# Blackgaurd/pathtracer-cpp

Hardware: AMD Instinct MI355X
Metric: Mray/s (all bounces) + achieved HBM GB/s, Cornell 1024² 10k spp depth-5 (higher is better)
Workload: dtype f32

## Files before the change

include/pt_hip_debug.h:

```cpp
#ifndef PT_HIP_DEBUG_H
#define PT_HIP_DEBUG_H

#include "pt_hip.h"

#ifdef __cplusplus
extern "C" {
#endif

int pt_debug_math(int device, int which, const float* in, int n, float* out);
int pt_debug_sweep(int device, int which, uint32_t lo_bits, uint32_t hi_bits, uint64_t* mismatches,
                   uint32_t* first_bad);
int pt_debug_rgb8(int device, const float* linear_rgb, int32_t res_x, int32_t res_y, float gamma, uint8_t* rgb8);
int pt_debug_rccl_failover(int32_t n_devices, int32_t fail_step, int64_t* out);
int pt_debug_wide_verify(const pt_scene* scene, int32_t width);
int pt_debug_pack_hash(const pt_scene* scene, uint64_t* hash);
int pt_rtc_check(const pt_scene* scene, char* src_out, size_t cap);
int pt_debug_rtc_start(const pt_scene* scene);
int64_t pt_debug_rtc_cache(int32_t op);

int pt_debug_ctx_flags(const pt_ctx* ctx, int32_t out[5]);
int pt_debug_ctx_plan(const pt_ctx* ctx, int64_t out[24]);
int pt_debug_walk_placement(int32_t num_nodes, int32_t num_tris, int32_t tree_depth, int32_t tri_f4,
                            int32_t rec_rows, uint64_t lds_usable, int32_t out[4]);
int pt_debug_scene_dark(const pt_scene* scene);
int pt_debug_emit_reject(const float* box6, const float* org, const float* dir, int64_t n, uint8_t* out);
int pt_debug_emit_slab_reject(const float* box6, const float* org, const float* inv, int64_t n, uint8_t* out);
int pt_debug_emit_box(const pt_scene* scene, float out[6]);
int pt_debug_ctx_emit_reject(const pt_ctx* ctx, int32_t* on, float box[6], uint64_t* early);
int pt_debug_ray_stack(int32_t which, int32_t count, int32_t n, int32_t reserve, int32_t flag);
int64_t pt_debug_counter(int32_t which);

#ifdef __cplusplus
}
#endif
#endif
```

pathtracer-cpp_amd/csrc/pt_kernel.hip:

```cpp
#include <hip/hip_runtime.h>

#include <stdint.h>
#include <stdio.h>
#include <stdlib.h>
#include <string.h>

#include <algorithm>
#include <chrono>
#include <future>
#include <map>
#include <memory>
#include <mutex>
#include <string>
#include <thread>
#include <vector>

#include <atomic>

#include "pt_grad.h"
#include "pt_hip_debug.h"
#include "pt_launch.h"
#include "pt_moments.h"
#include "pt_nee_grad.h"
#include "pt_rtc.h"
// ... 226 lines not shown
            const v3 r = __builtin_fabsf(x) <= 2.0f ? rcp3_exact<true>(v3{x, x, x}) : rcp3_exact<false>(v3{x, x, x});
            const uint32_t q = __float_as_uint(1.0f / x);
            same = __float_as_uint(r.x) == q && __float_as_uint(r.y) == q && __float_as_uint(r.z) == q;
        } else if (which >= 6 && which <= 9) {
            const uint32_t h1 = pt_mix32(bits * 0x9e3779b9u + 0x7f4a7c15u), h2 = pt_mix32(h1 ^ 0x85ebca6bu);
            auto pick = [&](uint32_t h, uint32_t k) {
                const uint32_t sign = h & 0x80000000u, mant = h & 0x7fffffu;
                if (which <= 7 && (bits & 15u) == 11u) {
                    switch (k & 7u) {
                        case 0: return __uint_as_float(sign);
                        case 1: return __uint_as_float(sign | mant | 1u);
                        case 2: return 0x1p127f;
                        case 3: return __uint_as_float(sign | 0x7f800000u);
                        case 4: return __uint_as_float(sign | 0x7e800000u | mant | 1u);
                        case 5: return __uint_as_float(sign | 0x7f000000u | mant);
                        case 6: return __uint_as_float(sign | 1u);
                        default: return __uint_as_float(0x80000000u);
                    }
                }
                const uint32_t e = (which == 6 || which == 9) ? 1u + (h >> 23) % 252u : 87u + (h >> 23) % 81u;
                return __uint_as_float(sign | (e << 23) | mant);
            };
            v3 a{x, pick(h1, h1 >> 8), pick(h2, (h1 >> 8) + 3u)};
            if (which == 9 && (bits & 15u) == 11u) a.y = __uint_as_float((h1 & 0x80000000u) | 0x7fc00000u | (h1 & 0x3fffffu));
            v3 r, q;
            if (which == 6 || which == 9) {
                r = rcp3_exact<false>(a);
                q = v3{1.0f / a.x, 1.0f / a.y, 1.0f / a.z};
            } else {
                r = normalize_fast(a);
                const float len = __builtin_sqrtf(dot(a, a));
                q = v3{a.x / len, a.y / len, a.z / len};
            }
            same = __float_as_uint(r.x) == __float_as_uint(q.x) &&
                   (__float_as_uint(r.y) == __float_as_uint(q.y) || (which == 9 && r.y != r.y && q.y != q.y)) &&
                   __float_as_uint(r.z) == __float_as_uint(q.z);
        } else {
            float s1, c1, s0, c0;
            sincosf_fast(x, s1, c1);
            sincosf_ref(x, s0, c0);
            same = __float_as_uint(s1) == __float_as_uint(s0) && __float_as_uint(c1) == __float_as_uint(c0);
        }
        if (!same) {
            nb++;
            fb = min(fb, bits);
        }
    }
    if (nb) {
        atomicAdd(bad, nb);
        atomicMin(first, fb);
    }
}

}

using namespace pt;

struct pt_ctx {
    int device = 0;
    hipStream_t stream = nullptr;
    std::thread init;
    std::once_flag init_once;
    std::string init_error;
    bool counted = false;
    int num_cus = 0;
    size_t lds_usable = 0;
    float4* d_nodes = nullptr;
    float4* d_tris = nullptr;
    float4* d_mats = nullptr;
    float4* d_leaves = nullptr;
    float4* d_wide = nullptr;
    float4* d_wtris = nullptr;
    float4* d_nrm = nullptr;
    float4* d_umats = nullptr;
    int32_t* d_rank_tri = nullptr;
    std::vector<f4> flat_host;
    FlatLeaves flat_tab;
    int flat_boxes_padded = 0;
    PackedScene meta;
    bool have_scene = false;
    bool has_specular = false;
    bool albedo_x2 = false;
    bool dark = false;
    EmitBox emit;
    uint64_t last_early = 0;
    void* flat_fast = nullptr;
    int flat_boxes = 0;
    bool rtc_requested = false;
    float* d_radiance = nullptr;
    size_t radiance_floats = 0;
    uint32_t* d_flags = nullptr;
    size_t flags_words = 0;
    float* d_accum = nullptr;
    size_t accum_floats = 0;
    float* d_out = nullptr;
    size_t out_floats = 0;
    unsigned long long* d_ctr = nullptr;
    unsigned long long* d_stamps = nullptr;
    int* d_xstack = nullptr;
    size_t xstack_ints = 0;
    uint8_t* d_rgb8 = nullptr;
    size_t rgb8_bytes = 0;
    float* d_thr = nullptr;
    int* d_qstack = nullptr;
    size_t qstack_ints = 0;
    float* d_qbuf = nullptr;
    size_t qbuf_floats = 0;
    unsigned long long* d_qhits = nullptr;
    float* d_tslab = nullptr;
    size_t tslab_floats = 0;
    float* d_trec = nullptr;
    size_t trec_words = 0;
    float* d_tbuf = nullptr;
    size_t tbuf_floats = 0;
    float* d_tstates = nullptr;
    size_t tstates_words = 0;
    unsigned long long* d_tctr = nullptr;
    LightTable lights;
    bool lights_uploaded = false;
    uint8_t* d_lights = nullptr;
    size_t lights_bytes = 0;
    double* d_gtab = nullptr;
    size_t gtab_doubles = 0;
    float4* d_gmats = nullptr;
    size_t gmats_f4 = 0;
    float* d_gbuf = nullptr;
    size_t gbuf_floats = 0;
    double* d_mom = nullptr;
    size_t mom_doubles = 0;
    unsigned long long* d_mcount = nullptr;
    float* d_sem = nullptr;
    size_t sem_floats = 0;
    int32_t* d_alist[2] = {nullptr, nullptr};
    size_t alist_ints[2] = {0, 0};
    int32_t* d_aspp = nullptr;
    size_t aspp_ints = 0;
    float* d_aslab = nullptr;
    size_t aslab_floats = 0;
    float* d_arec = nullptr;
    size_t arec_words = 0;
    unsigned long long* d_actr = nullptr;
    void* d_dn[kDnScratchSlots] = {};
    size_t dn_bytes[kDnScratchSlots] = {};
    TemporalState temporal;
    bool prog_valid = false;
    bool prog_moments = false;
    int prog_spp = 0;
    int prog_npix = 0;
    pt_camera prog_cam{};
    pt_params prog_prm{};
    hipFunction_t rtc_flat = nullptr;
    std::string rtc_status;
    std::string rtc_src;
    RtcFuture rtc_job;
    int64_t last_plan[24] = {};
};

namespace {

#define HIP_TRY(expr)                                                                              \
    do {                                                                                           \
        hipError_t e_ = (expr);                                                                    \
        if (e_ != hipSuccess) return set_error(PT_E_HIP, "%s failed: %s", #expr, hipGetErrorString(e_)); \
    } while (0)

int ctx_ready(pt_ctx* c) {
    std::call_once(c->init_once, [c] {
        if (c->init.joinable()) c->init.join();
    });
    if (!c->init_error.empty()) return set_error(PT_E_HIP, "%s", c->init_error.c_str());
    return PT_OK;
}

std::mutex g_dev_mu;
std::map<int, int> g_dev_contexts;

size_t batch_bytes_budget(int device, bool compile_pending) {
    const char* e = hook_env("PT_BATCH_BYTES");
    if (e && *e) return (size_t)strtoull(e, nullptr, 0);
    int sharers = 1;
    {
        std::lock_guard<std::mutex> lock(g_dev_mu);
        sharers = std::max(1, g_dev_contexts[device]);
    }
    size_t budget = ((size_t)(compile_pending ? 16 : 48) << 30) / sharers, free_b = 0, total_b = 0;
    if (hipMemGetInfo(&free_b, &total_b) == hipSuccess && free_b / 2 / sharers < budget) budget = free_b / 2 / sharers;
    return std::max<size_t>(budget, (size_t)64 << 20);
}

std::atomic<int64_t> g_ctx_created{0}, g_scene_uploads{0};

constexpr double kRtcWaitPaths = 256.0 * 1024 * 1024;

constexpr int kTailDiv = 0;

}

int64_t pt::kernel_counter(int which) { return which == 0 ? g_ctx_created.load() : g_scene_uploads.load(); }

int pt::ctx_release_slabs(pt_ctx* c) {
    if (!c) return PT_OK;
    if (int rc = ctx_ready(c)) return rc;
    HIP_TRY(hipSetDevice(c->device));
    if (c->stream) HIP_TRY(hipStreamSynchronize(c->stream));
    if (c->d_radiance) (void)hipFree(c->d_radiance);
    if (c->d_flags) (void)hipFree(c->d_flags);
    c->d_radiance = nullptr;
    c->radiance_floats = 0;
    c->d_flags = nullptr;
    c->flags_words = 0;
    if (c->d_mom) (void)hipFree(c->d_mom);
    c->d_mom = nullptr;
    c->mom_doubles = 0;
    if (c->prog_moments) c->prog_valid = false;
    return PT_OK;
}


namespace {

void rtc_resolve(pt_ctx* c, bool wait) {
    if (!c->rtc_job.valid()) return;
    if (!wait && c->rtc_job.wait_for(std::chrono::seconds(0)) != std::future_status::ready) return;
    c->rtc_flat = rtc_load(c->device, c->rtc_src, *c->rtc_job.get(), c->rtc_status);
    if (!c->rtc_flat && c->rtc_status == "evicted") {
        c->rtc_job = rtc_job(c->rtc_src);
        c->rtc_status = "compiling";
        if (wait) rtc_resolve(c, true);
        return;
    }
    c->rtc_job = RtcFuture();
    c->rtc_src.clear();
}

}

static std::mutex g_theta_mu;
static std::map<int, float2*> g_theta_tabs;

static void theta_table_release(int device) {
    std::lock_guard<std::mutex> dev_lock(g_dev_mu);
    std::lock_guard<std::mutex> lock(g_theta_mu);
    if (g_dev_contexts[device] != 0) return;
    auto it = g_theta_tabs.find(device);
    if (it == g_theta_tabs.end()) return;
    (void)hipFree(it->second);
    g_theta_tabs.erase(it);
}

[[maybe_unused]] static int theta_table(pt_ctx* c, const float2** out) {
    std::lock_guard<std::mutex> lock(g_theta_mu);
    auto it = g_theta_tabs.find(c->device);
    if (it != g_theta_tabs.end()) {
        *out = it->second;
        return PT_OK;
    }
    float2* t = nullptr;
    HIP_TRY(hipMalloc((void**)&t, sizeof(float2) * (size_t)kThetaEntries));
    hipLaunchKernelGGL(pt_theta_table_kernel, dim3((kThetaEntries + kBlock - 1) / kBlock), dim3(kBlock), 0, c->stream, t);
    const hipError_t e = hipStreamSynchronize(c->stream);
    if (e != hipSuccess) {
        (void)hipFree(t);
        return set_error(PT_E_HIP, "theta table: %s", hipGetErrorString(e));
    }
    g_theta_tabs[c->device] = t;
    *out = t;
    return PT_OK;
}

namespace {

struct RenderPlan {
    PartShape shape;
    int s_lo = 0, spp = 0;
    int batch = 0, per_item = 1, tail = 0;
    bool fused = false, flagged = false;
    bool moments = false;
    int flags_pm = 0;
    size_t slab_floats = 0, slab_words = 0;
    bool flat = false, wide = false, pairs = false, wide_single = false, lds_scene = false;
    int rec = 1, stack = 1, exact_rows = 1;
    int pair_queue = 0, wide_rows = 0, wide_queue = 0, wide_top = 0;
    size_t box_tab_bytes = 0, lds_bytes = 0;
    TraceKernel kern = nullptr;
    bool use_rtc = false;
    bool may_switch = false;
    int rtc_switch_at = -1;
    int blocks_per_cu = 1;
};

int force_exact_slab() {
    const char* fe = hook_env("PT_FORCE_EXACT_SLAB");
    return (fe && (*fe == '1' || *fe == '2')) ? *fe - '0' : 0;
}

void plan_batch(const pt_ctx* c, const pt_params* prm, RenderPlan& P) {
    const int npix = P.shape.npix, spp = P.spp, s_lo = P.s_lo;
    int batch = prm->batch_spp > 0 ? prm->batch_spp : 0;
    const bool compile_pending = c->rtc_job.valid();
    bool halved = false;
    if (batch <= 0) {
        const size_t per_sample = 3 * sizeof(float) * (size_t)std::max(npix, 1);
        const size_t whole = std::max<size_t>(1, batch_bytes_budget(c->device, compile_pending) / per_sample);
        halved = (size_t)std::max(spp - s_lo, 1) > whole;
        batch = (int)std::min<size_t>(halved ? (whole + 1) / 2 : whole, (size_t)INT32_MAX);
    }
    batch = std::max(1, std::min(batch, std::max(spp - s_lo, 1)));
    int per_item = prm->samples_per_item > 0 ? std::min(prm->samples_per_item, batch) : 1;
    batch = (int)std::min<long long>(batch, std::max<long long>(per_item, ((1ll << 31) - 1) / std::max(npix, 1) * per_item));
    if (P.flat && per_item != 1) {
        per_item = 1;
        batch = (int)std::min<long long>(batch, std::max<long long>(1, ((1ll << 31) - 1) / std::max(npix, 1)));
    }
    bool fused = (spp - s_lo) > batch && !hook_off("PT_FUSED_ACC") && !P.moments;
    if (fused && prm->batch_spp <= 0 && !halved) batch = std::max(1, (batch + 1) / 2);
    if (fused && prm->batch_spp > 0 && 2 * 3 * sizeof(float) * (size_t)batch * npix > batch_bytes_budget(c->device, compile_pending))
        fused = false;
    P.batch = batch;
    P.per_item = per_item;
    P.fused = fused;
    P.slab_floats = 3 * (size_t)batch * npix;
    const int tail_div = std::max(0, hook_int("PT_TAIL_DIV", kTailDiv));
    P.tail = fused && tail_div > 0 ? std::max(1, batch / tail_div) : 0;
    P.flagged = c->dark && !hook_off("PT_FLAGS");
    const char* pm_env = hook_env("PT_FLAGS_PM");
    const bool several = fused || (P.moments && (spp - s_lo) > batch);
    P.flags_pm = (pm_env && *pm_env) ? (*pm_env == '1' ? 1 : 0) : (several ? 1 : 0);
    P.slab_words = P.flags_pm ? ((size_t)batch + 31) / 32 * npix : ((size_t)batch * npix + 31) / 32;
}

int batch_at(const RenderPlan& P, int s0) {
    const int left = P.spp - s0;
    if (P.tail <= 0 || left <= P.tail) return std::min(P.batch, left);
    return left <= P.batch + P.tail ? left - P.tail : P.batch;
}

size_t flat_lds_bytes(const pt_ctx* c, const RenderPlan& P, int queue) {
    return sizeof(float4) * (size_t)(3 + 2) * c->meta.num_tris + sizeof(uint16_t) * (size_t)queue * (kBlock / kWave) +
           (sizeof(uint16_t) + sizeof(float)) * (size_t)kBlock * P.rec + sizeof(unsigned long long) * kBlock +
           (sizeof(float4) + sizeof(uint32_t)) * kBlock + P.box_tab_bytes;
}

void plan_flat(const pt_ctx* c, RenderPlan& P) {
    P.pairs = !hook_off("PT_PAIRS");
    P.box_tab_bytes = (sizeof(uint16_t) * (size_t)c->flat_boxes + 3) & ~(size_t)3;
    int queue = P.pairs ? 512 : 0;
    const char* pq = hook_env("PT_PAIR_QUEUE");
    if (P.pairs && pq && *pq) {
        queue = std::max(1, std::min(queue, atoi(pq)));
    } else if (P.pairs && c->lds_usable > 0) {
        auto blocks = [&](int q) { return std::min(8, lds_blocks(c->lds_usable, flat_lds_bytes(c, P, q))); };
        const int want = blocks(kPairQueueMin);
        while (queue > kPairQueueMin && blocks(queue) < want) queue -= 32;
    }
    P.pair_queue = (queue + 3) & ~3;
    P.lds_scene = true;
    P.lds_bytes = flat_lds_bytes(c, P, P.pair_queue);
}

size_t wide_lds_bytes(const pt_ctx* c, const RenderPlan& P, int top) {
    return (size_t)top * 16 * kWideNodeU4(c->meta.wide_width, c->meta.wide_fmt) + sizeof(int) * (size_t)kBlock * P.wide_rows +
           (P.wide_single ? 4 : 8) * (size_t)P.wide_queue * (kBlock / kWave) +
           (sizeof(float) + (P.lds_scene ? sizeof(uint8_t) : sizeof(int))) * (size_t)kBlock * P.rec +
           sizeof(unsigned long long) * kBlock + (P.lds_scene ? sizeof(float4) * 2 * (size_t)c->meta.num_umats : 0);
}

int plan_wide(const pt_ctx* c, RenderPlan& P) {
    if (c->meta.num_tris >= (1 << 26))
        return set_error(PT_E_ARG, "wide path: %d triangles exceed 2^26", c->meta.num_tris);
    P.wide_rows = std::max(1, c->meta.wide_depth - 1);
    P.wide_queue = 160;
    if (const char* wl = hook_env("PT_WIDE_QUEUE_LEN")) P.wide_queue = std::max(64, std::min(1024, atoi(wl)));
    P.wide_top = c->meta.wide_top;
    P.wide_single = c->meta.wide_single && !hook_off("PT_WIDE_SINGLE");
    P.lds_scene = c->meta.num_umats <= std::min(hook_int("PT_UMAT_LDS_MAX", kMaxLdsMaterials), kMaxLdsRowsByte);
    P.lds_bytes = wide_lds_bytes(c, P, P.wide_top);
    return PT_OK;
}

int shrink_wide_top(const pt_ctx* c, RenderPlan& P) {
    int full = 0, with = 0, rc;
    if ((rc = occupancy((const void*)P.kern, wide_lds_bytes(c, P, 0), c->lds_usable, &full, "render"))) return rc;
    while (P.wide_top > 0) {
        if ((rc = occupancy((const void*)P.kern, wide_lds_bytes(c, P, P.wide_top), c->lds_usable, &with, "render"))) return rc;
        if (with >= full) break;
        P.wide_top--;
    }
    P.lds_bytes = wide_lds_bytes(c, P, P.wide_top);
    return PT_OK;
}

void plan_tree(const pt_ctx* c, RenderPlan& P) {
    const size_t work = sizeof(int) * (size_t)kBlock * (P.stack + 2 * P.rec);
    const size_t scene = sizeof(float4) * ((size_t)2 * c->meta.num_nodes + (size_t)(3 + 2) * c->meta.num_tris);
    P.lds_scene = scene <= lds_scene_budget() && scene + work <= 64 * 1024;
    P.lds_bytes = work + (P.lds_scene ? scene : 0);
}

int plan_render(pt_ctx* c, const PartShape& shape, const pt_params* prm, int s_lo, int spp, bool moments, RenderPlan& P) {
    P.shape = shape;
    P.moments = moments;
    P.s_lo = s_lo;
    P.spp = spp;
    P.rec = std::max(1, prm->depth - 1);
    P.stack = std::max(1, c->meta.tree_depth);
    P.exact_rows = std::max(1, c->meta.tree_depth);
    const char* wenv = hook_env("PT_WIDE");
    const bool flat_ok = flat_eligible(c->meta) && !hook_off("PT_FLAT");
    P.wide = c->meta.num_wide > 0 && !(wenv && *wenv == '0') && (!flat_ok || (wenv && *wenv == '1'));
    P.flat = flat_ok && !P.wide;
    plan_batch(c, prm, P);
    int rc;
    if (P.flat) plan_flat(c, P);
    else if (P.wide) {
        if ((rc = plan_wide(c, P))) return rc;
    } else plan_tree(c, P);
    if (P.lds_bytes > 160 * 1024)
        return set_error(PT_E_ARG, "BVH depth (%d) x path depth needs %zu B of LDS", P.wide ? P.wide_rows : P.stack, P.lds_bytes);
    const bool rtc_switch = !hook_off("PT_RTC_SWITCH");
    P.rtc_switch_at = hook_int("PT_RTC_SWITCH_AT", -1);
    if (P.flat && c->rtc_job.valid()) rtc_resolve(c, !rtc_switch && (double)shape.npix * (spp - s_lo) >= kRtcWaitPaths);
    P.kern = P.flat        ? (c->flat_fast                    ? (TraceKernel)c->flat_fast
                              : ray_stack_on(c->has_specular) ? pt_trace_kernel<true, true>
                                                              : pt_trace_kernel<true, true, 0, kWideByte, false>)
             : P.wide      ? wide_kernel(c->meta.wide_width, c->meta.wide_fmt, P.lds_scene)
             : P.lds_scene ? pt_trace_kernel<true, false>
                           : pt_trace_kernel<false, false>;
    P.use_rtc = P.flat && c->rtc_flat != nullptr;
    if (P.wide && P.wide_top > 0 && (rc = shrink_wide_top(c, P))) return rc;
    if ((rc = P.use_rtc ? plan_grid_module(c->rtc_flat, P.lds_bytes, c->lds_usable, c->num_cus, 0, &P.blocks_per_cu, nullptr, "render")
                        : plan_grid((const void*)P.kern, P.lds_bytes, c->lds_usable, c->num_cus, 0, &P.blocks_per_cu, nullptr, "render")))
        return rc;
    P.may_switch = P.flat && !P.use_rtc && c->rtc_job.valid();
    return PT_OK;
}

int render_buffers(pt_ctx* c, const RenderPlan& P, bool out_is_device) {
    const size_t npix = (size_t)P.shape.npix;
    int rc;
    if ((rc = ensure(&c->d_accum, &c->accum_floats, 3 * npix))) return rc;
    if (P.moments && (rc = ensure(&c->d_mom, &c->mom_doubles, 6 * npix))) return rc;
    if (!out_is_device && (rc = ensure(&c->d_out, &c->out_floats, 3 * npix))) return rc;
    if (P.wide || P.flat) {
        const size_t need = (size_t)(P.may_switch ? std::max(P.blocks_per_cu, 8) : P.blocks_per_cu) * c->num_cus * kBlock * P.exact_rows;
        if ((rc = ensure(&c->d_xstack, &c->xstack_ints, need))) return rc;
    }
    if ((rc = ensure(&c->d_radiance, &c->radiance_floats, (P.fused ? 2 : 1) * P.slab_floats))) return rc;
    if (P.flagged && (rc = ensure(&c->d_flags, &c->flags_words, (P.fused ? 2 : 1) * P.slab_words))) return rc;
    return PT_OK;
}

int theta_choice(pt_ctx* c, int* lanes, const float2** tab) {
    *lanes = 0;
    *tab = nullptr;
#if PT_THETA_TAB
    *lanes = hook_int("PT_THETA_LANES", c->has_specular ? 32 : 0);
    if (PT_THETA_TAB == 1 || *lanes > 0) {
        if (int rc = theta_table(c, tab)) {
            if (PT_THETA_TAB == 1) return rc;
            *lanes = 0;
            *tab = nullptr;
        }
    }
#else
    (void)c;
#endif
    return PT_OK;
}

void build_flat_table(pt_ctx* c) {
    memset(&c->flat_tab, 0, sizeof(c->flat_tab));
    c->flat_boxes_padded = 0;
    if (!flat_eligible(c->meta)) return;
    int nb = 0;
    for (int k = 0; k < c->meta.num_leaves; k++) {
        const f4* L = &c->flat_host[2 * k];
        const float b6[6] = {L[0].x, L[0].y, L[0].z, L[0].w, L[1].x, L[1].y};
        int u = 0;
        while (u < nb && memcmp(c->flat_tab.box[u], b6, sizeof(b6)) != 0) u++;
        if (u == nb) {
            memcpy(c->flat_tab.box[nb], b6, sizeof(b6));
            c->flat_tab.bits[nb++] = 0;
        }
        c->flat_tab.bits[u] |= 1ull << k;
    }
    c->flat_boxes_padded = (nb + 3) & ~3;
    for (int u = nb; u < c->flat_boxes_padded; u++) memcpy(c->flat_tab.box[u], c->flat_tab.box[0], sizeof(c->flat_tab.box[0]));
}

int fill_trace_args(pt_ctx* c, const RenderPlan& P, const pt_camera* cam, const pt_params* prm, TraceArgs& A) {
    memset(&A, 0, sizeof(A));
    A.nodes = c->d_nodes;
    A.tris = c->d_tris;
    A.mats = c->d_mats;
    A.leaves = c->d_leaves;
    A.wide = reinterpret_cast<const uint4*>(c->d_wide);
    A.wtris = c->d_wtris;
    A.nrm = c->d_nrm;
    A.umats = c->d_umats;
    A.num_umat4 = P.wide ? 2 * c->meta.num_umats : 0;
    if (P.flat) {
        A.num_leaves = c->meta.num_leaves;
        A.num_boxes_padded = c->flat_boxes_padded;
        A.flat = c->flat_tab;
    }
    A.radiance = c->d_radiance;
    const float2* theta_tab = nullptr;
    if (int rc = theta_choice(c, &A.theta_lanes, &theta_tab)) return rc;
    A.theta_tab = theta_tab;
    A.work = c->d_ctr;
    A.ctr = c->d_ctr;
    A.dark = c->dark ? 1 : 0;
    A.emit_on = emit_mode(c->emit);
    A.emit_lo_x = c->emit.lo[0], A.emit_lo_y = c->emit.lo[1], A.emit_lo_z = c->emit.lo[2];
    A.emit_hi_x = c->emit.hi[0], A.emit_hi_y = c->emit.hi[1], A.emit_hi_z = c->emit.hi[2];
    fill_camera(A, cam, P.shape, prm);
    A.depth = prm->depth;
    A.per_item = P.per_item;
    A.stack_size = P.stack;
    A.rec_size = P.rec;
    A.num_node4 = 2 * c->meta.num_nodes;
    A.num_tri4 = 3 * c->meta.num_tris;
    A.num_mat4 = 2 * c->meta.num_tris;
    A.force_exact_slab = force_exact_slab();
    A.wide_thresh = std::max(1, std::min(64, hook_int("PT_WIDE_THRESH", 28)));
    A.pair_queue = P.pair_queue;
    A.wide_rows = P.wide_rows;
    A.exact_stack = c->d_xstack;
    A.exact_rows = P.exact_rows;
    A.wide_queue = P.wide_queue;
    A.wide_top = P.wide_top;
    A.wide_nodes = P.wide ? (uint32_t)c->meta.num_wide : 0u;
    A.wide_span_x = c->meta.wide_span[0];
    A.wide_span_y = c->meta.wide_span[1];
    A.wide_span_z = c->meta.wide_span[2];
    A.wide_single = P.wide_single ? 1 : 0;
    A.wide_compact = P.wide && c->meta.wide_compact ? 1 : 0;
    A.tri_fast = P.wide && c->meta.coords_small && !hook_off("PT_WIDE_NB") ? 1 : 0;
    const char* wq = hook_env("PT_WIDE_QUEUE_CAP");
    if (P.wide && wq && *wq) A.wide_queue = std::max(1, std::min(A.wide_queue, atoi(wq)));
    A.regen_thresh = std::max(1, std::min(64, hook_int("PT_REGEN_THRESH", c->has_specular ? 40 : 32)));
    A.ray_reserve = ray_reserve();
    A.flags_pm = P.flags_pm;
    A.acc_chunks = 0;
    return PT_OK;
}

struct RenderEvents {
    std::vector<hipEvent_t> ev;
    ~RenderEvents() {
        for (hipEvent_t e : ev) (void)hipEventDestroy(e);
    }
};

struct LaunchLog {
    std::vector<int> samples;
    int grid = 0, chunk = 0, acc_every = 0;
    uint32_t static_items = 0;
};

int launch_batch(pt_ctx* c, RenderPlan& P, TraceArgs& A, int b, int s0, int sc, int prev_s0, int prev_sc, float* dst, int keep,
                 RenderEvents& E, LaunchLog& log) {
    const int npix = P.shape.npix;
    auto flags_at = [&](int k) -> uint32_t* {
        return P.flagged ? c->d_flags + (P.fused ? (size_t)(k & 1) * P.slab_words : 0) : nullptr;
    };
    A.s_begin = s0;
    A.s_count = sc;
    float* slab = c->d_radiance + (P.fused ? (size_t)(b & 1) * P.slab_floats : 0);
    A.radiance = slab;
    A.flags = flags_at(b);
    const size_t words_b = P.flags_pm ? ((size_t)sc + 31) / 32 * npix : ((size_t)sc * npix + 31) / 32;
    if (A.flags && hipMemsetAsync(A.flags, 0, words_b * sizeof(uint32_t), c->stream) != hipSuccess)
        return set_error(PT_E_HIP, "hipMemsetAsync of the slab flags failed");
    A.total_items = (unsigned long long)((sc + P.per_item - 1) / P.per_item) * (unsigned long long)npix;
    if (A.total_items >= (1ull << 31))
        return set_error(PT_E_ARG, "batch of %d samples x %d pixels exceeds 2^31 work items", sc, npix);
    if (P.flat && !P.use_rtc && c->rtc_job.valid() && b >= 1) {
        (void)hipEventSynchronize(E.ev[3 * (size_t)(b - 1) + 1]);
        rtc_resolve(c, b == P.rtc_switch_at);
        if (c->rtc_flat) {
            int rb = 0;
            if (int rc = plan_grid_module(c->rtc_flat, P.lds_bytes, c->lds_usable, c->num_cus, 0, &rb, nullptr, "render")) return rc;
            P.blocks_per_cu = std::min(rb, 8);
            P.use_rtc = true;
        }
    }
    const unsigned long long want_blocks = (A.total_items + kBlock - 1) / kBlock;
    const int grid = (int)std::min<unsigned long long>(want_blocks, (unsigned long long)P.blocks_per_cu * c->num_cus);
    const PoolSizing pool = pool_sizing(A.total_items, grid, P.flat ? 512 : 128);
    A.chunk = pool.chunk;
    A.static_items = pool.static_items;
    A.static_base = pool.static_base;
    hipEvent_t e[3] = {nullptr, nullptr, nullptr};
    for (hipEvent_t& ek : e) {
        if (hipEventCreate(&ek) != hipSuccess) {
            for (hipEvent_t made : e)
                if (made) (void)hipEventDestroy(made);
            return set_error(PT_E_HIP, "hipEventCreate failed");
        }
    }
    E.ev.insert(E.ev.end(), e, e + 3);
    (void)hipMemsetAsync(c->d_ctr, 0, sizeof(unsigned long long), c->stream);
    if (P.fused && prev_s0 >= 0) {
        A.acc_src = c->d_radiance + (size_t)((b - 1) & 1) * P.slab_floats;
        A.acc_flags = flags_at(b - 1);
        A.acc_sum = c->d_accum;
        A.acc_count = prev_sc;
        A.acc_first = prev_s0 == 0 ? 1 : 0;
        A.acc_chunks = (npix + kWave - 1) / kWave;
        const unsigned long long refills =
            std::max<unsigned long long>(1, (A.total_items - A.static_base) / (unsigned long long)A.chunk);
        const unsigned long long div = (unsigned long long)std::max(1, hook_int("PT_ACC_DIV", 2));
        A.acc_every = (int)std::max<unsigned long long>(1, refills / (div * (unsigned long long)A.acc_chunks));
        (void)hipMemsetAsync(c->d_ctr + 2, 0, sizeof(unsigned long long), c->stream);
    } else {
        A.acc_chunks = 0;
        A.acc_flags = nullptr;
    }
    (void)hipEventRecord(e[0], c->stream);
    if (P.use_rtc) {
        size_t arg_bytes = sizeof(A);
        void* cfg[] = {HIP_LAUNCH_PARAM_BUFFER_POINTER, &A, HIP_LAUNCH_PARAM_BUFFER_SIZE, &arg_bytes,
                       HIP_LAUNCH_PARAM_END};
        const hipError_t le = hipModuleLaunchKernel(c->rtc_flat, grid, 1, 1, kBlock, 1, 1, (unsigned)P.lds_bytes,
                                                    c->stream, nullptr, cfg);
        if (le != hipSuccess) return set_error(PT_E_HIP, "hipModuleLaunchKernel failed: %s", hipGetErrorString(le));
    } else {
        hipLaunchKernelGGL(P.kern, dim3(grid), dim3(kBlock), P.lds_bytes, c->stream, A);
    }
    (void)hipEventRecord(e[1], c->stream);
    if (P.moments)
        hipLaunchKernelGGL(pt_accumulate_moments_kernel, dim3((npix + kBlock - 1) / kBlock), dim3(kBlock), 0, c->stream,
                           slab, c->d_accum, dst, c->d_mom, npix, sc, s0 == 0 ? 1 : 0, s0 + sc >= P.spp ? 1 : 0,
                           (float)P.spp, A.flags, P.flags_pm);
    else if (!P.fused || s0 + sc >= P.spp)
        hipLaunchKernelGGL(pt_accumulate_kernel, dim3((npix + kBlock - 1) / kBlock), dim3(kBlock), 0, c->stream, slab,
                           c->d_accum, dst, npix, sc, s0 == 0 ? 1 : 0, s0 + sc >= P.spp ? 1 : 0, keep, (float)P.spp, A.flags,
                           P.flags_pm);
    (void)hipEventRecord(e[2], c->stream);
    log.samples.push_back(sc);
    log.grid = grid;
    log.chunk = A.chunk;
    log.static_items = A.static_items;
    log.acc_every = A.acc_chunks ? A.acc_every : 0;
    return PT_OK;
}

#ifdef PT_STAMPS
void report_stamps(const pt_ctx* c, bool wide, const unsigned long long* h_ctr) {
    unsigned long long hs[kStampSections];
    if (hipMemcpy(hs, c->d_stamps, sizeof(hs), hipMemcpyDeviceToHost) == hipSuccess) {
        if (wide) {
            const double tot = (double)(hs[0] + hs[1] + hs[2] + hs[3] + hs[4]);
            fprintf(stderr,
                    "[stamps] wide: waves %llu  cycles/wave %.3g  start %.1f%%  steps %.1f%%  drains %.1f%%  "
                    "shade %.1f%%  fold %.1f%%  | steps/wave %.0f, traversing lanes/step %.1f, in-loop drains/wave %.0f\n",
                    hs[6], tot / (double)(hs[6] ? hs[6] : 1), 100 * hs[0] / tot, 100 * hs[1] / tot, 100 * hs[2] / tot,
                    100 * hs[3] / tot, 100 * hs[4] / tot, (double)hs[7] / (hs[6] ? hs[6] : 1),
                    (double)hs[8] / (hs[7] ? hs[7] : 1), (double)hs[9] / (hs[6] ? hs[6] : 1));
            const double oi = (double)(hs[10] ? hs[10] : 1), ray = (double)(h_ctr[1] ? h_ctr[1] : 1);
            fprintf(stderr,
// ... 201 lines not shown
            HIP_TRY(hipGetLastError());
        }
        if (!is_device) HIP_TRY(hipMemcpyAsync(mom->sem, dst, nval * sizeof(float), hipMemcpyDeviceToHost, c->stream));
    }
    HIP_TRY(hipStreamSynchronize(c->stream));
    return PT_OK;
}

int unconverged_count(pt_ctx* c, float rel, float abs_tol, int64_t* count, uint8_t* mask, int mask_is_device, double* ms) {
    const int npix = c->prog_npix;
    *count = 0;
    if (npix <= 0) return PT_OK;
    HIP_TRY(hipSetDevice(c->device));
    if (!c->d_mcount) HIP_TRY(hipMalloc((void**)&c->d_mcount, sizeof(unsigned long long)));
    uint8_t* d_mask = mask;
    if (mask && !mask_is_device) {
        if (int rc = ensure(&c->d_rgb8, &c->rgb8_bytes, (size_t)npix)) return rc;
        d_mask = c->d_rgb8;
    }
    hipEvent_t e0 = nullptr, e1 = nullptr;
    if (ms && (hipEventCreate(&e0) != hipSuccess || hipEventCreate(&e1) != hipSuccess)) {
        if (e0) (void)hipEventDestroy(e0);
        return set_error(PT_E_HIP, "hipEventCreate failed");
    }
    unsigned long long h = 0;
    hipError_t e = hipMemsetAsync(c->d_mcount, 0, sizeof(unsigned long long), c->stream);
    if (ms) (void)hipEventRecord(e0, c->stream);
    hipLaunchKernelGGL(pt_unconverged_kernel, dim3((npix + kBlock - 1) / kBlock), dim3(kBlock), 0, c->stream, c->d_mom, npix,
                       c->prog_spp, (double)rel, (double)abs_tol, c->d_mcount, d_mask);
    if (ms) (void)hipEventRecord(e1, c->stream);
    if (e == hipSuccess) e = hipGetLastError();
    if (e == hipSuccess) e = hipMemcpyAsync(&h, c->d_mcount, sizeof(h), hipMemcpyDeviceToHost, c->stream);
    if (e == hipSuccess && mask && !mask_is_device)
        e = hipMemcpyAsync(mask, d_mask, (size_t)npix, hipMemcpyDeviceToHost, c->stream);
    if (e == hipSuccess) e = hipStreamSynchronize(c->stream);
    if (ms) {
        float t = 0;
        if (e == hipSuccess && hipEventElapsedTime(&t, e0, e1) == hipSuccess) *ms += t;
        (void)hipEventDestroy(e0);
        (void)hipEventDestroy(e1);
    }
    if (e != hipSuccess) return set_error(PT_E_HIP, "convergence count failed: %s", hipGetErrorString(e));
    *count = (int64_t)h;
    return PT_OK;
}

}

extern "C" {

int pt_device_count(void) {
    int n = 0;
    if (hipGetDeviceCount(&n) != hipSuccess) return 0;
    return n;
}

int pt_ctx_create(int device, pt_ctx** out) {
    if (!out) return set_error(PT_E_ARG, "pt_ctx_create: out is NULL");
    *out = nullptr;
    const bool timed = hook_env("PT_TIME_CTX") != nullptr;
    auto t_last = std::chrono::steady_clock::now();
    auto phase = [&](const char* what) {
        if (!timed) return;
        const auto t = std::chrono::steady_clock::now();
        fprintf(stderr, "[pt_ctx_create] %s %.3f ms\n", what, std::chrono::duration<double, std::milli>(t - t_last).count());
        t_last = t;
    };
    int n = 0;
    if (hipGetDeviceCount(&n) != hipSuccess || n <= 0) return set_error(PT_E_HIP, "no HIP device available");
    if (device < 0 || device >= n) return set_error(PT_E_ARG, "device %d out of range (have %d)", device, n);
    HIP_TRY(hipSetDevice(device));
    phase("device count + set");
    pt_ctx* c = new pt_ctx();
    c->device = device;
    hipDeviceProp_t prop;
    if (hipGetDeviceProperties(&prop, device) != hipSuccess) {
        delete c;
        return set_error(PT_E_HIP, "hipGetDeviceProperties failed");
    }
    phase("device properties");
    c->num_cus = prop.multiProcessorCount;
    c->lds_usable = strncmp(prop.gcnArchName, "gfx950", 6) == 0 ? kLdsUsable
                    : prop.sharedMemPerMultiprocessor > 0   ? (size_t)prop.sharedMemPerMultiprocessor
                                                            : (size_t)65536;
    auto make = [c] {
        if (hipSetDevice(c->device) != hipSuccess) c->init_error = "hipSetDevice failed";
        else if (hipStreamCreateWithFlags(&c->stream, hipStreamNonBlocking) != hipSuccess)
            c->init_error = "stream creation failed";
        else if (hipMalloc((void**)&c->d_ctr, 5 * sizeof(unsigned long long)) != hipSuccess)
            c->init_error = "counter allocation failed";
    };
    const char* cs = hook_env("PT_CTX_SYNC");
    if (!(cs && *cs == '1')) {
        try {
            c->init = std::thread(make);
        } catch (const std::system_error&) {
        }
    }
    if (!c->init.joinable()) make();
    if (!c->init_error.empty()) {
        const std::string err = c->init_error;
        pt_ctx_destroy(c);
        return set_error(PT_E_HIP, "%s", err.c_str());
    }
    phase("stream + counter (started)");
    {
        std::lock_guard<std::mutex> lock(g_dev_mu);
        g_dev_contexts[device]++;
    }
    c->counted = true;
    g_ctx_created++;
    *out = c;
    return PT_OK;
}

void pt_ctx_destroy(pt_ctx* c) {
    if (!c) return;
    (void)ctx_ready(c);
    bool last = false;
    if (c->counted) {
        std::lock_guard<std::mutex> lock(g_dev_mu);
        last = --g_dev_contexts[c->device] == 0;
    }
    (void)hipSetDevice(c->device);
    if (c->stream) (void)hipStreamSynchronize(c->stream);
    if (last) theta_table_release(c->device);
    for (void* p : {(void*)c->d_nodes, (void*)c->d_tris, (void*)c->d_mats, (void*)c->d_leaves, (void*)c->d_wide, (void*)c->d_wtris, (void*)c->d_nrm, (void*)c->d_umats, (void*)c->d_radiance, (void*)c->d_flags,
                    (void*)c->d_accum, (void*)c->d_out, (void*)c->d_ctr, (void*)c->d_stamps, (void*)c->d_rgb8, (void*)c->d_thr, (void*)c->d_xstack,
                    (void*)c->d_rank_tri, (void*)c->d_qstack, (void*)c->d_qbuf, (void*)c->d_qhits,
                    (void*)c->d_tslab, (void*)c->d_trec, (void*)c->d_tbuf, (void*)c->d_tstates, (void*)c->d_tctr,
                    (void*)c->d_lights,
                    (void*)c->d_gtab, (void*)c->d_gmats, (void*)c->d_gbuf, (void*)c->d_mom, (void*)c->d_mcount, (void*)c->d_sem,
                    (void*)c->d_alist[0], (void*)c->d_alist[1], (void*)c->d_aspp, (void*)c->d_aslab, (void*)c->d_arec, (void*)c->d_actr})
        if (p) (void)hipFree(p);
    for (void* p : c->d_dn)
        if (p) (void)hipFree(p);
    if (c->stream) (void)hipStreamDestroy(c->stream);
    delete c;
}

int pt_ctx_set_scene(pt_ctx* c, const pt_scene* scene) {
    if (!c) return set_error(PT_E_ARG, "context is NULL");
    g_scene_uploads++;
    PackedScene ps;
    int rc = pack_scene(scene, ps);
    if (rc) return rc;
    const bool specular = scene_has_specular(ps);
    const bool albedo_x2 = albedo_x2_ok(ps);
    const bool dark = scene_dark(ps);
    const EmitBox emit = scene_emit_box(ps, dark);
    const bool want_rtc = flat_eligible(ps) && !hook_off("PT_RTC");
    std::string src;
    RtcFuture job;
    if (want_rtc) {
        src = rtc_flat_source(ps.leaves, ps.num_leaves, specular, ps.coords_small, albedo_x2, dark, emit);
        job = rtc_job(src);
    }
    if ((rc = ctx_ready(c))) return rc;
    HIP_TRY(hipSetDevice(c->device));
    for (float4** p : {&c->d_nodes, &c->d_tris, &c->d_mats, &c->d_leaves, &c->d_wide, &c->d_wtris, &c->d_nrm, &c->d_umats}) {
        if (*p) (void)hipFree(*p);
        *p = nullptr;
    }
    if (c->d_rank_tri) (void)hipFree(c->d_rank_tri);
    c->d_rank_tri = nullptr;
    c->have_scene = false;
    c->prog_valid = false;
    c->temporal.valid = false;
    c->lights_uploaded = false, scene_light_table(scene, c->lights);
    HIP_TRY(hipMalloc((void**)&c->d_nodes, ps.nodes.size() * sizeof(float4)));
    HIP_TRY(hipMalloc((void**)&c->d_tris, ps.tris.size() * sizeof(float4)));
    HIP_TRY(hipMalloc((void**)&c->d_mats, ps.mats.size() * sizeof(float4)));
    HIP_TRY(hipMemcpyAsync(c->d_nodes, ps.nodes.data(), ps.nodes.size() * sizeof(float4), hipMemcpyHostToDevice,
                           c->stream));
    HIP_TRY(hipMemcpyAsync(c->d_tris, ps.tris.data(), ps.tris.size() * sizeof(float4), hipMemcpyHostToDevice,
                           c->stream));
    HIP_TRY(hipMemcpyAsync(c->d_mats, ps.mats.data(), ps.mats.size() * sizeof(float4), hipMemcpyHostToDevice,
                           c->stream));
    HIP_TRY(hipMalloc((void**)&c->d_rank_tri, ps.rank_tri.size() * sizeof(int32_t)));
    HIP_TRY(hipMemcpyAsync(c->d_rank_tri, ps.rank_tri.data(), ps.rank_tri.size() * sizeof(int32_t),
                           hipMemcpyHostToDevice, c->stream));
    if (!ps.leaves.empty()) {
        HIP_TRY(hipMalloc((void**)&c->d_leaves, ps.leaves.size() * sizeof(float4)));
        HIP_TRY(hipMemcpyAsync(c->d_leaves, ps.leaves.data(), ps.leaves.size() * sizeof(float4),
                               hipMemcpyHostToDevice, c->stream));
    }
    if (!ps.wide.empty()) {
        HIP_TRY(hipMalloc((void**)&c->d_wide, ps.wide.size() * sizeof(float4)));
        HIP_TRY(hipMemcpyAsync(c->d_wide, ps.wide.data(), ps.wide.size() * sizeof(float4), hipMemcpyHostToDevice,
                               c->stream));
        HIP_TRY(hipMalloc((void**)&c->d_wtris, ps.wtris.size() * sizeof(float4)));
        HIP_TRY(hipMemcpyAsync(c->d_wtris, ps.wtris.data(), ps.wtris.size() * sizeof(float4), hipMemcpyHostToDevice,
                               c->stream));
        HIP_TRY(hipMalloc((void**)&c->d_nrm, ps.nrm.size() * sizeof(float4)));
        HIP_TRY(hipMemcpyAsync(c->d_nrm, ps.nrm.data(), ps.nrm.size() * sizeof(float4), hipMemcpyHostToDevice,
                               c->stream));
        HIP_TRY(hipMalloc((void**)&c->d_umats, ps.umats.size() * sizeof(float4)));
        HIP_TRY(hipMemcpyAsync(c->d_umats, ps.umats.data(), ps.umats.size() * sizeof(float4), hipMemcpyHostToDevice,
                               c->stream));
    }
    HIP_TRY(hipStreamSynchronize(c->stream));
    ps.wide.clear();
    ps.wtris.clear();
    ps.nrm.clear();
    ps.umats.clear();
    ps.nodes.clear();
    ps.tris.clear();
    ps.mats.clear();
    ps.rank_tri.clear();
    c->has_specular = specular;
    c->dark = dark;
    c->emit = emit;
    c->albedo_x2 = false;
    c->flat_fast = nullptr;
    if (flat_eligible(ps) && !hook_off("PT_FLAT_FAST") && leaves_single(ps.leaves, ps.num_leaves) && ps.coords_small &&
        c->dark && albedo_x2)
        c->flat_fast = flat_fast_kernel(specular, ps.num_leaves <= 32);
    c->flat_boxes = 0;
    c->rtc_requested = false;
    c->flat_host = ps.leaves;
    ps.leaves.clear();
    c->meta = ps;
    build_flat_table(c);
    c->rtc_flat = nullptr;
    c->rtc_job = RtcFuture();
    c->rtc_src.clear();
    c->rtc_status = "not a flat scene";
    if (want_rtc) {
        c->rtc_src = std::move(src);
        c->albedo_x2 = albedo_x2;
        c->rtc_requested = true;
        c->flat_boxes = flat_box_pairs(c->flat_host, ps.num_leaves);
        c->rtc_job = job;
        c->rtc_status = "compiling";
        const char* w = hook_env("PT_RTC_WAIT");
        if ((w && *w == '1') || !rtc_async_ready()) rtc_resolve(c, true);
    }
    c->have_scene = true;
    return PT_OK;
}

int pt_rtc_wait(void) { return rtc_wait_all(); }

int pt_ctx_prepare(pt_ctx* c) {
    if (!c) return set_error(PT_E_ARG, "context is NULL");
    if (int rc = ctx_ready(c)) return rc;
    if (c->rtc_job.valid()) {
        HIP_TRY(hipSetDevice(c->device));
        rtc_resolve(c, true);
    }
    return PT_OK;
}

int pt_ctx_render(pt_ctx* c, const pt_camera* cam, const pt_params* prm, float* out, int out_is_device,
                  pt_stats* stats) {
    if (c) c->prog_valid = false;
    return render_range(c, cam, prm, 0, prm && prm->spp > 0 ? prm->spp : 0, 0, out, out_is_device, stats);
}

int pt_ctx_render_progressive(pt_ctx* c, const pt_camera* cam, const pt_params* prm, int32_t s_first,
                              int32_t s_count, float* out, int out_is_device, pt_stats* stats) {
    if (!c || !cam || !prm) return set_error(PT_E_ARG, "pt_ctx_render_progressive: NULL argument");
    if (s_first < 0 || s_count < 0 || (long long)s_first + s_count > 0x7fffffffll)
        return set_error(PT_E_ARG, "pt_ctx_render_progressive: bad sample range");
    if (s_first > 0 && !continues_sum(c, false, cam, prm, s_first))
        return set_error(PT_E_ARG,
                         "progressive render: samples from %d do not continue this context's running sum "
                         "(%d samples, a moments sum, or another camera / parameters)",
                         s_first, c->prog_valid && !c->prog_moments ? c->prog_spp : 0);
    c->prog_valid = false;
    const int rc = render_range(c, cam, prm, s_first, s_first + s_count, 1, out, out_is_device, stats);
    if (rc) return rc;
    keep_sum(c, false, cam, prm, s_first + s_count, 0);
    return PT_OK;
}

int pt_ctx_render_moments(pt_ctx* c, const pt_camera* cam, const pt_params* prm, int32_t s_first, int32_t s_count,
                          float* out, const pt_moments* mom, int out_is_device, pt_stats* stats) {
    const int rc = moments_range(c, cam, prm, s_first, s_count, out, out_is_device, stats);
    if (rc && rc != PT_E_RUNAWAY) return rc;
    if (int xrc = moments_export(c, mom, out_is_device, c->prog_npix, c->prog_spp)) return xrc;
    return rc;
}

int pt_ctx_unconverged(pt_ctx* c, float rel, float abs_tol, int64_t* count, uint8_t* mask, int mask_is_device) {
    if (!c || !count) return set_error(PT_E_ARG, "pt_ctx_unconverged: NULL argument");
    if (!tolerances_ok(rel, abs_tol))
        return set_error(PT_E_ARG, "pt_ctx_unconverged: rel and abs must be >= 0 and not both 0");
    if (!c->prog_valid || !c->prog_moments)
        return set_error(PT_E_ARG, "pt_ctx_unconverged: the context has no running moments sum");
    return unconverged_count(c, rel, abs_tol, count, mask, mask_is_device, nullptr);
}

int pt_ctx_render_converge(pt_ctx* c, const pt_camera* cam, const pt_params* prm, const pt_converge* cv, float* out,
                           const pt_moments* mom, int out_is_device, pt_converge_stats* cs) {
    const auto t_start = std::chrono::steady_clock::now();
    if (!c || !cam || !prm || !cv) return set_error(PT_E_ARG, "pt_ctx_render_converge: NULL argument");
    if (!tolerances_ok(cv->rel, cv->abs))
        return set_error(PT_E_ARG, "pt_ctx_render_converge: rel and abs must be >= 0 and not both 0");
    if (cv->min_spp < 2 || cv->max_spp < cv->min_spp || cv->step < 0 || cv->max_unconverged < 0)
        return set_error(PT_E_ARG, "pt_ctx_render_converge: needs 2 <= min_spp <= max_spp, step >= 0, max_unconverged >= 0");
    pt_converge_stats S{};
    int runaway = PT_OK;
    for (int32_t done = 0, n = cv->min_spp;;) {
        pt_stats st{};
        const int rc = moments_range(c, cam, prm, done, n - done, out_is_device ? out : nullptr, out_is_device, &st);
        if (rc && rc != PT_E_RUNAWAY) return rc;
        if (rc) runaway = rc;
        S.rays += st.rays;
        S.kernel_ms += st.kernel_ms;
        S.reduce_ms += st.reduce_ms;
        if (int urc = unconverged_count(c, cv->rel, cv->abs, &S.unconverged, nullptr, 0, &S.reduce_ms)) return urc;
        S.rounds++;
        S.spp = done = n;
        if (S.unconverged <= cv->max_unconverged || n >= cv->max_spp) break;
        const int64_t next = cv->step > 0 ? (int64_t)n + cv->step : 2 * (int64_t)n;
        n = (int32_t)std::min<int64_t>(next, cv->max_spp);
    }
    if (out && !out_is_device && c->prog_npix > 0) {
        HIP_TRY(hipMemcpyAsync(out, c->d_out, 3 * (size_t)c->prog_npix * sizeof(float), hipMemcpyDeviceToHost, c->stream));
        HIP_TRY(hipStreamSynchronize(c->stream));
    }
    if (int xrc = moments_export(c, mom, out_is_device, c->prog_npix, c->prog_spp)) return xrc;
    S.total_ms = std::chrono::duration<double, std::milli>(std::chrono::steady_clock::now() - t_start).count();
    if (cs) *cs = S;
    if (runaway)
        return set_error(PT_E_RUNAWAY, "specular rejection loops hit the %d-iteration bound during the rounds", kMaxSpecularIters);
    return PT_OK;
}

}

namespace {

constexpr int64_t kQueryChunk = 1ll << 28;
constexpr int64_t kQueryHostChunk = 1ll << 22;

QueryScene query_scene(const pt_ctx* c) {
    return QueryScene{reinterpret_cast<const f4*>(c->d_nodes), reinterpret_cast<const f4*>(c->d_tris),
                      reinterpret_cast<const f4*>(c->d_mats), c->d_rank_tri, c->meta.num_nodes, c->meta.num_tris,
                      c->meta.tree_depth};
}

int query_force_exact() {
    return force_exact_slab() ? 1 : 0;
}

int query_buffers(pt_ctx* c, const WalkPlan& plan) {
    if (plan.stack_ints > 0)
        if (int rc = ensure(&c->d_qstack, &c->qstack_ints, plan.stack_ints)) return rc;
    if (!c->d_qhits) HIP_TRY(hipMalloc((void**)&c->d_qhits, sizeof(unsigned long long)));
    HIP_TRY(hipMemsetAsync(c->d_qhits, 0, sizeof(unsigned long long), c->stream));
    return PT_OK;
}

struct EventPair {
    hipEvent_t a = nullptr, b = nullptr;
    int create() {
        HIP_TRY(hipEventCreate(&a));
        HIP_TRY(hipEventCreate(&b));
        return PT_OK;
    }
    ~EventPair() {
        if (a) (void)hipEventDestroy(a);
        if (b) (void)hipEventDestroy(b);
    }
};

int query_finish(pt_ctx* c, const WalkPlan& plan, uint64_t rays, double kernel_ms, int launches,
                 std::chrono::steady_clock::time_point t_start, pt_query_stats* stats) {
    unsigned long long hits = 0;
    HIP_TRY(hipMemcpyAsync(&hits, c->d_qhits, sizeof(hits), hipMemcpyDeviceToHost, c->stream));
    HIP_TRY(hipStreamSynchronize(c->stream));
    if (stats) {
        stats->rays = rays;
        stats->hits = hits;
        stats->kernel_ms = kernel_ms;
        stats->total_ms = std::chrono::duration<double, std::milli>(std::chrono::steady_clock::now() - t_start).count();
        stats->launches = launches;
        stats->lds_scene = plan.lds_scene;
        stats->lds_stack = plan.lds_stack;
    }
// ... 903 lines not shown
    if (!c || slot < 0 || slot >= kDnScratchSlots) return set_error(PT_E_ARG, "ctx_scratch: bad argument");
    if (int rc = ctx_ready(c)) return rc;
    HIP_TRY(hipSetDevice(c->device));
    if (int rc = ensure_bytes(&c->d_dn[slot], &c->dn_bytes[slot], bytes, 1)) return rc;
    *out = c->d_dn[slot];
    return PT_OK;
}

void* pt::ctx_stream(pt_ctx* c) { return c && ctx_ready(c) == PT_OK ? (void*)c->stream : nullptr; }

pt::TemporalState* pt::ctx_temporal_state(pt_ctx* c) { return &c->temporal; }

int pt::rgb8_device(pt_ctx* c, const float* d_lin, int rows, int W, float gamma, int flip, uint8_t* d_dst) {
    if (int rc0 = ctx_ready(c)) return rc0;
    float thr[256];
    int32_t neg_mode = 0;
    const int rc = pt_rgb8_thresholds(gamma, thr, &neg_mode);
    if (rc) return rc;
    thr[255] = __builtin_inff();
    if (rows > 65535) return set_error(PT_E_ARG, "pt_rgb8: %d rows exceed the quantiser grid", rows);
    if (!c->d_thr) HIP_TRY(hipMalloc((void**)&c->d_thr, 256 * sizeof(float)));
    HIP_TRY(hipMemcpyAsync(c->d_thr, thr, sizeof(thr), hipMemcpyHostToDevice, c->stream));
    if (rows > 0 && W > 0)
        hipLaunchKernelGGL(pt_rgb8_kernel, dim3((3 * W + kBlock - 1) / kBlock, rows), dim3(kBlock), 0, c->stream,
                           d_lin, d_dst, c->d_thr, rows, W, flip, neg_mode);
    HIP_TRY(hipGetLastError());
    HIP_TRY(hipStreamSynchronize(c->stream));
    return PT_OK;
}

extern "C" {

int pt_ctx_render_rgb8(pt_ctx* c, const pt_camera* cam, const pt_params* prm, float gamma, int flip, uint8_t* out,
                       int out_is_device, pt_stats* stats) {
    if (!c || !cam || !prm || !out) return set_error(PT_E_ARG, "pt_ctx_render_rgb8: NULL argument");
    PartShape shape;
    int rc;
    if ((rc = part_shape(cam, prm, -1, &shape))) return rc;
    const int rows = shape.rows, W = shape.W;
    const size_t n = (size_t)shape.npix * 3;
    HIP_TRY(hipSetDevice(c->device));
    if ((rc = ensure(&c->d_out, &c->out_floats, n))) return rc;
    c->prog_valid = false;
    if ((rc = render_range(c, cam, prm, 0, prm->spp > 0 ? prm->spp : 0, 0, c->d_out, 1, stats))) return rc;
    uint8_t* dst = out;
    if (!out_is_device) {
        if ((rc = ensure(&c->d_rgb8, &c->rgb8_bytes, n))) return rc;
        dst = c->d_rgb8;
    }
    if ((rc = rgb8_device(c, c->d_out, rows, W, gamma, flip, dst))) return rc;
    if (!out_is_device && n) HIP_TRY(hipMemcpy(out, dst, n, hipMemcpyDeviceToHost));
    return PT_OK;
}

int pt_debug_rgb8(int device, const float* lin, int32_t W, int32_t H, float gamma, uint8_t* rgb8) {
    if (!lin || !rgb8 || W <= 0 || H <= 0) return set_error(PT_E_ARG, "pt_debug_rgb8: bad argument");
    pt_ctx* c = nullptr;
    int rc = pt_ctx_create(device, &c);
    if (rc) return rc;
    const size_t n = (size_t)W * H * 3;
    float* d_lin = nullptr;
    uint8_t* d_o = nullptr;
    hipError_t e = hipMalloc((void**)&d_lin, n * sizeof(float));
    if (e == hipSuccess) e = hipMalloc((void**)&d_o, n);
    if (e == hipSuccess) e = hipMemcpy(d_lin, lin, n * sizeof(float), hipMemcpyHostToDevice);
    if (e != hipSuccess) rc = set_error(PT_E_HIP, "pt_debug_rgb8: %s", hipGetErrorString(e));
    if (!rc) rc = rgb8_device(c, d_lin, H, W, gamma, 1, d_o);
    if (!rc && hipMemcpy(rgb8, d_o, n, hipMemcpyDeviceToHost) != hipSuccess)
        rc = set_error(PT_E_HIP, "pt_debug_rgb8: copy failed");
    if (d_lin) (void)hipFree(d_lin);
    if (d_o) (void)hipFree(d_o);
    pt_ctx_destroy(c);
    return rc;
}

int pt_render_f32(const pt_scene* scene, const pt_camera* cam, const pt_params* params, float* out_rgb,
                  pt_stats* stats) {
    if (!params) return set_error(PT_E_ARG, "params is NULL");
    if (scene && scene->num_tris <= 0) return set_error(PT_E_EMPTY, "No triangles in scene.");
    pt_ctx* c = nullptr;
    int rc = pt_ctx_create(0, &c);
    if (rc) return rc;
    rc = pt_ctx_set_scene(c, scene);
    if (!rc) {
        pt_params p = *params;
        p.part_index = 0;
        p.part_count = 1;
        if (p.band_rows <= 0) p.band_rows = 1;
        rc = pt_ctx_render(c, cam, &p, out_rgb, 0, stats);
    }
    pt_ctx_destroy(c);
    return rc;
}

int pt_debug_ctx_flags(const pt_ctx* c, int32_t out[5]) {
    if (!c || !out) return set_error(PT_E_ARG, "pt_debug_ctx_flags: NULL argument");
    out[0] = c->albedo_x2 ? 1 : 0;
    out[1] = c->has_specular ? 1 : 0;
    out[2] = c->rtc_requested ? 1 : 0;
    out[3] = c->meta.num_wide;
    out[4] = c->dark ? 1 : 0;
    return PT_OK;
}

int pt_debug_ctx_emit_reject(const pt_ctx* c, int32_t* on, float box[6], uint64_t* early) {
    if (!c) return set_error(PT_E_ARG, "pt_debug_ctx_emit_reject: NULL argument");
    if (on) *on = c->emit.on ? 1 : 0;
    if (box)
        for (int a = 0; a < 3; a++) box[a] = c->emit.lo[a], box[3 + a] = c->emit.hi[a];
    if (early) *early = c->last_early;
    return PT_OK;
}

int pt_debug_emit_box(const pt_scene* scene, float out[6]) {
    if (!out) return set_error(PT_E_ARG, "pt_debug_emit_box: NULL argument");
    PackedScene ps;
    const int rc = pack_scene(scene, ps);
    if (rc) return rc;
    const EmitBox e = scene_emit_box(ps, scene_dark(ps));
    for (int a = 0; a < 3; a++) out[a] = e.lo[a], out[3 + a] = e.hi[a];
    return e.on ? 1 : 0;
}

int pt_debug_emit_reject(const float* box6, const float* org, const float* dir, int64_t n, uint8_t* out) {
    if (!box6 || !org || !dir || !out || n < 0) return set_error(PT_E_ARG, "pt_debug_emit_reject: bad argument");
    for (int64_t i = 0; i < n; i++) {
        const float *b = box6 + 6 * i, *o = org + 3 * i, *d = dir + 3 * i;
        out[i] = emit_reject(v3{b[0], b[1], b[2]}, v3{b[3], b[4], b[5]}, v3{o[0], o[1], o[2]}, v3{d[0], d[1], d[2]}) ? 1 : 0;
    }
    return PT_OK;
}

int pt_debug_emit_slab_reject(const float* box6, const float* org, const float* inv, int64_t n, uint8_t* out) {
    if (!box6 || !org || !inv || !out || n < 0) return set_error(PT_E_ARG, "pt_debug_emit_slab_reject: bad argument");
    for (int64_t i = 0; i < n; i++) {
        const float *b = box6 + 6 * i, *o = org + 3 * i, *v = inv + 3 * i;
        out[i] = emit_slab_reject(v3{b[0], b[1], b[2]}, v3{b[3], b[4], b[5]}, v3{o[0], o[1], o[2]}, v3{v[0], v[1], v[2]}) ? 1 : 0;
    }
    return PT_OK;
}

int pt_debug_ray_stack(int32_t which, int32_t count, int32_t n, int32_t reserve, int32_t flag) {
    switch (which) {
        case 0: return ray_stack_generate(count, n, reserve, flag != 0) ? 1 : 0;
        case 1: return ray_stack_filled(count, n);
        case 2: return ray_stack_dry(count, n) ? 1 : 0;
        case 3: return ray_stack_slot(count, n);
        case 4: return ray_stack_taken(count, n);
        case 5: return ray_stack_done(flag != 0, count, n != 0) ? 1 : 0;
    }
    return set_error(PT_E_ARG, "pt_debug_ray_stack: which = %d", which);
}

int pt_debug_ctx_plan(const pt_ctx* c, int64_t out[24]) {
    if (!c || !out) return set_error(PT_E_ARG, "pt_debug_ctx_plan: NULL argument");
    memcpy(out, c->last_plan, sizeof(c->last_plan));
    return PT_OK;
}

int pt_debug_scene_dark(const pt_scene* scene) {
    PackedScene ps;
    const int rc = pack_scene(scene, ps);
    if (rc) return rc;
    return scene_dark(ps) ? 1 : 0;
}

int pt_debug_math(int device, int which, const float* in, int n, float* out) {
    if (!in || !out || n <= 0 || which < 0 || which > 2) return set_error(PT_E_ARG, "pt_debug_math: bad argument");
    HIP_TRY(hipSetDevice(device));
    const size_t in_n = (size_t)n * (which == 2 ? 9 : 1), out_n = (size_t)n * (which == 0 ? 1 : which == 1 ? 2 : 4);
    float *di = nullptr, *dout = nullptr;
    HIP_TRY(hipMalloc((void**)&di, in_n * sizeof(float)));
    if (hipMalloc((void**)&dout, out_n * sizeof(float)) != hipSuccess) {
        (void)hipFree(di);
        return set_error(PT_E_HIP, "hipMalloc failed");
    }
    hipError_t e = hipMemcpy(di, in, in_n * sizeof(float), hipMemcpyHostToDevice);
    if (e == hipSuccess) {
        hipLaunchKernelGGL(pt_math_kernel, dim3((n + 255) / 256), dim3(256), 0, 0, which, di, dout, n);
        e = hipGetLastError();
    }
    if (e == hipSuccess) e = hipMemcpy(out, dout, out_n * sizeof(float), hipMemcpyDeviceToHost);
    (void)hipFree(di);
    (void)hipFree(dout);
    if (e != hipSuccess) return set_error(PT_E_HIP, "pt_debug_math: %s", hipGetErrorString(e));
    return PT_OK;
}

int pt_debug_sweep(int device, int which, uint32_t lo_bits, uint32_t hi_bits, uint64_t* mismatches,
                   uint32_t* first_bad) {
    if (!mismatches || !first_bad || which < 0 || which > 9 || hi_bits < lo_bits)
        return set_error(PT_E_ARG, "pt_debug_sweep: bad argument");
    HIP_TRY(hipSetDevice(device));
    unsigned long long* d_bad = nullptr;
    uint32_t* d_first = nullptr;
    HIP_TRY(hipMalloc((void**)&d_bad, sizeof(unsigned long long)));
    if (hipMalloc((void**)&d_first, sizeof(uint32_t)) != hipSuccess) {
        (void)hipFree(d_bad);
        return set_error(PT_E_HIP, "hipMalloc failed");
    }
    hipError_t e = hipMemset(d_bad, 0, sizeof(unsigned long long));
    if (e == hipSuccess) e = hipMemset(d_first, 0xff, sizeof(uint32_t));
    if (e == hipSuccess) {
        const unsigned long long n = (unsigned long long)(hi_bits - lo_bits) + 1ull;
        hipLaunchKernelGGL(pt_sweep_kernel, dim3(8192), dim3(256), 0, 0, which, lo_bits, n, d_bad, d_first);
        e = hipGetLastError();
    }
    unsigned long long hb = 0;
    uint32_t hf = 0;
    if (e == hipSuccess) e = hipMemcpy(&hb, d_bad, sizeof(hb), hipMemcpyDeviceToHost);
    if (e == hipSuccess) e = hipMemcpy(&hf, d_first, sizeof(hf), hipMemcpyDeviceToHost);
    (void)hipFree(d_bad);
    (void)hipFree(d_first);
    if (e != hipSuccess) return set_error(PT_E_HIP, "pt_debug_sweep: %s", hipGetErrorString(e));
    *mismatches = hb;
    *first_bad = hf;
    return PT_OK;
}

}
```

pathtracer-cpp_amd/csrc/pt_rtc.h:

```cpp
#pragma once

#include <hip/hip_runtime_api.h>

#include <future>
#include <memory>
#include <string>
#include <vector>

#include "pt_internal.h"

namespace pt {

struct RtcCode {
    std::vector<char> code;
    std::string status;
    std::string disk_key;
};
typedef std::shared_future<std::shared_ptr<const RtcCode>> RtcFuture;

int flat_box_pairs(const std::vector<f4>& leaves, int n, std::vector<uint16_t>* tab = nullptr);
bool leaves_single(const std::vector<f4>& leaves, int n);
std::string rtc_flat_source(const std::vector<f4>& leaves, int n, bool specular, bool tri_fast, bool albedo_x2,
                            bool dark, const EmitBox& emit);
RtcFuture rtc_job(const std::string& src);
bool rtc_async_ready();
int rtc_wait_all();
hipFunction_t rtc_load(int device, const std::string& src, const RtcCode& code, std::string& status);

}
```

pathtracer-cpp_amd/csrc/pt_rtc.hip:

```cpp
#include <hip/hip_runtime.h>
#include <hip/hiprtc.h>

#include <dlfcn.h>
#include <errno.h>
#include <fcntl.h>
#include <link.h>
#include <signal.h>
#include <spawn.h>
#include <stdint.h>
#include <stdio.h>
#include <stdlib.h>
#include <string.h>
#include <sys/socket.h>
#include <sys/stat.h>
#include <sys/wait.h>
#include <unistd.h>

#include <algorithm>
#include <atomic>
#include <chrono>
#include <fstream>
#include <future>
#include <limits>
#include <map>
#include <memory>
#include <mutex>
#include <set>
#include <sstream>
#include <string>
#include <thread>
#include <vector>

extern char** environ;

#include "pt_hip_debug.h"
#include "pt_launch.h"
#include "pt_rtc.h"
#include "pt_sha256.h"
#include "pt_trace.h"

extern "C" const char* pt_rtc_src_trace;
extern "C" const char* pt_rtc_src_math;
extern "C" const char* pt_rtc_src_stack;
extern "C" const char* pt_rtc_src_hip;

namespace pt {

namespace {

std::string hexf(float v) {
    char b[64];
    snprintf(b, sizeof(b), "%af", (double)v);
    return b;
}

std::string litf(float v) {
    if (v == std::numeric_limits<float>::infinity()) return "__builtin_inff()";
    if (v == -std::numeric_limits<float>::infinity()) return "-__builtin_inff()";
    return hexf(v);
}

}

int flat_box_pairs(const std::vector<f4>& leaves, int n, std::vector<uint16_t>* tab) {
    const char* e = hook_env("PT_BOX_PAIRS");
    if (!e || *e != '1') return 0;
    std::map<std::vector<uint32_t>, int> box_id;
    std::vector<std::vector<int>> box_leaves;
    for (int k = 0; k < n; k++) {
        const f4 a = leaves[2 * k], b = leaves[2 * k + 1];
        if (__builtin_bit_cast(int, b.z) != k || __builtin_bit_cast(int, b.w) != k) return 0;
        const std::vector<uint32_t> key = {f2u(a.x), f2u(a.y), f2u(a.z), f2u(a.w), f2u(b.x), f2u(b.y)};
        auto it = box_id.find(key);
        if (it == box_id.end()) {
            it = box_id.emplace(key, (int)box_leaves.size()).first;
            box_leaves.emplace_back();
        }
        box_leaves[it->second].push_back(k);
    }
    for (const auto& l : box_leaves)
        if (l.size() > 2 || l.back() > 254) return 0;
    if (tab) {
        tab->clear();
        for (const auto& l : box_leaves) tab->push_back((uint16_t)(l[0] | ((l.size() > 1 ? l[1] : 0xff) << 8)));
    }
    return (int)box_leaves.size();
}

bool leaves_single(const std::vector<f4>& leaves, int n) {
    for (int k = 0; k < n; k++)
        if (__builtin_bit_cast(int, leaves[2 * k + 1].z) != k || __builtin_bit_cast(int, leaves[2 * k + 1].w) != k)
            return false;
    return true;
}

namespace {

std::string flat_mask_source(const std::vector<f4>& leaves, int n, bool specular, bool tri_fast, bool albedo_x2,
                             bool dark, const EmitBox& emit) {
    std::vector<std::map<uint32_t, int>> planes(3);
    auto plane = [&](int ax, float c) {
        auto it = planes[ax].find(f2u(c));
        if (it != planes[ax].end()) return it->second;
        const int id = (int)planes[ax].size();
        planes[ax][f2u(c)] = id;
        return id;
    };
    std::string body;
    std::map<std::vector<uint32_t>, int> box_id;
    std::vector<unsigned long long> box_bits;
    struct BoxExpr {
        std::string lo[3], hi[3];
    };
    std::vector<BoxExpr> boxes;
    for (int k = 0; k < n; k++) {
        const f4 a = leaves[2 * k], b = leaves[2 * k + 1];
        const float lb[3] = {a.x, a.y, a.z}, rt[3] = {a.w, b.x, b.y};
        std::vector<uint32_t> key = {f2u(lb[0]), f2u(lb[1]), f2u(lb[2]), f2u(rt[0]), f2u(rt[1]), f2u(rt[2])};
        auto it = box_id.find(key);
        if (it != box_id.end()) {
            box_bits[it->second] |= 1ull << k;
            continue;
        }
        const int id = (int)box_bits.size();
        box_id[key] = id;
        box_bits.push_back(1ull << k);
        BoxExpr e;
        const char ax_name[3] = {'x', 'y', 'z'};
        for (int ax = 0; ax < 3; ax++) {
            const std::string p1 = std::string("t") + ax_name[ax] + std::to_string(plane(ax, lb[ax]));
            const std::string p2 = std::string("t") + ax_name[ax] + std::to_string(plane(ax, rt[ax]));
            if (p1 == p2) {
                e.lo[ax] = e.hi[ax] = p1;
            } else {
                e.lo[ax] = "__builtin_fminf(" + p1 + ", " + p2 + ")";
                e.hi[ax] = "__builtin_fmaxf(" + p1 + ", " + p2 + ")";
            }
        }
        boxes.push_back(e);
    }
    std::map<std::string, int> lo_uses;
    for (const BoxExpr& e : boxes)
        for (int ax = 0; ax < 3; ax++) lo_uses[e.lo[ax]]++;
    std::map<std::string, std::string> clamp_name;
    std::string clamps, tests, tests_plain, tests_sign;
    for (size_t id = 0; id < boxes.size(); id++) {
        const BoxExpr& e = boxes[id];
        int cax = 0;
        for (int ax = 1; ax < 3; ax++)
            if (lo_uses[e.lo[ax]] > lo_uses[e.lo[cax]]) cax = ax;
        auto cn = clamp_name.find(e.lo[cax]);
        if (cn == clamp_name.end()) {
            const std::string nm = "c" + std::to_string(clamp_name.size());
            clamps += "        const float " + nm + " = __builtin_fmaxf(" + e.lo[cax] + ", 0.0f);\n";
            cn = clamp_name.emplace(e.lo[cax], nm).first;
        }
        const int a1 = cax == 0 ? 1 : 0, a2 = cax == 2 ? 1 : 2;
        const std::string tmax = "__builtin_fminf(__builtin_fminf(" + e.hi[0] + ", " + e.hi[1] + "), " + e.hi[2] + ")";
        tests += "        const bool b" + std::to_string(id) + " = __builtin_fmaxf(__builtin_fmaxf(" + e.lo[a1] + ", " +
                 e.lo[a2] + "), " + cn->second + ") <= " + tmax + ";\n";
        tests_plain += "        const bool b" + std::to_string(id) + " = __builtin_fmaxf(__builtin_fmaxf(__builtin_fmaxf(" +
                       e.lo[0] + ", " + e.lo[1] + "), " + e.lo[2] + "), 0.0f) <= " + tmax + ";\n";
        tests_sign += "        const uint32_t f" + std::to_string(id) + " = box_fail_bits(__builtin_fmaxf(__builtin_fmaxf(" +
                      e.lo[0] + ", " + e.lo[1] + "), " + e.lo[2] + "), " + tmax + " + 0.0f);\n";
    }
    tests = "#if KSIGN\n" + tests_sign + "#elif PT_SHARED_CLAMP\n" + clamps + tests + "#else\n" + tests_plain + "#endif\n";
    const char ax_name[3] = {'x', 'y', 'z'};
    body += "#if PT_PK_PLANES\n";
    for (int ax = 0; ax < 3; ax++) {
        const std::string comp(1, ax_name[ax]);
        std::vector<std::pair<uint32_t, int>> ps(planes[ax].begin(), planes[ax].end());
        if (ps.empty()) continue;
        body += "        const f2v o" + comp + "2 = {o." + comp + ", o." + comp + "}, i" + comp + "2 = {inv." + comp +
                ", inv." + comp + "};\n";
        for (size_t i = 0; i < ps.size(); i += 2) {
            const auto& a = ps[i];
            const auto& b = ps[i + 1 < ps.size() ? i + 1 : i];
            const std::string pv = "p" + comp + std::to_string(i);
            body += "        const f2v " + pv + " = (f2v{" + hexf(u2f(a.first)) + ", " + hexf(u2f(b.first)) + "} - o" +
                    comp + "2) * i" + comp + "2;\n";
            body += "        const float t" + comp + std::to_string(a.second) + " = " + pv + ".x;\n";
            if (i + 1 < ps.size()) body += "        const float t" + comp + std::to_string(b.second) + " = " + pv + ".y;\n";
        }
    }
    body += "#else\n";
    for (int ax = 0; ax < 3; ax++)
        for (const auto& kv : planes[ax]) {
            const std::string comp(1, ax_name[ax]);
            body += "        const float t" + comp + std::to_string(kv.second) + " = (" + hexf(u2f(kv.first)) +
                    " - o." + comp + ") * inv." + comp + ";\n";
        }
    body += "#endif\n";
    std::vector<int> leaf_box(n, -1);
    for (size_t i = 0; i < box_bits.size(); i++)
        for (int k = 0; k < n; k++)
            if (box_bits[i] >> k & 1) leaf_box[k] = (int)i;
    auto multi = [&](int k) { return __builtin_popcountll(box_bits[leaf_box[k]]) > 1; };
    std::string acc = "        uint32_t lo = 0, hi = 0;\n#if KSIGN\n";
    for (int k = n - 1; k >= 0; k--) {
        const char* w = k >= 32 ? "hi" : "lo";
        acc += std::string("        ") + w + " = shl1_add_sign(" + w + ", f" + std::to_string(leaf_box[k]) + ");\n";
    }
    acc += "        lo = ~lo" + std::string(n < 32 ? " & " + std::to_string((1u << n) - 1u) + "u" : "") + ";\n";
    if (n > 32) acc += "        hi = ~hi" + std::string(n < 64 ? " & " + std::to_string((uint32_t)((1ull << (n - 32)) - 1u)) + "u" : "") + ";\n";
    acc += "#else\n";
    for (int k = n - 1; k >= 0; k--) {
        const char* w = k >= 32 ? "hi" : "lo";
        const std::string bit = std::string("#if PT_ADDC_MASK\n        ") + w + " = shl1_add_bit(" + w +
                                ", __builtin_amdgcn_ballot_w64(b" + std::to_string(leaf_box[k]) + "));\n#else\n        " + w +
                                " = " + w + " + " + w + " + (b" + std::to_string(leaf_box[k]) + " ? 1u : 0u);\n#endif\n";
        if (multi(k))
            acc += std::string("#if PT_MULTI_LEAF_OR\n        ") + w + " = dbl_u32(" + w + ");\n#else\n" + bit + "#endif\n";
        else
            acc += bit;
    }
    acc += "#if PT_MULTI_LEAF_OR\n";
    for (size_t i = 0; i < box_bits.size(); i++) {
        const unsigned long long m = box_bits[i];
        if (__builtin_popcountll(m) < 2) continue;
        const std::string bal = "__builtin_amdgcn_ballot_w64(b" + std::to_string(i) + ")";
        if ((uint32_t)m)
            acc += "        lo = or_if_bit(lo, " + std::to_string((uint32_t)m) + "u, " + bal + ");\n";
        if ((uint32_t)(m >> 32))
            acc += "        hi = or_if_bit(hi, " + std::to_string((uint32_t)(m >> 32)) + "u, " + bal + ");\n";
    }
    acc += "#endif\n";
    acc += "#endif\n";
    std::vector<uint16_t> box_tab;
    const int nbox = flat_box_pairs(leaves, n, &box_tab);
    if (nbox > 0) {
        std::string chain = "        lo = 0;\n        hi = 0;\n";
        for (int u = nbox - 1; u >= 0; u--) {
            const char* w = u >= 32 ? "hi" : "lo";
            chain += std::string("        ") + w + " = shl1_add_bit(" + w + ", __builtin_amdgcn_ballot_w64(b" +
                     std::to_string(u) + "));\n";
        }
        acc = "#if KBOX\n        uint32_t lo, hi;\n" + chain + "#else\n" + acc + "#endif\n";
    }
    acc += "        const unsigned long long m = ((unsigned long long)hi << 32) | lo;\n";
    const bool single = leaves_single(leaves, n);
    const bool sign = tri_fast;
    std::string tabs = "{";
    for (size_t u = 0; u < box_tab.size(); u++) tabs += (u ? ", " : "") + std::to_string(box_tab[u]) + "u";
    tabs += box_tab.empty() ? "0u}" : "}";
    std::string rej = "    using EmitRej = NoEmitReject;\n";
    if (emit.on)
        rej = "    struct EmitRej {\n        static constexpr bool kCompiled = true;\n"
              "        __device__ __forceinline__ static bool on() { return true; }\n"
              "        __device__ __forceinline__ static bool rejected(v3 o, v3 d) {\n"
              "            return emit_reject(v3{" + litf(emit.lo[0]) + ", " + litf(emit.lo[1]) + ", " + litf(emit.lo[2]) +
              "}, v3{" + litf(emit.hi[0]) + ", " + litf(emit.hi[1]) + ", " + litf(emit.hi[2]) + "}, o, d);\n"
              "        }\n"
              "        static constexpr bool kSlab = !PT_EMIT_SIGN_ONLY;\n"
              "        __device__ __forceinline__ static bool rejected_slab(v3 o, v3, v3 inv) {\n"
              "            return emit_slab_reject(v3{" + litf(emit.lo[0]) + ", " + litf(emit.lo[1]) + ", " + litf(emit.lo[2]) +
              "}, v3{" + litf(emit.hi[0]) + ", " + litf(emit.hi[1]) + ", " + litf(emit.hi[2]) + "}, o, inv);\n"
              "        }\n    };\n";
    return std::string("#ifndef PT_FLAT_SIGN_MASK\n#define PT_FLAT_SIGN_MASK 0\n#endif\n#define KSIGN (PT_FLAT_SIGN_MASK && ") +
           (sign ? "1" : "0") + ")\n" + "#define KBOX " + (nbox > 0 ? "(!KSIGN)" : "0") + "\n" +
           "namespace pt {\nstruct SceneBoxMask {\n    static constexpr bool kSignMask = KSIGN;\n"
           "    static constexpr bool kBoxPairs = KBOX;\n    static constexpr bool kCamInvGen = PT_CAM_INV == 2;\n"
           "    static constexpr bool kRayStack = PT_RAY_STACK != 0;\n"
           "    static constexpr int kBoxes = " + std::to_string(nbox) +
           ";\n    static constexpr uint16_t kBoxTab[" + std::to_string(std::max<size_t>(1, box_tab.size())) + "] = " + tabs +
           ";\n    static constexpr bool kMask32 = " +
           (n <= 32 ? "true" : "false") + ";\n    static constexpr bool kSingleTri = " + (single ? "true" : "false") +
           ";\n    static constexpr bool kSpecular = " + (specular ? "true" : "false") +
           ";\n    static constexpr bool kTriFast = " + (tri_fast ? "true" : "false") +
           ";\n    static constexpr bool kAlbedoX2 = " + (albedo_x2 ? "true" : "false") +
           ";\n    static constexpr bool kDarkKnown = true;\n    static constexpr bool kDark = " + (dark ? "true" : "false") +
           ";\n" + rej + "    __device__ __forceinline__ static unsigned long long "
           "mask(const TraceArgs&, v3 o, v3 inv) {\n" +
           body + tests + acc + "        return m;\n    }\n};\n}  // namespace pt\n";
}

struct RtcCache {
    std::mutex mu;
    std::map<std::string, RtcFuture> code;
    std::map<std::pair<int, std::string>, hipFunction_t> funcs;
    std::set<std::string> refused;
};
RtcCache& rtc_cache() {
    static RtcCache* c = new RtcCache();
    return *c;
}

int rtc_waves() {
    const int w = hook_int("PT_RTC_WAVES", 8);
    return (w >= 1 && w <= 8) ? w : 8;
}

std::string rtc_defines() {
    const char* e = hook_env("PT_RTC_DEFINES");
    std::string out;
    if (!e) return out;
    std::stringstream ss(e);
    std::string item;
    while (std::getline(ss, item, ',')) {
        const size_t eq = item.find('=');
        if (!item.empty()) out += "#define " + (eq == std::string::npos ? item : item.substr(0, eq) + " " + item.substr(eq + 1)) + "\n";
    }
    return out;
}

std::vector<std::string> rtc_extra_flags() {
    std::vector<std::string> out;
    const char* e = hook_env("PT_RTC_FLAGS");
    if (!e) return out;
    std::string flags(e);
    std::replace(flags.begin(), flags.end(), ',', ' ');
    std::stringstream ss(flags);
    std::string f;
    while (ss >> f) out.push_back(f);
    return out;
}

}

std::string rtc_flat_source(const std::vector<f4>& leaves, int n, bool specular, bool tri_fast, bool albedo_x2,
                            bool dark, const EmitBox& emit) {
    std::string fl = "// extra flags:";
    for (const std::string& f : rtc_extra_flags()) fl += " " + f;
    return fl + "\n" + rtc_defines() + (emit.on && emit.sign_only ? "#define PT_EMIT_SIGN_ONLY 1\n" : "") +
           (ray_stack_on(specular) ? "#define PT_RAY_RESERVE " + std::to_string(ray_reserve()) + "\n" : "#define PT_RAY_STACK 0\n") +
           "#define PT_WAVES " + std::to_string(rtc_waves()) +
           "\n#define PT_FLAT_ONLY 1\n#ifndef PT_CAM_KERNARG\n#define PT_CAM_KERNARG 0\n#endif\n"
           "#ifndef PT_FRESH_TID\n#define PT_FRESH_TID " + (specular ? "1" : "0") + "\n#endif\n"
           "typedef __hip_internal::int32_t int32_t; typedef __hip_internal::uint32_t uint32_t;\n"
           "typedef __hip_internal::int64_t int64_t; typedef __hip_internal::uint64_t uint64_t;\n"
           "typedef __hip_internal::uint8_t uint8_t; typedef __hip_internal::uint16_t uint16_t;\n"
           "#if !defined(__HIP_DEVICE_COMPILE__)\n#error expected a device compilation (pt_math.h fast paths)\n#endif\n"
           "#include \"pt_trace.h\"\n" +
           flat_mask_source(leaves, n, specular, tri_fast, albedo_x2, dark, emit) +
           "extern \"C\" __global__ __launch_bounds__(256, PT_WAVES) void pt_trace_flat_rtc(pt::TraceArgs A) {\n"
           "    pt::trace_body_flat<pt::SceneBoxMask>(A);\n}\n";
}

namespace {

std::vector<std::string> rtc_flags() {
    std::vector<std::string> flags = {"--offload-arch=gfx950", "-O3", "-std=c++17", "-ffp-contract=off",
                                      "-fno-fast-math", "-fhip-fp32-correctly-rounded-divide-sqrt",
                                      "-fno-gpu-flush-denormals-to-zero", "-fno-slp-vectorize",
                                      "-mllvm", "-disable-machine-licm", "-mllvm", "-amdgpu-use-amdgpu-trackers"};
#ifdef PT_STAMPS
    flags.push_back("-DPT_STAMPS");
#endif
    for (const std::string& f : rtc_extra_flags()) flags.push_back(f);
    return flags;
}

std::atomic<int64_t> g_rtc_disk_hits{0}, g_rtc_disk_rejects{0}, g_rtc_compiles{0};
std::atomic<int64_t> g_rtc_last_compile_us{0}, g_rtc_server_compiles{0};
constexpr char kRtcMagic[8] = {'P', 'T', 'R', 'T', 'C', '0', '0', '1'};

std::string rtc_cache_dir() {
    const char* off = getenv("PT_RTC_CACHE");
    if (off && *off == '0') return "";
    const char* d = getenv("PT_RTC_CACHE_DIR");
    if (d && *d) return d;
    const char* x = getenv("XDG_CACHE_HOME");
    if (x && *x) return std::string(x) + "/pathtracer-amd/rtc";
    const char* h = getenv("HOME");
    if (h && *h) return std::string(h) + "/.cache/pathtracer-amd/rtc";
    return "";
}

std::string lib_of(const void* addr) {
    Dl_info di;
    return dladdr(addr, &di) && di.dli_fname ? std::string(di.dli_fname) : std::string();
}

std::vector<std::string> rtc_compiler_libs(bool runtime) {
    std::vector<std::string> libs;
    if (void* h = dlopen("libamd_comgr.so.3", RTLD_NOW | RTLD_NOLOAD)) {
        struct link_map* lm = nullptr;
        if (dlinfo(h, RTLD_DI_LINKMAP, &lm) == 0 && lm && lm->l_name && *lm->l_name) libs.push_back(lm->l_name);
        dlclose(h);
    }
    const std::string rtc = lib_of(reinterpret_cast<const void*>(&hiprtcCompileProgram));
    if (!rtc.empty()) libs.push_back(rtc);
    if (runtime) {
        const std::string hip = lib_of(reinterpret_cast<const void*>(&hipModuleLoadData));
        if (!hip.empty()) libs.push_back(hip);
    }
    return libs;
}

std::string rtc_key(const std::string& src) {
    Sha256 k;
    k.update("pathtracer-amd hipRTC code object v1");
    k.update(src.c_str(), src.size() + 1);
    for (const char* h : {pt_rtc_src_trace, pt_rtc_src_math, pt_rtc_src_stack, pt_rtc_src_hip}) k.update(h, strlen(h) + 1);
    for (const std::string& f : rtc_flags()) k.update(f.c_str(), f.size() + 1);
    int maj = 0, mnr = 0;
    (void)hiprtcVersion(&maj, &mnr);
    k.update(std::to_string(maj) + "." + std::to_string(mnr));
    k.update(std::to_string(HIP_VERSION) + " " + HIP_VERSION_GITHASH);
    for (const std::string& lib : rtc_compiler_libs(true)) {
        struct stat st;
        const bool ok = stat(lib.c_str(), &st) == 0;
        k.update(lib + " " + (ok ? std::to_string((long long)st.st_size) + " " + std::to_string((long long)st.st_mtime) : "?"));
    }
    return k.hex();
}

bool rtc_dir_private(const std::string& dir) {
    struct stat st;
    return stat(dir.c_str(), &st) == 0 && S_ISDIR(st.st_mode) && st.st_uid == geteuid() &&
           !(st.st_mode & (S_IWGRP | S_IWOTH));
}

bool rtc_disk_load(const std::string& key, std::vector<char>& code) {
    const std::string dir = rtc_cache_dir();
    if (dir.empty()) return false;
    if (!rtc_dir_private(dir)) {
        g_rtc_disk_rejects++;
        return false;
    }
    const std::string path = dir + "/" + key + ".co";
    const int fd = open(path.c_str(), O_RDONLY | O_NOFOLLOW | O_CLOEXEC);
    if (fd < 0) {
        if (errno == ELOOP) g_rtc_disk_rejects++;
        return false;
    }
    struct stat st;
    if (fstat(fd, &st) != 0 || st.st_uid != geteuid() || (st.st_mode & (S_IWGRP | S_IWOTH)) || !S_ISREG(st.st_mode)) {
        close(fd);
        g_rtc_disk_rejects++;
        return false;
    }
    auto rd = [fd](void* p, size_t n) {
        char* c = static_cast<char*>(p);
        while (n > 0) {
            const ssize_t r = read(fd, c, n);
            if (r <= 0) return false;
            c += r;
            n -= (size_t)r;
        }
        return true;
    };
    char magic[8], kh[64];
    uint64_t size = 0;
    uint8_t sum[32], got[32];
    bool ok = rd(magic, 8) && memcmp(magic, kRtcMagic, 8) == 0 && rd(kh, 64) && memcmp(kh, key.data(), 64) == 0 &&
              rd(&size, 8) && size > 0 && size < ((uint64_t)1 << 30) && (uint64_t)st.st_size == 112 + size &&
              rd(sum, 32);
    if (ok) {
        code.resize(size);
        ok = rd(code.data(), size);
    }
    close(fd);
    if (ok) {
        Sha256 p;
        p.update(code.data(), code.size());
        p.digest(got);
        ok = memcmp(got, sum, 32) == 0;
    }
    if (!ok) {
        code.clear();
        g_rtc_disk_rejects++;
        return false;
    }
    g_rtc_disk_hits++;
    return true;
}

void rtc_disk_store(const std::string& key, const std::vector<char>& code) {
    const std::string dir = rtc_cache_dir();
    if (dir.empty() || code.empty()) return;
    for (size_t i = 1; i <= dir.size(); i++)
        if (i == dir.size() || dir[i] == '/') (void)mkdir(dir.substr(0, i).c_str(), 0700);
    if (!rtc_dir_private(dir)) return;
    std::ostringstream tn;
    tn << dir << "/" << key << ".co.tmp." << getpid() << "." << std::this_thread::get_id();
    const std::string tmp = tn.str();
    {
        const int fd = open(tmp.c_str(), O_WRONLY | O_CREAT | O_EXCL, 0600);
        if (fd < 0) return;
        close(fd);
        std::ofstream f(tmp, std::ios::binary | std::ios::trunc);
        if (!f) return;
        uint8_t sum[32];
        Sha256 p;
        p.update(code.data(), code.size());
        p.digest(sum);
        const uint64_t size = code.size();
        f.write(kRtcMagic, 8);
        f.write(key.data(), 64);
        f.write(reinterpret_cast<const char*>(&size), 8);
        f.write(reinterpret_cast<const char*>(sum), 32);
        f.write(code.data(), (std::streamsize)code.size());
        if (!f) {
            f.close();
            (void)unlink(tmp.c_str());
            return;
        }
    }
    if (rename(tmp.c_str(), (dir + "/" + key + ".co").c_str()) != 0) (void)unlink(tmp.c_str());
}

struct RtcServer {
    std::mutex mu;
    pid_t pid = -1;
    int fd = -1;
    bool broken = false;
};
RtcServer& rtc_server() {
    static RtcServer* s = new RtcServer();
    return *s;
}

std::string rtc_server_path() {
    if (hook_off("PT_RTC_SERVER")) return "";
    std::string p = lib_of(reinterpret_cast<const void*>(&rtc_server_path));
    const size_t k = p.rfind('/');
    if (k == std::string::npos) return "";
    p = p.substr(0, k) + "/../bin/pt_rtc_server";
    return access(p.c_str(), X_OK) == 0 ? p : "";
}

bool rtc_server_start(RtcServer& s) {
    const std::string path = rtc_server_path();
    if (path.empty()) return false;
    int sv[2];
    if (socketpair(AF_UNIX, SOCK_STREAM | SOCK_CLOEXEC, 0, sv) != 0) return false;
    std::vector<std::string> args{path};
    for (const std::string& lib : rtc_compiler_libs(false)) args.insert(args.end(), {"--lib", lib});
    std::vector<char*> argv;
    for (std::string& a : args) argv.push_back(&a[0]);
    argv.push_back(nullptr);
    posix_spawn_file_actions_t fa;
    posix_spawnattr_t at;
    posix_spawn_file_actions_init(&fa);
    posix_spawn_file_actions_adddup2(&fa, sv[1], 0);
    posix_spawn_file_actions_adddup2(&fa, sv[1], 1);
    posix_spawn_file_actions_addclosefrom_np(&fa, 3);
    posix_spawnattr_init(&at);
    sigset_t none, dflt;
    sigemptyset(&none);
    sigemptyset(&dflt);
    sigaddset(&dflt, SIGPIPE);
    posix_spawnattr_setsigmask(&at, &none);
    posix_spawnattr_setsigdefault(&at, &dflt);
    posix_spawnattr_setflags(&at, POSIX_SPAWN_SETSIGMASK | POSIX_SPAWN_SETSIGDEF);
    pid_t pid = -1;
    const int rc = posix_spawn(&pid, path.c_str(), &fa, &at, argv.data(), environ);
    posix_spawn_file_actions_destroy(&fa);
    posix_spawnattr_destroy(&at);
    close(sv[1]);
    if (rc != 0) {
        close(sv[0]);
        return false;
    }
    s.pid = pid;
    s.fd = sv[0];
    return true;
}

void rtc_server_stop(RtcServer& s) {
    if (s.fd >= 0) close(s.fd);
    if (s.pid > 0) {
        kill(s.pid, SIGKILL);
        (void)waitpid(s.pid, nullptr, 0);
    }
    s.fd = -1;
    s.pid = -1;
    s.broken = true;
}

bool rtc_server_compile(const std::string& src, RtcCode& out) {
    RtcServer& s = rtc_server();
    std::lock_guard<std::mutex> lock(s.mu);
    if (s.broken) return false;
    if (s.fd < 0 && !rtc_server_start(s)) {
        s.broken = true;
        return false;
    }
    const int fd = s.fd;
    auto put = [fd](const void* p, size_t n) {
        const char* c = static_cast<const char*>(p);
        while (n > 0) {
            const ssize_t r = send(fd, c, n, MSG_NOSIGNAL);
            if (r <= 0) return false;
            c += r;
            n -= (size_t)r;
        }
        return true;
    };
    auto get = [fd](void* p, size_t n) {
        char* c = static_cast<char*>(p);
        while (n > 0) {
            const ssize_t r = recv(fd, c, n, 0);
            if (r <= 0) return false;
            c += r;
            n -= (size_t)r;
        }
        return true;
    };
    auto put_str = [&put](const char* str, size_t n) {
        const uint64_t len = n;
        return put(&len, 8) && put(str, n);
    };
    const char* hdrs[] = {pt_rtc_src_trace, pt_rtc_src_math, pt_rtc_src_stack, pt_rtc_src_hip};
    const char* names[] = {"pt_trace.h", "pt_math.h", "pt_raystack.h", "pt_hip.h"};
    const std::vector<std::string> flags = rtc_flags();
    const uint32_t head[3] = {0x51525450u , 4u, (uint32_t)flags.size()};
    bool ok = put(head, 12) && put_str(src.data(), src.size());
    for (int i = 0; ok && i < 4; i++) ok = put_str(names[i], strlen(names[i])) && put_str(hdrs[i], strlen(hdrs[i]));
    for (size_t i = 0; ok && i < flags.size(); i++) ok = put_str(flags[i].data(), flags[i].size());
    uint32_t resp[2] = {0, 0};
    uint64_t n = 0;
    ok = ok && get(resp, 8) && resp[0] == 0x53525450u  && get(&n, 8) && n < ((uint64_t)1 << 30);
    std::vector<char> bytes;
    if (ok) {
        bytes.resize(n);
        ok = n == 0 || get(bytes.data(), n);
    }
    if (!ok) {
        rtc_server_stop(s);
        return false;
    }
    if (resp[1] == 1) {
        out.code = std::move(bytes);
    } else {
        out.status = "hipRTC compile failed: " + std::string(bytes.begin(), bytes.begin() + std::min<size_t>(bytes.size(), 400));
    }
    return true;
}

std::shared_ptr<const RtcCode> rtc_compile(const std::string& src, const std::string& key) {
    auto out = std::make_shared<RtcCode>();
    g_rtc_compiles++;
    const auto t0 = std::chrono::steady_clock::now();
    auto done = [&t0]() {
        g_rtc_last_compile_us =
            std::chrono::duration_cast<std::chrono::microseconds>(std::chrono::steady_clock::now() - t0).count();
    };
    if (rtc_server_compile(src, *out)) {
        done();
        g_rtc_server_compiles++;
        if (!out->code.empty()) rtc_disk_store(key, out->code);
        return out;
    }
    const char* hdrs[] = {pt_rtc_src_trace, pt_rtc_src_math, pt_rtc_src_stack, pt_rtc_src_hip};
    const char* names[] = {"pt_trace.h", "pt_math.h", "pt_raystack.h", "pt_hip.h"};
    hiprtcProgram prog;
    if (hiprtcCreateProgram(&prog, src.c_str(), "pt_trace_flat_rtc.hip", 4, hdrs, names) != HIPRTC_SUCCESS) {
        out->status = "hiprtcCreateProgram failed";
        return out;
    }
    const std::vector<std::string> flags = rtc_flags();
    std::vector<const char*> opts;
    for (const std::string& f : flags) opts.push_back(f.c_str());
    if (hiprtcCompileProgram(prog, (int)opts.size(), opts.data()) != HIPRTC_SUCCESS) {
        size_t ls = 0;
        hiprtcGetProgramLogSize(prog, &ls);
        std::string log(ls, '\0');
        if (ls) hiprtcGetProgramLog(prog, &log[0]);
        out->status = "hipRTC compile failed: " + log.substr(0, 400);
    } else {
        size_t cs = 0;
        hiprtcGetCodeSize(prog, &cs);
        out->code.resize(cs);
        hiprtcGetCode(prog, out->code.data());
        done();
        rtc_disk_store(key, out->code);
    }
    hiprtcDestroyProgram(&prog);
    return out;
}

}

int rtc_wait_all() {
    std::vector<RtcFuture> jobs;
    {
        RtcCache& c = rtc_cache();
        std::lock_guard<std::mutex> lock(c.mu);
        for (auto& kv : c.code) jobs.push_back(kv.second);
    }
    int running = 0;
    for (RtcFuture& f : jobs) {
        if (!f.valid()) continue;
        const std::future_status st = f.wait_for(std::chrono::seconds(0));
        if (st == std::future_status::deferred) continue;
        if (st != std::future_status::ready) running++;
        f.wait();
    }
    return running;
}

bool rtc_async_ready() {
    static const bool ok = [] {
        if (rtc_server_path().empty()) {
            void* h = dlopen("libamd_comgr.so.3", RTLD_NOW | RTLD_GLOBAL);
            if (!h) h = dlopen("libamd_comgr.so", RTLD_NOW | RTLD_GLOBAL);
            if (!h) return false;
        }
        std::atexit([] { (void)rtc_wait_all(); });
        return true;
    }();
    return ok;
}

RtcFuture rtc_job(const std::string& src) {
    RtcCache& cache = rtc_cache();
    const bool async = rtc_async_ready();
    std::lock_guard<std::mutex> lock(cache.mu);
    auto it = cache.code.find(src);
    if (it != cache.code.end()) return it->second;
    const std::string key = rtc_key(src);
    RtcFuture f;
    auto disk = std::make_shared<RtcCode>();
    if (!cache.refused.count(key) && rtc_disk_load(key, disk->code)) {
        disk->disk_key = key;
        std::promise<std::shared_ptr<const RtcCode>> p;
        p.set_value(disk);
        f = p.get_future().share();
    } else {
        f = async ? std::async(std::launch::async, rtc_compile, src, key).share()
                  : std::async(std::launch::deferred, rtc_compile, src, key).share();
    }
    cache.code.emplace(src, f);
    return f;
}

hipFunction_t rtc_load(int device, const std::string& src, const RtcCode& code, std::string& status) {
    if (code.code.empty()) {
        status = code.status;
        return nullptr;
    }
    RtcCache& cache = rtc_cache();
    std::lock_guard<std::mutex> lock(cache.mu);
    auto fit = cache.funcs.find({device, src});
    if (fit != cache.funcs.end()) return fit->second;
    hipModule_t mod;
    hipFunction_t fn;
    if (hipModuleLoadData(&mod, code.code.data()) != hipSuccess ||
        hipModuleGetFunction(&fn, mod, "pt_trace_flat_rtc") != hipSuccess) {
        status = "hipModuleLoadData/GetFunction failed";
        if (!code.disk_key.empty()) {
            const std::string dir = rtc_cache_dir();
            if (!dir.empty()) (void)unlink((dir + "/" + code.disk_key + ".co").c_str());
            g_rtc_disk_rejects++;
            cache.code.erase(src);
            cache.refused.insert(code.disk_key);
            status = "evicted";
        }
        return nullptr;
    }
    cache.funcs[{device, src}] = fn;
    status.clear();
    return fn;
}

}

using namespace pt;

extern "C" {

int pt_rtc_check(const pt_scene* scene, char* src_out, size_t cap) {
    PackedScene ps;
    const int rc = pack_scene(scene, ps);
    if (rc) return rc;
    if (!flat_eligible(ps))
        return set_error(PT_E_ARG, "scene has no flat leaf list (%d leaves, %d triangles)", ps.num_leaves, ps.num_tris);
    const std::string src =
        rtc_flat_source(ps.leaves, ps.num_leaves, scene_has_specular(ps), ps.coords_small, albedo_x2_ok(ps), scene_dark(ps),
                        scene_emit_box(ps, scene_dark(ps)));
    if (src_out && cap) {
        const size_t n = std::min(cap - 1, src.size());
        memcpy(src_out, src.data(), n);
        src_out[n] = 0;
    }
    const std::shared_ptr<const RtcCode> code = rtc_job(src).get();
    if (code->code.empty()) return set_error(PT_E_HIP, "%s", code->status.c_str());
    return (int)code->code.size();
}

int pt_debug_rtc_start(const pt_scene* scene) {
    PackedScene ps;
    const int rc = pack_scene(scene, ps);
    if (rc) return rc;
    if (!flat_eligible(ps))
        return set_error(PT_E_ARG, "scene has no flat leaf list (%d leaves, %d triangles)", ps.num_leaves, ps.num_tris);
    const RtcFuture f = rtc_job(
        rtc_flat_source(ps.leaves, ps.num_leaves, scene_has_specular(ps), ps.coords_small, albedo_x2_ok(ps), scene_dark(ps),
                        scene_emit_box(ps, scene_dark(ps))));
    return f.wait_for(std::chrono::seconds(0)) == std::future_status::ready ? 0 : 1;
}

int64_t pt_debug_rtc_cache(int32_t op) {
    if (op == 0) {
        RtcCache& c = rtc_cache();
        std::lock_guard<std::mutex> lock(c.mu);
        for (auto& kv : c.code) kv.second.wait();
        c.code.clear();
        c.funcs.clear();
        return 0;
    }
    if (op == 1) return g_rtc_disk_hits.load();
    if (op == 2) return g_rtc_disk_rejects.load();
    if (op == 3) return g_rtc_compiles.load();
    if (op == 4) return g_rtc_last_compile_us.load();
    if (op == 5) return g_rtc_server_compiles.load();
    return set_error(PT_E_ARG, "pt_debug_rtc_cache: bad op %d", op);
}

}
```

pathtracer-cpp_amd/csrc/pt_trace.h:

```cpp
#pragma once

#include "pt_hip.h"
#include "pt_math.h"
#include "pt_raystack.h"

namespace pt {

constexpr int kBlock = 256;
constexpr int kWave = 64;
static_assert(kRaySlots == kWave, "one prefetched camera ray per lane (pt_raystack.h)");
constexpr int kMaxSpecularIters = 1 << 16;
#ifndef PT_CHUNK
#define PT_CHUNK 1024
#endif
constexpr int kChunk = PT_CHUNK;
static_assert(kChunk >= kWave, "a work-pool refill must cover one claim of every lane of a wave");
constexpr int kMaxFlatLeaves = 64;

#ifndef PT_WAVES
#define PT_WAVES 7
#endif

#ifdef PT_STAMPS
#define PT_STAMP(v)                                  \
    __builtin_amdgcn_sched_barrier(0);               \
    const uint64_t v = __builtin_amdgcn_s_memtime(); \
    __builtin_amdgcn_sched_barrier(0);
#define PT_STAMP_ADD(i, a, b) stamp_acc[i] += (b) - (a);
#elif defined(PT_MARKS)
#define PT_STAMP(v)                       \
    __builtin_amdgcn_sched_barrier(0);    \
    asm volatile("; @mark " #v);          \
    __builtin_amdgcn_sched_barrier(0);
#define PT_STAMP_ADD(i, a, b)
#else
#define PT_STAMP(v)
#define PT_STAMP_ADD(i, a, b)
#endif
constexpr int kStampSections = 23;

#ifndef PT_PK_PLANES
#define PT_PK_PLANES 0
#endif
#ifndef PT_PRIO_PAIRS
#define PT_PRIO_PAIRS 1
#endif
#ifndef PT_PRIO_MASK
#define PT_PRIO_MASK 0
#endif
#ifndef PT_PRIO_FOLD
#define PT_PRIO_FOLD 0
#endif
#ifndef PT_PRIO_SHADE
#define PT_PRIO_SHADE 0
#endif
#ifndef PT_PRIO_DRAIN
#define PT_PRIO_DRAIN 2
#endif
#ifndef PT_PRIO_STEP
#define PT_PRIO_STEP 0
#endif
#ifndef PT_WIDE_THR_SCALE
#define PT_WIDE_THR_SCALE 1
#endif
#ifndef PT_WIDE_ADDC
#define PT_WIDE_ADDC 1
#endif
#ifndef PT_WIDE_FAST_M
#define PT_WIDE_FAST_M 1
#endif
#ifndef PT_ADDC_MASK
#define PT_ADDC_MASK 1
#endif
#ifndef PT_SIGN_MASK
#define PT_SIGN_MASK 1
#endif
__device__ __forceinline__ bool bounded_ray(v3 o, v3 inv) {
    const float ri = __builtin_fmaxf(__builtin_fmaxf(__builtin_fabsf(inv.x), __builtin_fabsf(inv.y)), __builtin_fabsf(inv.z));
    const float ro = __builtin_fmaxf(__builtin_fmaxf(__builtin_fabsf(o.x), __builtin_fabsf(o.y)), __builtin_fabsf(o.z));
    return ri <= 0x1p60f && ro < 0x1p60f;
}
__device__ __forceinline__ uint32_t shl1_add_sign(uint32_t fail, uint32_t f) {
    return __builtin_amdgcn_alignbit(fail, f, 31u);
}
__device__ __forceinline__ uint32_t box_fail_bits(float tmin3, float tmax) {
    return __float_as_uint(tmax - tmin3) | __float_as_uint(tmax);
}
#ifndef PT_SHARED_CLAMP
#define PT_SHARED_CLAMP 1
#endif
#ifndef PT_MULTI_LEAF_OR
#define PT_MULTI_LEAF_OR 0
#endif

typedef float f2v __attribute__((ext_vector_type(2)));

__device__ __forceinline__ uint32_t shl1_add_bit(uint32_t x, unsigned long long m) {
    uint32_t r;
    unsigned long long c;
    asm("v_addc_co_u32_e64 %0, %1, %2, %2, %3" : "=v"(r), "=s"(c) : "v"(x), "s"(m));
    return r;
}

__device__ __forceinline__ uint32_t dbl_u32(uint32_t x) {
    uint32_t r;
    asm("v_add_u32_e32 %0, %1, %1" : "=v"(r) : "v"(x));
    return r;
}

__device__ __forceinline__ uint32_t or_if_bit(uint32_t x, uint32_t pattern, unsigned long long m) {
    uint32_t t, r;
    asm("v_cndmask_b32_e64 %0, 0, %1, %2" : "=v"(t) : "v"(pattern), "s"(m));
    asm("v_or_b32_e32 %0, %1, %2" : "=v"(r) : "v"(t), "v"(x));
    return r;
}

struct FlatLeaves {
    float box[kMaxFlatLeaves][6];
    unsigned long long bits[kMaxFlatLeaves];
};

struct FastDiv {
    uint32_t d, m, sh1, sh2;
};

__device__ __forceinline__ uint32_t fdiv(uint32_t n, FastDiv f) {
    const uint32_t t = __umulhi(f.m, n);
    return (t + ((n - t) >> f.sh1)) >> f.sh2;
}

struct TraceArgs {
    const float4* __restrict__ nodes;
    const float4* __restrict__ tris;
    const float4* __restrict__ mats;
    const float4* __restrict__ leaves;
    const uint4* __restrict__ wide;
    const float4* __restrict__ wtris;
    const float4* __restrict__ nrm;
    const float4* __restrict__ umats;
    float* __restrict__ radiance;
    unsigned long long* __restrict__ ctr;
    unsigned long long* __restrict__ work;
    unsigned long long* stamps;
    unsigned long long total_items;
    float pos_x, pos_y, pos_z;
    float col0_x, col0_y, col0_z;
    float col1_x, col1_y, col1_z;
    float col2_x, col2_y, col2_z;
    float half_vres_x, half_vres_y, cell;
    float cz_col0, cz_col1, cz_col2;
    int W, npix;
    int part_index, part_count, band_rows;
    int depth;
    uint32_t seed;
    int s_begin, s_count, per_item;
    int stack_size;
    int rec_size;
    int num_node4, num_tri4, num_mat4;
    int num_umat4;
    int num_leaves;
    int num_boxes_padded;
    int force_exact_slab;
    int wide_thresh;
    int chunk;
    uint32_t static_items;
    unsigned long long static_base;
    int pair_queue;
    int regen_thresh;
    int wide_queue;
    int wide_rows;
    int wide_top;
    uint32_t wide_nodes;
    float wide_span_x, wide_span_y, wide_span_z;
    int wide_single;
    int wide_compact;
    int tri_fast;
    int* __restrict__ exact_stack;
    int exact_rows;
    const float* __restrict__ acc_src;
    float* __restrict__ acc_sum;
    int acc_count, acc_first, acc_chunks, acc_every;
    FastDiv div_npix, div_w, div_band;
    const float2* __restrict__ theta_tab;
    int theta_lanes;
    int dark;
    int emit_on;
    float emit_lo_x, emit_lo_y, emit_lo_z, emit_hi_x, emit_hi_y, emit_hi_z;
    uint32_t* __restrict__ flags;
    int flags_pm;
    const uint32_t* __restrict__ acc_flags;
    int ray_reserve;
    FlatLeaves flat;
};

__device__ __forceinline__ int part_row(const TraceArgs& A, int r) {
    const int k = (int)fdiv((uint32_t)r, A.div_band), i = r - k * A.band_rows;
    return (k * A.part_count + A.part_index) * A.band_rows + i;
}

__device__ __forceinline__ const __attribute__((address_space(4))) TraceArgs* kernarg_args() {
    const __attribute__((address_space(4))) TraceArgs* K =
        (const __attribute__((address_space(4))) TraceArgs*)__builtin_amdgcn_kernarg_segment_ptr();
    asm volatile("" : "+s"(K));
    return K;
}

struct NoEmitReject {
    static constexpr bool kCompiled = false;
    __device__ __forceinline__ static bool on() { return false; }
    __device__ __forceinline__ static bool rejected(v3, v3) { return false; }
};
struct KernargEmitReject {
    static constexpr bool kCompiled = true;
    __device__ __forceinline__ static bool on() { return kernarg_args()->emit_on != 0; }
    __device__ __forceinline__ static bool rejected(v3 o, v3 d) {
        const auto* K = kernarg_args();
        return emit_reject(v3{K->emit_lo_x, K->emit_lo_y, K->emit_lo_z}, v3{K->emit_hi_x, K->emit_hi_y, K->emit_hi_z}, o,
                           d);
    }
};

constexpr int kEmitSlab = 1, kEmitSignOnly = 2, kEmitSlabEmpty = 3;
#ifndef PT_EMIT_SIGN_ONLY
#define PT_EMIT_SIGN_ONLY 0
#endif
struct KernargEmitSlabReject : KernargEmitReject {
    static constexpr bool kSlab = true;
    __device__ __forceinline__ static bool rejected_slab(v3 o, v3, v3 inv) {
        const auto* K = kernarg_args();
        const int mode = K->emit_on;
        if (mode == kEmitSlabEmpty) return true;
        return emit_slab_reject_nonempty(v3{K->emit_lo_x, K->emit_lo_y, K->emit_lo_z},
                                         v3{K->emit_hi_x, K->emit_hi_y, K->emit_hi_z}, o, inv, mode == kEmitSignOnly);
    }
};
template <typename Rej, typename = void>
struct RejSlab {
    static constexpr bool value = false;
};
template <typename Rej>
struct RejSlab<Rej, decltype((void)Rej::kSlab)> {
    static constexpr bool value = Rej::kCompiled && Rej::kSlab;
};

struct NodeBox {
    v3 lb, rt;
    int a, b;
};

__device__ __forceinline__ NodeBox load_node(const float4* __restrict__ nodes, int n) {
    const float4 p = nodes[2 * n], q = nodes[2 * n + 1];
    return NodeBox{v3{p.x, p.y, p.z}, v3{p.w, q.x, q.y}, __float_as_int(q.z), __float_as_int(q.w)};
}

template <bool kFiniteInv>
__device__ __forceinline__ bool box_hit(v3 lb, v3 rt, v3 o, v3 inv) {
    return kFiniteInv ? slab_hit_finite(lb, rt, o, inv) : slab_hit(lb, rt, o, inv);
}

template <bool kFiniteInv, typename NodePtr, typename TriPtr>
__device__ __forceinline__ int intersect_tree(NodePtr nodes, TriPtr tris, int* __restrict__ stk, int tid, v3 o,
                                              v3 d, v3 inv, float& t_out) {
    int hit = -1;
    float t = 1e30f;
    int sp = 0;
    const NodeBox root = load_node(nodes, 0);
    int ca = root.a, cb = root.b;
    bool go = box_hit<kFiniteInv>(root.lb, root.rt, o, inv);
    while (go) {
        if (ca >= 0) {
            const NodeBox L = load_node(nodes, ca);
            const NodeBox R = load_node(nodes, ca + 1);
            const bool hl = box_hit<kFiniteInv>(L.lb, L.rt, o, inv);
            const bool hr = box_hit<kFiniteInv>(R.lb, R.rt, o, inv);
            if (hr) {
                if (hl) {
                    stk[sp * kBlock + tid] = ca;
                    sp++;
                }
                ca = R.a;
                cb = R.b;
                continue;
            }
            if (hl) {
                ca = L.a;
                cb = L.b;
                continue;
            }
        } else {
            for (int i = -ca - 1; i <= cb; i++) {
                const float4 t0 = tris[3 * i], t1 = tris[3 * i + 1], t2 = tris[3 * i + 2];
                float tt;
                if (tri_hit(v3{t0.x, t0.y, t0.z}, v3{t0.w, t1.x, t1.y}, v3{t1.z, t1.w, t2.x}, o, d, tt) && tt < t) {
                    t = tt;
                    hit = i;
                }
            }
        }
        if (sp == 0) break;
        sp--;
        const float4 q = nodes[2 * stk[sp * kBlock + tid] + 1];
        ca = __float_as_int(q.z);
        cb = __float_as_int(q.w);
    }
    t_out = t;
    return hit;
}

struct TableBoxMask {
    static constexpr bool kMask32 = false;
    static constexpr bool kSingleTri = false;
    static constexpr bool kSpecular = true;
    static constexpr bool kTriFast = false;
    static constexpr bool kSignMask = false;
    static constexpr bool kAlbedoX2 = false;
    static constexpr bool kDarkKnown = false;
    static constexpr bool kBoxPairs = false;
    static constexpr bool kCamInvGen = false;
    static constexpr bool kRayStack = true;
    static constexpr int kBoxes = 0;
    static constexpr uint16_t kBoxTab[1] = {0};
    static constexpr bool kDark = false;
    using EmitRej = KernargEmitSlabReject;
    __device__ __forceinline__ static unsigned long long mask(const TraceArgs& A, v3 o, v3 inv) {
        const float(*box)[6] = A.flat.box;
        unsigned long long m = 0;
        const int n = A.num_boxes_padded;
        for (int k = 0; k < n; k += 4) {
#pragma unroll
            for (int j = 0; j < 4; j++) {
                const float* b = box[k + j];
                if (slab_hit_finite(v3{b[0], b[1], b[2]}, v3{b[3], b[4], b[5]}, o, inv)) m |= A.flat.bits[k + j];
            }
        }
        return m;
    }
};

template <bool kSpec, bool kM32>
struct FastTableMask : TableBoxMask {
    static constexpr bool kMask32 = kM32;
    static constexpr bool kSingleTri = true;
    static constexpr bool kSpecular = kSpec;
    static constexpr bool kTriFast = true;
    static constexpr bool kAlbedoX2 = true;
    static constexpr bool kDarkKnown = true;
    static constexpr bool kDark = true;
    static constexpr bool kCamInvGen = kSpec;
    static constexpr bool kRayStack = false;
};

template <typename Mask>
struct PerLaneRays : Mask {
    static constexpr bool kRayStack = false;
};

template <typename TriPtr, typename LeafPtr>
__device__ __forceinline__ int flat_tri_loop(unsigned long long mask, LeafPtr lleaves, TriPtr tris, v3 o, v3 d,
                                             float& t_out) {
    int hit = -1;
    float t = 1e30f;
    while (mask) {
        const int k = __builtin_ctzll(mask);
        mask &= mask - 1;
        const float4 b = lleaves[2 * k + 1];
        const int last = __float_as_int(b.w);
        for (int i = __float_as_int(b.z); i <= last; i++) {
            const float4 t0 = tris[3 * i], t1 = tris[3 * i + 1], t2 = tris[3 * i + 2];
            float tt;
            if (tri_hit(v3{t0.x, t0.y, t0.z}, v3{t0.w, t1.x, t1.y}, v3{t1.z, t1.w, t2.x}, o, d, tt) && tt < t) {
                t = tt;
                hit = i;
            }
        }
    }
    t_out = t;
    return hit;
}

__device__ __forceinline__ int flat_box_loop(unsigned long long mask, const uint16_t* __restrict__ boxtab,
                                             const float4* __restrict__ tris, v3 o, v3 d, float& t_out) {
    int hit = -1;
    float t = 1e30f;
    while (mask) {
        const int u = __builtin_ctzll(mask);
        mask &= mask - 1;
        const uint32_t code = boxtab[u];
        for (int j = 0; j < 2; j++) {
            const uint32_t r = j ? code >> 8 : code & 0xffu;
            if (r == 0xffu) continue;
            const int i = (int)r;
            const float4 t0 = tris[3 * i], t1 = tris[3 * i + 1], t2 = tris[3 * i + 2];
            float tt;
            if (tri_hit(v3{t0.x, t0.y, t0.z}, v3{t0.w, t1.x, t1.y}, v3{t1.z, t1.w, t2.x}, o, d, tt) &&
                (tt < t || (tt == t && i < hit))) {
                t = tt;
                hit = i;
            }
        }
    }
    t_out = t;
    return hit;
}

template <typename BoxMask, typename TriPtr, typename LeafPtr>
__device__ __forceinline__ int intersect_flat(const TraceArgs& A, LeafPtr lleaves, TriPtr tris, v3 o, v3 d, v3 inv,
                                              float& t_out, const uint16_t* __restrict__ boxtab) {
    if constexpr (BoxMask::kBoxPairs) return flat_box_loop(BoxMask::mask(A, o, inv), boxtab, tris, o, d, t_out);
    return flat_tri_loop(BoxMask::mask(A, o, inv), lleaves, tris, o, d, t_out);
}

__device__ __forceinline__ uint32_t wave_incl_scan(uint32_t x) {
    x += (uint32_t)__builtin_amdgcn_update_dpp(0, (int)x, 0x111, 0xf, 0xf, false);
    x += (uint32_t)__builtin_amdgcn_update_dpp(0, (int)x, 0x112, 0xf, 0xf, false);
    x += (uint32_t)__builtin_amdgcn_update_dpp(0, (int)x, 0x114, 0xf, 0xf, false);
    x += (uint32_t)__builtin_amdgcn_update_dpp(0, (int)x, 0x118, 0xf, 0xf, false);
    x += (uint32_t)__builtin_amdgcn_update_dpp(0, (int)x, 0x142, 0xa, 0xf, false);
    x += (uint32_t)__builtin_amdgcn_update_dpp(0, (int)x, 0x143, 0xc, 0xf, false);
    return x;
}

__device__ __forceinline__ void wave_lds_sync() {
    __builtin_amdgcn_fence(__ATOMIC_RELEASE, "wavefront");
    __builtin_amdgcn_wave_barrier();
    __builtin_amdgcn_fence(__ATOMIC_ACQUIRE, "wavefront");
}

__device__ __forceinline__ float lane_float(int addr, float v) {
    return __int_as_float(__builtin_amdgcn_ds_bpermute(addr, __float_as_int(v)));
}

template <typename BoxMask, typename TriPtr, typename LeafPtr>
__device__ __forceinline__ int intersect_flat_pairs(const TraceArgs& A, unsigned long long mask, LeafPtr lleaves,
                                                    TriPtr tris, uint16_t* __restrict__ queue,
                                                    unsigned long long* __restrict__ best, int tid, int lane, v3 o,
                                                    v3 d, float& t_out, const uint16_t* __restrict__ boxtab) {
    const uint32_t c = (uint32_t)__popcll(mask);
    const uint32_t incl = wave_incl_scan(c);
    const uint32_t total = (uint32_t)__builtin_amdgcn_readlane((int)incl, 63);
    if (total > (uint32_t)A.pair_queue) {
        if constexpr (BoxMask::kBoxPairs) return flat_box_loop(mask, boxtab, tris, o, d, t_out);
        return flat_tri_loop(mask, lleaves, tris, o, d, t_out);
    }
    best[tid] = ~0ull;
    uint16_t* at = queue + (incl - c);
    uint32_t tag = (uint32_t)lane << 6;
    asm volatile("" : "+v"(tag));
    if constexpr (BoxMask::kMask32) {
        uint32_t m = (uint32_t)mask;
        while (m) {
            const uint32_t b0 = (uint32_t)__builtin_ctz(m);
            m &= m - 1;
            at[0] = (uint16_t)(tag | b0);
            if (m) {
                at[1] = (uint16_t)(tag | (uint32_t)__builtin_ctz(m));
                m &= m - 1;
            }
            at += 2;
        }
    } else {
        while (mask) {
            const uint32_t b0 = (uint32_t)__builtin_ctzll(mask);
            mask &= mask - 1;
            at[0] = (uint16_t)(tag | b0);
            if (mask) {
                at[1] = (uint16_t)(tag | (uint32_t)__builtin_ctzll(mask));
                mask &= mask - 1;
            }
            at += 2;
        }
    }
    wave_lds_sync();
    unsigned long long* wbest = best + (tid - lane);
    for (uint32_t base = 0; base < total; base += kWave) {
        const uint32_t p = base + (uint32_t)lane;
        const uint32_t e = p < total ? (uint32_t)queue[p] : 0u;
        const int owner = (int)(e >> 6), leaf = (int)(e & 63u);
        const int addr = owner << 2;
        const v3 ro{lane_float(addr, o.x), lane_float(addr, o.y), lane_float(addr, o.z)};
        const v3 rd{lane_float(addr, d.x), lane_float(addr, d.y), lane_float(addr, d.z)};
        if (BoxMask::kBoxPairs && p < total) {
            const uint32_t code = boxtab[leaf];
#pragma unroll
            for (int j = 0; j < 2; j++) {
                const uint32_t r = j ? code >> 8 : code & 0xffu;
                if (j == 0 || r != 0xffu) {
                    const int i = (int)r;
                    const float4 t0 = tris[3 * i], t1 = tris[3 * i + 1], t2 = tris[3 * i + 2];
                    const v3 v1{t0.x, t0.y, t0.z}, e1{t0.w, t1.x, t1.y}, e2{t1.z, t1.w, t2.x};
                    float tt;
                    const bool h = BoxMask::kTriFast ? tri_hit_nb(v1, e1, e2, ro, rd, tt) : tri_hit(v1, e1, e2, ro, rd, tt);
                    if (h && tt < 1e30f)
                        atomicMin(wbest + owner, ((unsigned long long)__float_as_uint(tt) << 32) | (uint32_t)i);
                }
            }
        } else if (p < total) {
            int first = leaf, last = leaf;
            if constexpr (!BoxMask::kSingleTri) {
                const float4 b = lleaves[2 * leaf + 1];
                first = __float_as_int(b.z);
                last = __float_as_int(b.w);
            }
            for (int i = first; i <= last; i++) {
                const float4 t0 = tris[3 * i], t1 = tris[3 * i + 1], t2 = tris[3 * i + 2];
                const v3 v1{t0.x, t0.y, t0.z}, e1{t0.w, t1.x, t1.y}, e2{t1.z, t1.w, t2.x};
                float tt;
                const bool h = BoxMask::kTriFast ? tri_hit_nb(v1, e1, e2, ro, rd, tt) : tri_hit(v1, e1, e2, ro, rd, tt);
#ifdef PT_EXP_DUP_PAIR
                {
                    v3 o2 = ro;
                    asm volatile("" : "+v"(o2.x));
                    float t2;
                    const bool h2 = BoxMask::kTriFast ? tri_hit_nb(v1, e1, e2, o2, rd, t2) : tri_hit(v1, e1, e2, o2, rd, t2);
                    asm volatile("" ::"v"(t2), "v"((int)h2));
                }
#endif
                if (h && tt < 1e30f)
                    atomicMin(wbest + owner, ((unsigned long long)__float_as_uint(tt) << 32) | (uint32_t)i);
            }
        }
    }
    wave_lds_sync();
    const unsigned long long kb = best[tid];
    if ((uint32_t)kb == 0xffffffffu) {
        t_out = 1e30f;
        return -1;
    }
    t_out = __uint_as_float((uint32_t)(kb >> 32));
    return (int)(uint32_t)kb;
}

#ifndef PT_THETA_TAB
#define PT_THETA_TAB 2
#endif

#ifndef PT_FLAT_ONLY
template <int W, int kPF = 1>
constexpr int kNodeU4 = kPF == 2 ? 1 + 3 * W / 2 : W == 8 ? 8 : 5;

__device__ __forceinline__ uint32_t lane_sel(uint32_t a, uint32_t b, unsigned long long m) {
    uint32_t r;
    asm volatile("v_cndmask_b32_e64 %0, %1, %2, %3" : "=v"(r) : "v"(a), "v"(b), "s"(m));
    return r;
}

template <int W, bool kF16>
struct WideNode {
    static constexpr int kWords = kF16 ? W / 2 : W / 4;
    uint4 h0, h1;
    uint32_t en[3][kWords], ex[3][kWords];
};

template <int W, bool kF16>
struct WideOff {
    uint32_t en[3], ex[3];
};

#ifndef PT_WIDE_EXIT_SUB
#define PT_WIDE_EXIT_SUB 1
#endif
template <int W>
__device__ __forceinline__ constexpr uint32_t wide_exit_c(int a) { return PT_WIDE_EXIT_SUB ? 32u + 4u * W * a : 0u; }
template <int W, bool kF16>
__device__ __forceinline__ WideOff<W, kF16> wide_offsets(uint32_t nb, const unsigned long long (&neg)[3]) {
    WideOff<W, kF16> f;
    const uint32_t nb2 = nb + 2u * W;
#if PT_WIDE_EXIT_SUB
    const uint32_t both = nb + nb2;
#endif
#pragma unroll
    for (int a = 0; a < 3; a++) {
        if constexpr (kF16) {
#if PT_WIDE_EXIT_SUB
            const uint32_t e = lane_sel(nb, nb2, neg[a]);
            f.en[a] = e + (32u + 4u * W * a);
            f.ex[a] = both - e;
#else
            f.en[a] = lane_sel(nb, nb2, neg[a]) + (32u + 4u * W * a);
            f.ex[a] = lane_sel(nb2, nb, neg[a]) + (32u + 4u * W * a);
#endif
        } else {
            f.en[a] = lane_sel(nb, nb2, neg[a]) + (32u + 4u * W * a);
            f.ex[a] = 0u;
        }
    }
    return f;
}

template <int W, bool kF16>
__device__ __forceinline__ WideNode<W, kF16> load_wide_node_lds(const char* __restrict__ base, uint32_t nb,
                                                                const WideOff<W, kF16>& off) {
    WideNode<W, kF16> n;
    n.h0 = *reinterpret_cast<const uint4*>(base + nb);
// ... 680 lines not shown
        float3 v[kDense];
#pragma unroll
        for (int j = 0; j < kDense; j++) v[j] = slab_at(src, (size_t)(s + j), q, npix);
#pragma unroll
        for (int j = 0; j < kDense; j++) {
            acc.add(v[j]);
        }
    }
    for (; s < n; s++) {
        const float3 v = slab_at(src, (size_t)s, q, npix);
        acc.add(v);
    }
}

struct SumF32 {
    float &x, &y, &z;
    __device__ __forceinline__ void add(const float3 v) {
        x += v.x;
        y += v.y;
        z += v.z;
    }
};
template <bool kParallel = false>
__device__ __forceinline__ void slab_sum(const float* __restrict__ src, const uint32_t* __restrict__ flags, int pm,
                                         int n, uint32_t q, uint32_t npix, float& x, float& y, float& z) {
    SumF32 acc{x, y, z};
    slab_walk<kParallel>(src, flags, pm, n, q, npix, acc);
}

__device__ __forceinline__ bool fused_accumulate_chunk(int lane) {
#ifdef PT_EXP_NO_ACC
    return false;
#endif
    const auto* K = kernarg_args();
    unsigned long long c = 0;
    if (lane == 0) c = atomicAdd(K->ctr + 2, 1ull);
    c = __builtin_amdgcn_readfirstlane((uint32_t)c);
    if (c >= (unsigned long long)K->acc_chunks) return false;
    const uint32_t npix = (uint32_t)K->npix, q = (uint32_t)c * kWave + (uint32_t)lane;
    if (q < npix) {
        float* __restrict__ sum = K->acc_sum;
        const float* __restrict__ src = K->acc_src;
        const int n = K->acc_count;
        float x = 0.0f, y = 0.0f, z = 0.0f;
        if (!K->acc_first) {
            x = sum[q];
            y = sum[npix + q];
            z = sum[2 * (size_t)npix + q];
        }
        slab_sum(src, K->acc_flags, K->flags_pm, n, q, npix, x, y, z);
        sum[q] = x;
        sum[npix + q] = y;
        sum[2 * (size_t)npix + q] = z;
    }
    return true;
}

__device__ __forceinline__ void after_refill(const TraceArgs& A, int lane, Pool& pool) {
    if (A.acc_chunks > 0 && --pool.acc_left == 0) {
        pool.acc_left = (uint32_t)A.acc_every;
        fused_accumulate_chunk(lane);
    }
}

__device__ __forceinline__ void drain_accumulate(const TraceArgs& A, int lane) {
    if (A.acc_chunks > 0)
        while (fused_accumulate_chunk(lane)) {
        }
}

__device__ __forceinline__ void claim_work(const TraceArgs& A, int lane, bool need, Pool& pool, bool& alive, int& q,
                                           int& s, int& s_end) {
    const unsigned long long want = __ballot(need);
    if (want == 0ull) return;
    const uint32_t cnt = (uint32_t)__popcll(want);
    const uint32_t avail = pool.end - pool.next;
    uint32_t fresh = 0;
    if (avail < cnt) {
        unsigned long long b = 0;
        if (lane == 0) b = atomicAdd(A.work, (unsigned long long)A.chunk);
        fresh = (uint32_t)A.static_base + __builtin_amdgcn_readfirstlane((uint32_t)b);
    }
    if (need) {
        const uint32_t rank =
            __builtin_amdgcn_mbcnt_hi((uint32_t)(want >> 32), __builtin_amdgcn_mbcnt_lo((uint32_t)want, 0u));
        const uint32_t item = rank < avail ? pool.next + rank : fresh + (rank - avail);
        if (item >= (uint32_t)A.total_items) {
            alive = false;
        } else {
            const uint32_t blk = fdiv(item, A.div_npix);
            q = (int)(item - blk * (uint32_t)A.npix);
            s = A.s_begin + (int)blk * A.per_item;
            s_end = min(s + A.per_item, A.s_begin + A.s_count);
        }
    }
    if (avail < cnt) {
        pool.next = fresh + (cnt - avail);
        pool.end = fresh + (uint32_t)A.chunk;
        after_refill(A, lane, pool);
    } else {
        pool.next += cnt;
    }
}

__device__ __forceinline__ void claim_item(const TraceArgs& A, int lane, bool need, Pool& pool, bool& alive,
                                           uint32_t& item_out) {
    const unsigned long long want = __ballot(need);
    if (want == 0ull) return;
    const uint32_t cnt = (uint32_t)__popcll(want);
    const uint32_t avail = pool.end - pool.next;
    uint32_t fresh = 0;
    if (avail < cnt) {
        unsigned long long b = 0;
        if (lane == 0) b = atomicAdd(A.work, (unsigned long long)A.chunk);
        fresh = (uint32_t)A.static_base + __builtin_amdgcn_readfirstlane((uint32_t)b);
    }
    if (need) {
        const uint32_t rank =
            __builtin_amdgcn_mbcnt_hi((uint32_t)(want >> 32), __builtin_amdgcn_mbcnt_lo((uint32_t)want, 0u));
        const uint32_t item = rank < avail ? pool.next + rank : fresh + (rank - avail);
        if (item >= (uint32_t)A.total_items) alive = false;
        else item_out = item;
    }
    if (avail < cnt) {
        pool.next = fresh + (cnt - avail);
        pool.end = fresh + (uint32_t)A.chunk;
        after_refill(A, lane, pool);
    } else {
        pool.next += cnt;
    }
}

#ifndef PT_CAM_KERNARG
#define PT_CAM_KERNARG 1
#endif
__device__ __forceinline__ void camera_ray(const TraceArgs& A, int q, int s, Lcg& g, v3& o, v3& d) {
    const auto* K = PT_CAM_KERNARG ? kernarg_args() : nullptr;
    const TraceArgs& C = PT_CAM_KERNARG ? *(const TraceArgs*)K : A;
    const int r = (int)fdiv((uint32_t)q, C.div_w);
    const int px = q - r * C.W;
    const int py = part_row(C, r);
    g.s = pt_sample_seed((uint32_t)(py * C.W + px), (uint32_t)s, C.seed);
    const float jy = g.next01();
    const float jx = g.next01();
    const float cx = ((float)px + jx) * C.cell - C.half_vres_x;
    const float cy = ((float)py + jy) * C.cell - C.half_vres_y;
    d = normalize_fast(v3{cx * C.col0_x + cy * C.col0_y + C.cz_col0, cx * C.col1_x + cy * C.col1_y + C.cz_col1,
                     cx * C.col2_x + cy * C.col2_y + C.cz_col2});
    o = v3{C.pos_x, C.pos_y, C.pos_z};
}

constexpr int kShadeGo = 0, kShadeEnd = 1, kShadeEndEarly = 2;

template <bool kSpecular = true, typename RecT = int, bool kIds = false, typename Rej = NoEmitReject>
__device__ __forceinline__ int shade_inv(const TraceArgs& A, const float4* __restrict__ mats,
                                          const float4* __restrict__ tris, RecT* __restrict__ rec_tri,
                                          float* __restrict__ rec_cos, int tid, int hit, float t, Lcg& g, v3& o,
                                          v3& d, v3& inv, int& k, v3& L) {
    L = v3{0.0f, 0.0f, 0.0f};
    if (hit < 0) return kShadeEnd;
#ifdef PT_EXP_DUP_SHADE
    {
        int h2 = hit;
        asm volatile("" : "+v"(h2));
        const float4 tn2 = kIds ? tris[h2] : tris[3 * h2 + 2];
        const int row2 = kIds ? __float_as_int(tn2.w) : h2;
        const float4 m02 = mats[2 * row2], m12 = mats[2 * row2 + 1];
        v3 n2 = kIds ? v3{tn2.x, tn2.y, tn2.z} : v3{tn2.y, tn2.z, tn2.w};
        if (!(dot(n2, d) < 0.0f)) n2 = neg(n2);
        const v3 hp2 = add(o, scale(d, t));
        asm volatile("" ::"v"(m02.x), "v"(m12.x), "v"(hp2.x), "v"(hp2.y), "v"(hp2.z), "v"(n2.x), "v"(n2.y), "v"(n2.z));
    }
#endif
    float4 tn;
    int row = hit;
    if constexpr (kIds) {
        tn = tris[hit];
        row = __float_as_int(tn.w);
    }
    const float4 m0 = mats[2 * row], m1 = mats[2 * row + 1];
    const int type = __float_as_int(m0.x);
    if (type == PT_MAT_EMIT) {
        L = v3{m1.x, m1.y, m1.z};
        return kShadeEnd;
    }
    const int depth = A.depth;
    if (k + 1 >= depth) {
        L = v3{m1.x + 0.0f * m0.y, m1.y + 0.0f * m0.z, m1.z + 0.0f * m0.w};
        return kShadeEnd;
    }
    v3 n;
    if constexpr (kIds) {
        n = v3{tn.x, tn.y, tn.z};
    } else {
        tn = tris[3 * hit + 2];
        n = v3{tn.y, tn.z, tn.w};
    }
    if (!(dot(n, d) < 0.0f)) n = neg(n);
    const v3 hp = add(o, scale(d, t));
    v3 nd;
    if (kSpecular && type == PT_MAT_SPECULAR) {
        if (!specular_dir(g, d, n, m1.w, kMaxSpecularIters, nd)) atomicAdd(A.ctr + 3, 1ull);
#ifdef PT_EXP_DUP_SPEC
        {
            Lcg g2 = g;
            asm volatile("" : "+v"(g2.s));
            v3 x;
            specular_dir(g2, d, n, m1.w, kMaxSpecularIters, x);
            asm volatile("" ::"v"(x.x), "v"(x.y), "v"(x.z));
        }
#endif
    } else {
#ifdef PT_EXP_NO_BRDF
        nd = n;
#else
#if PT_THETA_TAB == 1
        nd = hemisphere_dir_tab(g, n, kernarg_args()->theta_tab);
#elif PT_THETA_TAB == 2
        if ((int)__popcll(__ballot(true)) <= kernarg_args()->theta_lanes)
            nd = hemisphere_dir_tab(g, n, kernarg_args()->theta_tab);
        else
            nd = hemisphere_dir(g, n);
#else
        nd = hemisphere_dir(g, n);
#endif
#ifdef PT_EXP_DUP_BRDF
        {
            Lcg g2 = g;
            asm volatile("" : "+v"(g2.s));
            const v3 x = hemisphere_dir(g2, n);
            asm volatile("" ::"v"(x.x), "v"(x.y), "v"(x.z));
        }
#endif
#endif
#if defined(PT_EXP_COHERENT_DIR) || defined(PT_EXP_OCTANT_DIR)
        {
            const v3 w = v3{__int_as_float(__builtin_amdgcn_readfirstlane(__float_as_int(nd.x))),
                            __int_as_float(__builtin_amdgcn_readfirstlane(__float_as_int(nd.y))),
                            __int_as_float(__builtin_amdgcn_readfirstlane(__float_as_int(nd.z)))};
#ifdef PT_EXP_COHERENT_DIR
            nd = dot(w, n) < 0.0f ? neg(w) : w;
#else
            const v3 c = v3{__builtin_copysignf(nd.x, w.x), __builtin_copysignf(nd.y, w.y), __builtin_copysignf(nd.z, w.z)};
            if (dot(c, n) >= 0.0f) nd = c;
#endif
        }
#endif
    }
    rec_tri[k * kBlock + tid] = (RecT)row;
    rec_cos[k * kBlock + tid] = dot(n, nd);
    o = add(hp, scale(n, 1e-4f));
    d = nd;
    if constexpr (RejSlab<Rej>::value) inv = rcp3_exact<!kSpecular>(d);
    if constexpr (Rej::kCompiled) {
        if (Rej::on()) {
            bool rej;
            if constexpr (RejSlab<Rej>::value) rej = Rej::rejected_slab(o, d, inv);
            else rej = Rej::rejected(o, d);
            const bool early = ((int)(k + 2 >= depth) & (int)rej) != 0;
            k += early ? 0 : 1;
            return early ? kShadeEndEarly : kShadeGo;
        }
    }
    k++;
    return kShadeGo;
}

template <bool kSpecular = true, typename RecT = int, bool kIds = false, typename Rej = NoEmitReject>
__device__ __forceinline__ int shade(const TraceArgs& A, const float4* __restrict__ mats,
                                      const float4* __restrict__ tris, RecT* __restrict__ rec_tri,
                                      float* __restrict__ rec_cos, int tid, int hit, float t, Lcg& g, v3& o, v3& d,
                                      int& k, v3& L) {
    static_assert(!RejSlab<Rej>::value, "a policy with the slab rule carries inv: shade_inv");
    v3 unused{0.0f, 0.0f, 0.0f};
    return shade_inv<kSpecular, RecT, kIds, Rej>(A, mats, tris, rec_tri, rec_cos, tid, hit, t, g, o, d, unused, k, L);
}

__device__ __forceinline__ uint32_t slab_index(const TraceArgs& A, int s, int q) {
    return (uint32_t)(s - A.s_begin) * (uint32_t)A.npix + (uint32_t)q;
}

#ifndef PT_DARK_SKIP
#define PT_DARK_SKIP 1
#endif
template <typename RecT, bool kAlbedoX2 = false, bool kDarkKnown = false, bool kDark = false>
__device__ __forceinline__ void finish_path(const TraceArgs& A, const float4* __restrict__ mats,
                                            const RecT* __restrict__ rec_tri, const float* __restrict__ rec_cos,
                                            int tid, int k, v3 L, uint32_t at) {
#ifdef PT_EXP_NO_FOLD
    k = 0;
#endif
    const bool unwind = !(PT_DARK_SKIP && (kDarkKnown ? kDark : kernarg_args()->dark != 0) &&
                          (__float_as_uint(L.x) | __float_as_uint(L.y) | __float_as_uint(L.z)) == 0u);
    if (unwind) {
#ifndef PT_FOLD_UNROLL
#define PT_FOLD_UNROLL 1
#endif
    if (PT_FOLD_UNROLL && kernarg_args()->rec_size <= 4) {
        int tj[4];
        float cj[4];
#pragma unroll
        for (int j = 0; j < 4; j++) {
            tj[j] = 0;
            cj[j] = 0.0f;
            if (j < k) {
                tj[j] = (int)rec_tri[j * kBlock + tid];
                cj[j] = rec_cos[j * kBlock + tid];
            }
        }
        float4 m0[4], m1[4];
#pragma unroll
        for (int j = 0; j < 4; j++)
            if (j < k) {
                m0[j] = mats[2 * tj[j]];
                m1[j] = mats[2 * tj[j] + 1];
            }
#pragma unroll
        for (int j = 3; j >= 0; j--)
            if (j < k) {
                if constexpr (kAlbedoX2)
                    L = v3{m1[j].x + (L.x * m0[j].y) * cj[j], m1[j].y + (L.y * m0[j].z) * cj[j],
                           m1[j].z + (L.z * m0[j].w) * cj[j]};
                else
                    L = v3{m1[j].x + ((2.0f * L.x) * m0[j].y) * cj[j], m1[j].y + ((2.0f * L.y) * m0[j].z) * cj[j],
                           m1[j].z + ((2.0f * L.z) * m0[j].w) * cj[j]};
            }
    } else {
        for (int j = k - 1; j >= 0; j--) {
            const int tj = (int)rec_tri[j * kBlock + tid];
            const float cj = rec_cos[j * kBlock + tid];
            const float4 m0 = mats[2 * tj], m1 = mats[2 * tj + 1];
            if constexpr (kAlbedoX2)
                L = v3{m1.x + (L.x * m0.y) * cj, m1.y + (L.y * m0.z) * cj, m1.z + (L.z * m0.w) * cj};
            else
                L = v3{m1.x + ((2.0f * L.x) * m0.y) * cj, m1.y + ((2.0f * L.y) * m0.z) * cj,
                       m1.z + ((2.0f * L.z) * m0.w) * cj};
        }
    }
    }
#ifdef PT_EXP_DUP_FOLD
    {
        v3 L2 = L;
        asm volatile("" : "+v"(L2.x));
        for (int j = k - 1; j >= 0; j--) {
            const int tj = (int)rec_tri[j * kBlock + tid];
            const float cj = rec_cos[j * kBlock + tid];
            const float4 m0 = mats[2 * tj], m1 = mats[2 * tj + 1];
            L2 = v3{m1.x + ((2.0f * L2.x) * m0.y) * cj, m1.y + ((2.0f * L2.y) * m0.z) * cj,
                    m1.z + ((2.0f * L2.z) * m0.w) * cj};
        }
        asm volatile("" ::"v"(L2.x), "v"(L2.y), "v"(L2.z));
    }
#endif
#ifdef PT_EXP_NO_STORE
    if (L.x == 12345.0f)
#endif
    uint32_t* fl = kernarg_args()->flags;
    if (unwind || !fl)
        *reinterpret_cast<float3*>(A.radiance + 3 * (size_t)at) = make_float3(L.x, L.y, L.z);
    if (unwind && fl) {
        if (kernarg_args()->flags_pm) {
            const uint32_t sm = fdiv(at, A.div_npix), q = at - sm * (uint32_t)A.npix;
            atomicOr(fl + flag_word(sm, q, (uint32_t)A.npix), 1u << (sm & 31u));
        } else {
            atomicOr(fl + (at >> 5), 1u << (at & 31u));
        }
    }
}

__device__ __forceinline__ void count_rays(const TraceArgs& A, int lane, uint32_t n_rays) {
    unsigned long long r = n_rays;
    for (int off = 32; off > 0; off >>= 1) r += __shfl_down(r, off);
    if (lane == 0) atomicAdd(A.ctr + 1, r);
}

__device__ __forceinline__ void count_rays_wave(const TraceArgs& A, int lane, unsigned long long n_rays) {
    if (lane == 0) atomicAdd(A.ctr + 1, n_rays);
}

#ifndef PT_COUNT_EARLY
#define PT_COUNT_EARLY 0
#endif
__device__ __forceinline__ void count_early_wave(const TraceArgs& A, int lane, unsigned long long n_early) {
    if (PT_COUNT_EARLY && lane == 0 && n_early) atomicAdd(A.ctr + 4, n_early);
}

#ifndef PT_FRESH_TID
#define PT_FRESH_TID 1
#endif
#ifndef PT_CAM_INV
#define PT_CAM_INV 2
#endif
#ifndef PT_RAY_STACK
#define PT_RAY_STACK 1
#endif
#ifndef PT_RAY_RESERVE
#define PT_RAY_RESERVE (-1)
#endif
__device__ __forceinline__ int fresh_tid() {
    int t = (int)threadIdx.x;
    if (PT_FRESH_TID) asm volatile("" : "+v"(t));
    return t;
}

struct FlatRecs {
    uint16_t* tri;
    float* cos;
};
__device__ __forceinline__ FlatRecs flat_records(float4* lds4) {
    const auto* K = kernarg_args();
    uint16_t* rt = reinterpret_cast<uint16_t*>(lds4 + K->num_tri4 + K->num_mat4) + (kBlock / kWave) * K->pair_queue;
    return FlatRecs{rt, reinterpret_cast<float*>(rt + K->rec_size * kBlock)};
}

template <typename BoxMask>
__device__ __forceinline__ void trace_body_flat(const TraceArgs& A) {
    extern __shared__ float4 lds4[];
    const int tid = threadIdx.x;
    const int lane = tid & (kWave - 1);
    float4* s_tris = lds4;
    float4* s_mats = s_tris + A.num_tri4;
    uint16_t* queues = reinterpret_cast<uint16_t*>(s_mats + A.num_mat4);
    uint16_t* rec_tri = queues + (kBlock / kWave) * A.pair_queue;
    float* rec_cos = reinterpret_cast<float*>(rec_tri + A.rec_size * kBlock);
    unsigned long long* best = reinterpret_cast<unsigned long long*>(rec_cos + A.rec_size * kBlock);
    float4* next_ray = reinterpret_cast<float4*>(best + kBlock);
    uint32_t* next_at = reinterpret_cast<uint32_t*>(next_ray + kBlock);
    uint16_t* boxtab = reinterpret_cast<uint16_t*>(next_at + kBlock);
    if constexpr (BoxMask::kBoxPairs)
        for (int i = tid; i < BoxMask::kBoxes; i += kBlock) boxtab[i] = BoxMask::kBoxTab[i];
    for (int i = tid; i < A.num_tri4; i += kBlock) s_tris[i] = A.tris[i];
    for (int i = tid; i < A.num_mat4; i += kBlock) {
        float4 m = A.mats[i];
        if (BoxMask::kAlbedoX2 && !(i & 1)) m = make_float4(m.x, 2.0f * m.y, 2.0f * m.z, 2.0f * m.w);
        s_mats[i] = m;
    }
    __syncthreads();
    const float4* __restrict__ mats = s_mats;
    const float4* __restrict__ tris = s_tris;
    uint16_t* wq = queues + __builtin_amdgcn_readfirstlane(tid >> 6) * A.pair_queue;
    int* xstk = A.exact_stack + (size_t)blockIdx.x * A.exact_rows * kBlock;

    bool alive = true;
    bool active = false;
    bool has_next = false;
    int count = 0;
    bool dry = false;
    uint32_t at = 0;
    Lcg g{0};
    v3 o{0, 0, 0}, d{0, 0, 0};
    constexpr bool kCarry = RejSlab<typename BoxMask::EmitRej>::value;
    v3 inv{0, 0, 0};
    constexpr bool kGenInv = kCarry && BoxMask::kCamInvGen;
    v3 next_inv{0, 0, 0};
    int k = 0;
    unsigned long long n_rays = 0;
    unsigned long long n_early = 0;
    Pool pool = pool_start(A);
#ifdef PT_STAMPS
    uint64_t stamp_acc[kStampSections] = {};
#endif

    while (true) {
        PT_STAMP(st_a)
        auto generate = [&](uint32_t item) {
            const uint32_t blk = fdiv(item, A.div_npix);
            Lcg gn{0};
            v3 on, nd;
            camera_ray(A, (int)(item - blk * (uint32_t)A.npix), A.s_begin + (int)blk, gn, on, nd);
#ifdef PT_EXP_DUP_CAMF
            {
                uint32_t it2 = item;
                asm volatile("" : "+v"(it2));
                Lcg g2{0};
                v3 o2, d2;
                camera_ray(A, (int)(it2 - blk * (uint32_t)A.npix), A.s_begin + (int)blk, g2, o2, d2);
                asm volatile("" ::"v"(d2.x), "v"(d2.y), "v"(d2.z), "v"(g2.s));
            }
#endif
            next_ray[fresh_tid()] = make_float4(nd.x, nd.y, nd.z, __uint_as_float(gn.s));
            next_at[fresh_tid()] = item;
            if constexpr (kGenInv) next_inv = rcp3_exact(nd);
        };
        if constexpr (BoxMask::kRayStack) {
            const unsigned long long need = __ballot(!active);
            const int n_need = (int)__popcll(need);
            if (ray_stack_generate(count, n_need, PT_RAY_RESERVE >= 0 ? PT_RAY_RESERVE : A.ray_reserve, dry)) {
                const bool want = lane >= count;
                bool got = true;
                uint32_t item = 0;
                claim_item(A, lane, want, pool, got, item);
                if (want && got) generate(item);
                const int n_got = (int)__popcll(__ballot(want && got));
#ifdef PT_STAMPS
                stamp_acc[11] += 1;
                stamp_acc[12] += (uint32_t)n_got;
#endif
                dry = ray_stack_dry(count, n_got);
                count = ray_stack_filled(count, n_got);
                wave_lds_sync();
            }
            if (n_need > 0 && count > 0) {
                const int rank = (int)__builtin_amdgcn_mbcnt_hi((uint32_t)(need >> 32),
                                                                __builtin_amdgcn_mbcnt_lo((uint32_t)need, 0u));
                const int slot = ray_stack_slot(count, rank);
                const bool take = !active && slot >= 0;
                v3 ti{0, 0, 0};
                if constexpr (kGenInv)
                    ti = v3{lane_float(slot << 2, next_inv.x), lane_float(slot << 2, next_inv.y),
                            lane_float(slot << 2, next_inv.z)};
                if (take) {
                    const int t0 = (fresh_tid() & ~(kWave - 1)) + slot;
                    const float4 nr = next_ray[t0];
                    at = next_at[t0];
                    g.s = __float_as_uint(nr.w);
                    d = v3{nr.x, nr.y, nr.z};
                    if constexpr (kGenInv) inv = ti;
                    else if constexpr (kCarry) inv = rcp3_exact(d);
                    o = v3{A.pos_x, A.pos_y, A.pos_z};
                    k = 0;
                    active = true;
                }
                count = ray_stack_taken(count, n_need);
            }
            if (ray_stack_done(__any(active), count, dry)) break;
        } else {
            const bool want = alive && !has_next;
            const int n_want = (int)__popcll(__ballot(want));
            if (n_want > 0 && (n_want >= A.regen_thresh || !__any(active || has_next))) {
                uint32_t item = 0;
                claim_item(A, lane, want, pool, alive, item);
                if (want && alive) {
                    generate(item);
                    has_next = true;
                }
#ifdef PT_STAMPS
                stamp_acc[11] += 1;
                stamp_acc[12] += (uint32_t)__popcll(__ballot(want && alive));
#endif
            }
            if (!active && has_next) {
                const int t0 = fresh_tid();
                const float4 nr = next_ray[t0];
                at = next_at[t0];
                g.s = __float_as_uint(nr.w);
                d = v3{nr.x, nr.y, nr.z};
                if constexpr (kGenInv) inv = next_inv;
                else if constexpr (kCarry) inv = rcp3_exact(d);
                o = v3{A.pos_x, A.pos_y, A.pos_z};
                k = 0;
                active = true;
                has_next = false;
            }
            if (!__any(active)) break;
        }
        PT_STAMP(st_b)

        float t = 0.0f;
        int hit = -1;
        const bool tr = active && A.depth > 0;
        if (A.depth > 0) n_rays += (unsigned long long)__popcll(__ballot(tr));
        if constexpr (!kCarry) inv = rcp3_exact(d, tr);
        const bool forced = A.force_exact_slab == 1 || (A.force_exact_slab == 2 && ((tid >> 6) & 1));
        const bool fast = !forced && __all(!tr || (BoxMask::kSignMask ? bounded_ray(o, inv) : all_finite(inv)));
        if (fast && A.pair_queue > 0) {
            if (PT_PRIO_MASK) __builtin_amdgcn_s_setprio(PT_PRIO_MASK);
            unsigned long long mask = BoxMask::mask(A, o, inv);
#ifdef PT_EXP_DUP_MASK
            {
                v3 o2 = o;
                asm volatile("" : "+v"(o2.x));
                const unsigned long long m2 = BoxMask::mask(A, o2, inv);
                asm volatile("" ::"v"((uint32_t)m2), "v"((uint32_t)(m2 >> 32)));
            }
#endif
            if (PT_PRIO_MASK) __builtin_amdgcn_s_setprio(0);
            if (!tr) mask = 0ull;
            PT_STAMP(st_b2)
            PT_STAMP_ADD(1, st_b, st_b2)
#ifdef PT_STAMPS
            {
                const uint32_t pc = (uint32_t)__popcll(mask);
                const uint32_t tot = (uint32_t)__builtin_amdgcn_readlane((int)wave_incl_scan(pc), 63);
                int mx = (int)pc;
                for (int off = 32; off > 0; off >>= 1) mx = max(mx, __shfl_xor(mx, off));
                stamp_acc[7] += 1;
                stamp_acc[8] += tot;
                stamp_acc[9] += (tot + 63) / 64;
                stamp_acc[10] += (uint32_t)mx;
            }
#endif
#ifdef PT_EXP_NO_PAIRS
            hit = mask ? __builtin_ctzll(mask) : -1;
            t = 1.0f;
#else
            if (PT_PRIO_PAIRS) __builtin_amdgcn_s_setprio(PT_PRIO_PAIRS);
            hit = intersect_flat_pairs<BoxMask>(A, mask, A.leaves, tris, wq, best, fresh_tid(), lane, o, d, t, boxtab);
            if (PT_PRIO_PAIRS) __builtin_amdgcn_s_setprio(0);
#endif
            PT_STAMP(st_b3)
            PT_STAMP_ADD(2, st_b2, st_b3)
        } else if (tr) {
            if (fast) hit = intersect_flat<BoxMask>(A, A.leaves, tris, o, d, inv, t, boxtab);
            else hit = intersect_tree<false>(A.nodes, tris, xstk, tid, o, d, inv, t);
        }
        PT_STAMP(st_c)

        int sh = kShadeGo;
        v3 L{0.0f, 0.0f, 0.0f};
        if (PT_PRIO_SHADE) __builtin_amdgcn_s_setprio(PT_PRIO_SHADE);
        if (active) {
            const FlatRecs R = flat_records(lds4);
            sh = shade_inv<BoxMask::kSpecular, uint16_t, false, typename BoxMask::EmitRej>(
                A, mats, tris, R.tri, R.cos, fresh_tid(), hit, t, g, o, d, inv, k, L);
        }
        if (PT_PRIO_SHADE) __builtin_amdgcn_s_setprio(0);
        const bool end = sh != kShadeGo;
        if constexpr (BoxMask::EmitRej::kCompiled) {
            const unsigned long long ne = (unsigned long long)__popcll(__ballot(sh == kShadeEndEarly));
            n_rays += ne;
            if (PT_COUNT_EARLY) n_early += ne;
        }
        PT_STAMP(st_d)
        if (end) {
            if (PT_PRIO_FOLD) __builtin_amdgcn_s_setprio(PT_PRIO_FOLD);
            const FlatRecs R = flat_records(lds4);
            finish_path<uint16_t, BoxMask::kAlbedoX2, BoxMask::kDarkKnown, BoxMask::kDark>(A, mats, R.tri, R.cos,
                                                                                        fresh_tid(), k, L, at);
            if (PT_PRIO_FOLD) __builtin_amdgcn_s_setprio(0);
            active = false;
        }
        PT_STAMP(st_e)
        PT_STAMP_ADD(0, st_a, st_b)
        PT_STAMP_ADD(5, st_b, st_c)
        PT_STAMP_ADD(3, st_c, st_d)
        PT_STAMP_ADD(4, st_d, st_e)
    }
#ifdef PT_STAMPS
    if (lane == 0 && A.stamps) {
        for (int i = 0; i < kStampSections; i++)
            if (i != 6) atomicAdd(A.stamps + i, (unsigned long long)stamp_acc[i]);
        atomicAdd(A.stamps + 6, 1ull);
    }
#endif
    drain_accumulate(A, lane);
    count_rays_wave(A, lane, n_rays);
    count_early_wave(A, lane, n_early);
}

#ifndef PT_FLAT_ONLY
template <bool kLdsScene>
__device__ __forceinline__ void trace_body(const TraceArgs& A) {
    extern __shared__ float4 lds4[];
    const int tid = threadIdx.x;
    const int lane = tid & (kWave - 1);
    const int scene4 = kLdsScene ? (A.num_node4 + A.num_tri4 + A.num_mat4) : 0;
    float4* s_nodes = lds4;
    float4* s_tris = lds4 + A.num_node4;
    float4* s_mats = s_tris + A.num_tri4;
    int* stk = reinterpret_cast<int*>(lds4 + scene4);
    int* rec_tri = stk + A.stack_size * kBlock;
    float* rec_cos = reinterpret_cast<float*>(rec_tri + A.rec_size * kBlock);
    if (kLdsScene) {
        for (int i = tid; i < A.num_node4; i += kBlock) s_nodes[i] = A.nodes[i];
        for (int i = tid; i < A.num_tri4; i += kBlock) s_tris[i] = A.tris[i];
        for (int i = tid; i < A.num_mat4; i += kBlock) s_mats[i] = A.mats[i];
        __syncthreads();
    }
    const float4* __restrict__ mats = kLdsScene ? s_mats : A.mats;
    const float4* __restrict__ tris = kLdsScene ? s_tris : A.tris;

    bool alive = true;
    bool active = false;
    bool has_next = false;
    int gq = 0, gs = 0, gs_end = 0;
    int q = 0, s = 0;
    uint32_t next_state = 0;
    v3 next_d{0, 0, 0};
    Lcg g{0};
    v3 o{0, 0, 0}, d{0, 0, 0};
    int k = 0;
    unsigned long long n_rays = 0;
    unsigned long long n_early = 0;
    Pool pool = pool_start(A);

    while (true) {
        const bool want = alive && !has_next;
        const int n_want = (int)__popcll(__ballot(want));
        if (n_want > 0 && (n_want >= A.regen_thresh || !__any(active || has_next))) {
            claim_work(A, lane, want && gs == gs_end, pool, alive, gq, gs, gs_end);
            if (want && alive) {
                Lcg gn{0};
                v3 on;
                camera_ray(A, gq, gs, gn, on, next_d);
                next_state = gn.s;
                gs++;
                has_next = true;
            }
        }
        if (!active && has_next) {
            q = gq;
            s = gs - 1;
            g.s = next_state;
            d = next_d;
            o = v3{A.pos_x, A.pos_y, A.pos_z};
            k = 0;
            active = true;
            has_next = false;
        }
        if (!__any(active)) break;

        float t = 0.0f;
        int hit = -1;
        const bool tr = active && A.depth > 0;
        if (A.depth > 0) n_rays += (unsigned long long)__popcll(__ballot(tr));
        const v3 inv = rcp3_exact(d, tr);
        const bool forced = A.force_exact_slab == 1 || (A.force_exact_slab == 2 && ((tid >> 6) & 1));
        const bool fast = !forced && __all(!tr || all_finite(inv));
        if (tr) {
            if (fast)
                hit = kLdsScene ? intersect_tree<true>(s_nodes, s_tris, stk, tid, o, d, inv, t)
                                : intersect_tree<true>(A.nodes, A.tris, stk, tid, o, d, inv, t);
            else
                hit = kLdsScene ? intersect_tree<false>(s_nodes, s_tris, stk, tid, o, d, inv, t)
                                : intersect_tree<false>(A.nodes, A.tris, stk, tid, o, d, inv, t);
        }
        int sh = kShadeGo;
        v3 L{0.0f, 0.0f, 0.0f};
        if (active)
            sh = shade<true, int, false, KernargEmitReject>(A, mats, tris, rec_tri, rec_cos, tid, hit, t, g, o, d, k, L);
        {
            const unsigned long long ne = (unsigned long long)__popcll(__ballot(sh == kShadeEndEarly));
            n_rays += ne;
            if (PT_COUNT_EARLY) n_early += ne;
        }
        if (sh != kShadeGo) {
            finish_path(A, mats, rec_tri, rec_cos, tid, k, L, slab_index(A, s, q));
            active = false;
        }
    }
    drain_accumulate(A, lane);
    count_rays_wave(A, lane, n_rays);
    count_early_wave(A, lane, n_early);
}

template <bool B, typename T, typename F>
struct PickT {
    using type = T;
};
template <typename T, typename F>
struct PickT<false, T, F> {
    using type = F;
};

template <int W, int kPF, bool kLdsMats>
__device__ __forceinline__ void trace_body_wide(const TraceArgs& A) {
    extern __shared__ float4 lds4[];
    constexpr int NU = kNodeU4<W, kPF>;
    const int tid = threadIdx.x;
    const int lane = tid & (kWave - 1);
    float4* s_mats = lds4;
    uint4* top = reinterpret_cast<uint4*>(s_mats + (kLdsMats ? A.num_umat4 : 0));
    int* stk = reinterpret_cast<int*>(top + A.wide_top * NU);
    unsigned long long* best = reinterpret_cast<unsigned long long*>(stk + A.wide_rows * kBlock);
    using RecW = typename PickT<kLdsMats, uint8_t, int>::type;
    float* rec_cos = reinterpret_cast<float*>(best + kBlock);
    RecW* rec_tri = reinterpret_cast<RecW*>(rec_cos + A.rec_size * kBlock);
    uint32_t* queues = reinterpret_cast<uint32_t*>(rec_tri + A.rec_size * kBlock);
    const int qwords = A.wide_single ? 1 : 2;
    for (int i = tid; i < A.wide_top * NU; i += kBlock) top[i] = A.wide[i];
    if constexpr (kLdsMats)
        for (int i = tid; i < A.num_umat4; i += kBlock) s_mats[i] = A.umats[i];
    __syncthreads();
    const float4* __restrict__ mats = kLdsMats ? s_mats : A.umats;
    const float4* __restrict__ nrm = A.nrm;
    unsigned long long* wbest = best + __builtin_amdgcn_readfirstlane(tid - lane);
    uint32_t* wq = queues + __builtin_amdgcn_readfirstlane(tid >> 6) * A.wide_queue * qwords;

    bool alive = true;
    bool active = false;
    bool trav = false;
// ... 214 lines not shown
```

Before: 81190.

## Bake scene constants and fixed LDS layout into the runtime-compiled flat kernel

Scene-dependent values (triangle and material counts, box table size, pair-queue use, theta lanes) become compile-time constants in the hipRTC-generated flat trace kernel. The LDS layout is reordered so the fixed-size regions sit first, which lets the compiler fold offsets and drop kernarg loads. The plan recompiles the RTC kernel when the baked constants no longer match the runtime plan. This aims to cut scalar loads and address arithmetic in the hot loop, at the cost of possible extra recompiles and more template plumbing.

```diff
diff --git a/include/pt_hip_debug.h b/include/pt_hip_debug.h
--- a/include/pt_hip_debug.h
+++ b/include/pt_hip_debug.h
@@ -28,6 +28,7 @@
 int pt_debug_emit_box(const pt_scene* scene, float out[6]);
 int pt_debug_ctx_emit_reject(const pt_ctx* ctx, int32_t* on, float box[6], uint64_t* early);
 int pt_debug_ray_stack(int32_t which, int32_t count, int32_t n, int32_t reserve, int32_t flag);
+int pt_debug_flat_lds(int32_t num_tris, int32_t box_tab_bytes, int32_t pair_queue, int32_t rec_size, uint32_t out[10]);
 int64_t pt_debug_counter(int32_t which);
 
 #ifdef __cplusplus
diff --git a/pathtracer-cpp_amd/csrc/pt_flatlds.h b/pathtracer-cpp_amd/csrc/pt_flatlds.h
--- /dev/null
+++ b/pathtracer-cpp_amd/csrc/pt_flatlds.h
@@ -0,0 +1,41 @@
+#pragma once
+
+#if defined(__HIPCC__)
+#define PT_FL_HD __host__ __device__ __forceinline__
+#else
+#define PT_FL_HD inline
+#endif
+
+namespace pt {
+
+constexpr unsigned kFlatLdsBlock = 256, kFlatLdsWaves = 4;
+
+struct FlatLds {
+    unsigned tris, mats, next_ray, best, next_at, boxtab;
+    unsigned queues, rec_tri, rec_cos;
+    unsigned bytes;
+};
+
+PT_FL_HD constexpr unsigned flat_box_tab_bytes(unsigned boxes) { return (2u * boxes + 3u) & ~3u; }
+
+PT_FL_HD constexpr unsigned flat_lds_fixed(unsigned num_tri4, unsigned num_mat4, unsigned box_tab_bytes) {
+    return (16u * (num_tri4 + num_mat4) + (16u + 8u + 4u) * kFlatLdsBlock + box_tab_bytes + 7u) & ~7u;
+}
+
+PT_FL_HD constexpr FlatLds flat_lds_layout(unsigned num_tri4, unsigned num_mat4, unsigned box_tab_bytes, unsigned pair_queue,
+                                           unsigned rec_size) {
+    FlatLds l{};
+    l.tris = 0u;
+    l.mats = 16u * num_tri4;
+    l.next_ray = l.mats + 16u * num_mat4;
+    l.best = l.next_ray + 16u * kFlatLdsBlock;
+    l.next_at = l.best + 8u * kFlatLdsBlock;
+    l.boxtab = l.next_at + 4u * kFlatLdsBlock;
+    l.queues = flat_lds_fixed(num_tri4, num_mat4, box_tab_bytes);
+    l.rec_tri = l.queues + 2u * kFlatLdsWaves * pair_queue;
+    l.rec_cos = l.rec_tri + 2u * kFlatLdsBlock * rec_size;
+    l.bytes = l.rec_cos + 4u * kFlatLdsBlock * rec_size;
+    return l;
+}
+
+}
diff --git a/pathtracer-cpp_amd/csrc/pt_kernel.hip b/pathtracer-cpp_amd/csrc/pt_kernel.hip
--- a/pathtracer-cpp_amd/csrc/pt_kernel.hip
+++ b/pathtracer-cpp_amd/csrc/pt_kernel.hip
@@ -402,6 +402,7 @@
     hipFunction_t rtc_flat = nullptr;
     std::string rtc_status;
     std::string rtc_src;
+    RtcBaked rtc_baked;
     RtcFuture rtc_job;
     int64_t last_plan[24] = {};
 };
@@ -536,6 +537,8 @@
     bool use_rtc = false;
     bool may_switch = false;
     int rtc_switch_at = -1;
+    int theta_lanes = 0;
+    const float2* theta_tab = nullptr;
     int blocks_per_cu = 1;
 };
 
@@ -586,14 +589,13 @@
 }
 
 size_t flat_lds_bytes(const pt_ctx* c, const RenderPlan& P, int queue) {
-    return sizeof(float4) * (size_t)(3 + 2) * c->meta.num_tris + sizeof(uint16_t) * (size_t)queue * (kBlock / kWave) +
-           (sizeof(uint16_t) + sizeof(float)) * (size_t)kBlock * P.rec + sizeof(unsigned long long) * kBlock +
-           (sizeof(float4) + sizeof(uint32_t)) * kBlock + P.box_tab_bytes;
+    return flat_lds_layout(3u * (unsigned)c->meta.num_tris, 2u * (unsigned)c->meta.num_tris, (unsigned)P.box_tab_bytes,
+                           (unsigned)queue, (unsigned)P.rec).bytes;
 }
 
 void plan_flat(const pt_ctx* c, RenderPlan& P) {
     P.pairs = !hook_off("PT_PAIRS");
-    P.box_tab_bytes = (sizeof(uint16_t) * (size_t)c->flat_boxes + 3) & ~(size_t)3;
+    P.box_tab_bytes = (size_t)rtc_baked(c->meta.num_tris, c->has_specular, c->flat_boxes).box_tab_bytes;
     int queue = P.pairs ? 512 : 0;
     const char* pq = hook_env("PT_PAIR_QUEUE");
     if (P.pairs && pq && *pq) {
@@ -646,6 +648,8 @@
     P.lds_scene = scene <= lds_scene_budget() && scene + work <= 64 * 1024;
     P.lds_bytes = work + (P.lds_scene ? scene : 0);
 }
+
+int theta_choice(pt_ctx* c, int* lanes, const float2** tab);
 
 int plan_render(pt_ctx* c, const PartShape& shape, const pt_params* prm, int s_lo, int spp, bool moments, RenderPlan& P) {
     P.shape = shape;
@@ -670,6 +674,20 @@
     const bool rtc_switch = !hook_off("PT_RTC_SWITCH");
     P.rtc_switch_at = hook_int("PT_RTC_SWITCH_AT", -1);
     if (P.flat && c->rtc_job.valid()) rtc_resolve(c, !rtc_switch && (double)shape.npix * (spp - s_lo) >= kRtcWaitPaths);
+    if ((rc = theta_choice(c, &P.theta_lanes, &P.theta_tab))) return rc;
+    if (P.flat && c->rtc_requested) {
+        RtcBaked want = rtc_baked(c->meta.num_tris, c->has_specular, c->flat_boxes);
+        want.theta_lanes = P.theta_lanes;
+        want.pairs = P.pairs;
+        if (!c->rtc_baked.runs(want)) {
+            c->rtc_flat = nullptr;
+            c->rtc_baked = want;
+            c->rtc_src = rtc_flat_source(c->flat_host, c->meta.num_leaves, c->has_specular, c->meta.coords_small, c->albedo_x2,
+                                         c->dark, c->emit, want);
+            c->rtc_job = rtc_job(c->rtc_src);
+            c->rtc_status = "compiling";
+        }
+    }
     P.kern = P.flat        ? (c->flat_fast                    ? (TraceKernel)c->flat_fast
                               : ray_stack_on(c->has_specular) ? pt_trace_kernel<true, true>
                                                               : pt_trace_kernel<true, true, 0, kWideByte, false>)
@@ -704,7 +722,7 @@
     *lanes = 0;
     *tab = nullptr;
 #if PT_THETA_TAB
-    *lanes = hook_int("PT_THETA_LANES", c->has_specular ? 32 : 0);
+    *lanes = theta_lanes_wanted(c->has_specular);
     if (PT_THETA_TAB == 1 || *lanes > 0) {
         if (int rc = theta_table(c, tab)) {
             if (PT_THETA_TAB == 1) return rc;
@@ -755,9 +773,8 @@
         A.flat = c->flat_tab;
     }
     A.radiance = c->d_radiance;
-    const float2* theta_tab = nullptr;
-    if (int rc = theta_choice(c, &A.theta_lanes, &theta_tab)) return rc;
-    A.theta_tab = theta_tab;
+    A.theta_lanes = P.theta_lanes;
+    A.theta_tab = P.theta_tab;
     A.work = c->d_ctr;
     A.ctr = c->d_ctr;
     A.dark = c->dark ? 1 : 0;
@@ -1265,8 +1282,10 @@
     const bool want_rtc = flat_eligible(ps) && !hook_off("PT_RTC");
     std::string src;
     RtcFuture job;
+    RtcBaked baked;
     if (want_rtc) {
-        src = rtc_flat_source(ps.leaves, ps.num_leaves, specular, ps.coords_small, albedo_x2, dark, emit);
+        baked = rtc_baked(ps.num_tris, specular, flat_box_pairs(ps.leaves, ps.num_leaves));
+        src = rtc_flat_source(ps.leaves, ps.num_leaves, specular, ps.coords_small, albedo_x2, dark, emit, baked);
         job = rtc_job(src);
     }
     if ((rc = ctx_ready(c))) return rc;
@@ -1341,6 +1360,7 @@
     c->rtc_status = "not a flat scene";
     if (want_rtc) {
         c->rtc_src = std::move(src);
+        c->rtc_baked = baked;
         c->albedo_x2 = albedo_x2;
         c->rtc_requested = true;
         c->flat_boxes = flat_box_pairs(c->flat_host, ps.num_leaves);
@@ -2550,6 +2570,16 @@
     return set_error(PT_E_ARG, "pt_debug_ray_stack: which = %d", which);
 }
 
+int pt_debug_flat_lds(int32_t num_tris, int32_t box_tab_bytes, int32_t pair_queue, int32_t rec_size, uint32_t out[10]) {
+    if (!out || num_tris < 0 || box_tab_bytes < 0 || pair_queue < 0 || rec_size < 0)
+        return set_error(PT_E_ARG, "pt_debug_flat_lds: bad argument");
+    const FlatLds l = flat_lds_layout(3u * (unsigned)num_tris, 2u * (unsigned)num_tris, (unsigned)box_tab_bytes,
+                                      (unsigned)pair_queue, (unsigned)rec_size);
+    const uint32_t v[10] = {l.tris, l.mats, l.next_ray, l.best, l.next_at, l.boxtab, l.queues, l.rec_tri, l.rec_cos, l.bytes};
+    memcpy(out, v, sizeof(v));
+    return PT_OK;
+}
+
 int pt_debug_ctx_plan(const pt_ctx* c, int64_t out[24]) {
     if (!c || !out) return set_error(PT_E_ARG, "pt_debug_ctx_plan: NULL argument");
     memcpy(out, c->last_plan, sizeof(c->last_plan));
diff --git a/pathtracer-cpp_amd/csrc/pt_rtc.h b/pathtracer-cpp_amd/csrc/pt_rtc.h
--- a/pathtracer-cpp_amd/csrc/pt_rtc.h
+++ b/pathtracer-cpp_amd/csrc/pt_rtc.h
@@ -18,10 +18,24 @@
 };
 typedef std::shared_future<std::shared_ptr<const RtcCode>> RtcFuture;
 
+struct RtcBaked {
+    bool on = false;
+    int num_tri4 = 0, num_mat4 = 0;
+    int box_tab_bytes = 0;
+    bool pairs = false;
+    int theta_lanes = 0;
+    bool runs(const RtcBaked& plan) const {
+        return !on || (num_tri4 == plan.num_tri4 && num_mat4 == plan.num_mat4 && box_tab_bytes == plan.box_tab_bytes &&
+                       pairs == plan.pairs && theta_lanes == plan.theta_lanes);
+    }
+};
+RtcBaked rtc_baked(int num_tris, bool specular, int flat_boxes);
+int theta_lanes_wanted(bool specular);
+
 int flat_box_pairs(const std::vector<f4>& leaves, int n, std::vector<uint16_t>* tab = nullptr);
 bool leaves_single(const std::vector<f4>& leaves, int n);
 std::string rtc_flat_source(const std::vector<f4>& leaves, int n, bool specular, bool tri_fast, bool albedo_x2,
-                            bool dark, const EmitBox& emit);
+                            bool dark, const EmitBox& emit, const RtcBaked& baked);
 RtcFuture rtc_job(const std::string& src);
 bool rtc_async_ready();
 int rtc_wait_all();
diff --git a/pathtracer-cpp_amd/csrc/pt_rtc.hip b/pathtracer-cpp_amd/csrc/pt_rtc.hip
--- a/pathtracer-cpp_amd/csrc/pt_rtc.hip
+++ b/pathtracer-cpp_amd/csrc/pt_rtc.hip
@@ -42,6 +42,7 @@
 extern "C" const char* pt_rtc_src_trace;
 extern "C" const char* pt_rtc_src_math;
 extern "C" const char* pt_rtc_src_stack;
+extern "C" const char* pt_rtc_src_lds;
 extern "C" const char* pt_rtc_src_hip;
 
 namespace pt {
@@ -97,7 +98,7 @@
 namespace {
 
 std::string flat_mask_source(const std::vector<f4>& leaves, int n, bool specular, bool tri_fast, bool albedo_x2,
-                             bool dark, const EmitBox& emit) {
+                             bool dark, const EmitBox& emit, const RtcBaked& baked) {
     std::vector<std::map<uint32_t, int>> planes(3);
     auto plane = [&](int ax, float c) {
         auto it = planes[ax].find(f2u(c));
@@ -269,6 +270,10 @@
            ";\n    static constexpr bool kTriFast = " + (tri_fast ? "true" : "false") +
            ";\n    static constexpr bool kAlbedoX2 = " + (albedo_x2 ? "true" : "false") +
            ";\n    static constexpr bool kDarkKnown = true;\n    static constexpr bool kDark = " + (dark ? "true" : "false") +
+           ";\n    static constexpr bool kBaked = PT_KCONST != 0;\n    static constexpr int kNumTri4 = " +
+           std::to_string(baked.num_tri4) + ", kNumMat4 = " + std::to_string(baked.num_mat4) +
+           ", kBoxTabBytes = " + std::to_string(baked.box_tab_bytes) + ", kThetaLanes = " + std::to_string(baked.theta_lanes) +
+           ";\n    static constexpr bool kPairs = " + (baked.pairs ? "true" : "false") +
            ";\n" + rej + "    __device__ __forceinline__ static unsigned long long "
            "mask(const TraceArgs&, v3 o, v3 inv) {\n" +
            body + tests + acc + "        return m;\n    }\n};\n}  // namespace pt\n";
@@ -317,21 +322,47 @@
 
 }
 
+bool rtc_kconst_on() {
+    const std::string d = rtc_defines(), key = "#define PT_KCONST ";
+    const size_t at = d.rfind(key);
+    return at == std::string::npos || strtol(d.c_str() + at + key.size(), nullptr, 0) != 0;
+}
+
+int theta_lanes_wanted(bool specular) {
+#if PT_THETA_TAB
+    return hook_int("PT_THETA_LANES", specular ? 32 : 0);
+#else
+    (void)specular;
+    return 0;
+#endif
+}
+
+RtcBaked rtc_baked(int num_tris, bool specular, int flat_boxes) {
+    RtcBaked k;
+    k.on = rtc_kconst_on();
+    k.num_tri4 = 3 * num_tris;
+    k.num_mat4 = 2 * num_tris;
+    k.box_tab_bytes = (int)flat_box_tab_bytes((unsigned)flat_boxes);
+    k.pairs = !hook_off("PT_PAIRS");
+    k.theta_lanes = theta_lanes_wanted(specular);
+    return k;
+}
+
 std::string rtc_flat_source(const std::vector<f4>& leaves, int n, bool specular, bool tri_fast, bool albedo_x2,
-                            bool dark, const EmitBox& emit) {
+                            bool dark, const EmitBox& emit, const RtcBaked& baked) {
     std::string fl = "// extra flags:";
     for (const std::string& f : rtc_extra_flags()) fl += " " + f;
     return fl + "\n" + rtc_defines() + (emit.on && emit.sign_only ? "#define PT_EMIT_SIGN_ONLY 1\n" : "") +
            (ray_stack_on(specular) ? "#define PT_RAY_RESERVE " + std::to_string(ray_reserve()) + "\n" : "#define PT_RAY_STACK 0\n") +
            "#define PT_WAVES " + std::to_string(rtc_waves()) +
-           "\n#define PT_FLAT_ONLY 1\n#ifndef PT_CAM_KERNARG\n#define PT_CAM_KERNARG 0\n#endif\n"
+           "\n#define PT_FLAT_ONLY 1\n#ifndef PT_KCONST\n#define PT_KCONST 1\n#endif\n#ifndef PT_CAM_KERNARG\n#define PT_CAM_KERNARG 0\n#endif\n"
            "#ifndef PT_FRESH_TID\n#define PT_FRESH_TID " + (specular ? "1" : "0") + "\n#endif\n"
            "typedef __hip_internal::int32_t int32_t; typedef __hip_internal::uint32_t uint32_t;\n"
            "typedef __hip_internal::int64_t int64_t; typedef __hip_internal::uint64_t uint64_t;\n"
            "typedef __hip_internal::uint8_t uint8_t; typedef __hip_internal::uint16_t uint16_t;\n"
            "#if !defined(__HIP_DEVICE_COMPILE__)\n#error expected a device compilation (pt_math.h fast paths)\n#endif\n"
            "#include \"pt_trace.h\"\n" +
-           flat_mask_source(leaves, n, specular, tri_fast, albedo_x2, dark, emit) +
+           flat_mask_source(leaves, n, specular, tri_fast, albedo_x2, dark, emit, baked) +
            "extern \"C\" __global__ __launch_bounds__(256, PT_WAVES) void pt_trace_flat_rtc(pt::TraceArgs A) {\n"
            "    pt::trace_body_flat<pt::SceneBoxMask>(A);\n}\n";
 }
@@ -391,7 +422,8 @@
     Sha256 k;
     k.update("pathtracer-amd hipRTC code object v1");
     k.update(src.c_str(), src.size() + 1);
-    for (const char* h : {pt_rtc_src_trace, pt_rtc_src_math, pt_rtc_src_stack, pt_rtc_src_hip}) k.update(h, strlen(h) + 1);
+    for (const char* h : {pt_rtc_src_trace, pt_rtc_src_math, pt_rtc_src_stack, pt_rtc_src_lds, pt_rtc_src_hip})
+        k.update(h, strlen(h) + 1);
     for (const std::string& f : rtc_flags()) k.update(f.c_str(), f.size() + 1);
     int maj = 0, mnr = 0;
     (void)hiprtcVersion(&maj, &mnr);
@@ -602,12 +634,12 @@
         const uint64_t len = n;
         return put(&len, 8) && put(str, n);
     };
-    const char* hdrs[] = {pt_rtc_src_trace, pt_rtc_src_math, pt_rtc_src_stack, pt_rtc_src_hip};
-    const char* names[] = {"pt_trace.h", "pt_math.h", "pt_raystack.h", "pt_hip.h"};
+    const char* hdrs[] = {pt_rtc_src_trace, pt_rtc_src_math, pt_rtc_src_stack, pt_rtc_src_lds, pt_rtc_src_hip};
+    const char* names[] = {"pt_trace.h", "pt_math.h", "pt_raystack.h", "pt_flatlds.h", "pt_hip.h"};
     const std::vector<std::string> flags = rtc_flags();
-    const uint32_t head[3] = {0x51525450u , 4u, (uint32_t)flags.size()};
+    const uint32_t head[3] = {0x51525450u , 5u, (uint32_t)flags.size()};
     bool ok = put(head, 12) && put_str(src.data(), src.size());
-    for (int i = 0; ok && i < 4; i++) ok = put_str(names[i], strlen(names[i])) && put_str(hdrs[i], strlen(hdrs[i]));
+    for (int i = 0; ok && i < 5; i++) ok = put_str(names[i], strlen(names[i])) && put_str(hdrs[i], strlen(hdrs[i]));
     for (size_t i = 0; ok && i < flags.size(); i++) ok = put_str(flags[i].data(), flags[i].size());
     uint32_t resp[2] = {0, 0};
     uint64_t n = 0;
@@ -643,10 +675,10 @@
         if (!out->code.empty()) rtc_disk_store(key, out->code);
         return out;
     }
-    const char* hdrs[] = {pt_rtc_src_trace, pt_rtc_src_math, pt_rtc_src_stack, pt_rtc_src_hip};
-    const char* names[] = {"pt_trace.h", "pt_math.h", "pt_raystack.h", "pt_hip.h"};
+    const char* hdrs[] = {pt_rtc_src_trace, pt_rtc_src_math, pt_rtc_src_stack, pt_rtc_src_lds, pt_rtc_src_hip};
+    const char* names[] = {"pt_trace.h", "pt_math.h", "pt_raystack.h", "pt_flatlds.h", "pt_hip.h"};
     hiprtcProgram prog;
-    if (hiprtcCreateProgram(&prog, src.c_str(), "pt_trace_flat_rtc.hip", 4, hdrs, names) != HIPRTC_SUCCESS) {
+    if (hiprtcCreateProgram(&prog, src.c_str(), "pt_trace_flat_rtc.hip", 5, hdrs, names) != HIPRTC_SUCCESS) {
         out->status = "hiprtcCreateProgram failed";
         return out;
     }
@@ -769,7 +801,8 @@
         return set_error(PT_E_ARG, "scene has no flat leaf list (%d leaves, %d triangles)", ps.num_leaves, ps.num_tris);
     const std::string src =
         rtc_flat_source(ps.leaves, ps.num_leaves, scene_has_specular(ps), ps.coords_small, albedo_x2_ok(ps), scene_dark(ps),
-                        scene_emit_box(ps, scene_dark(ps)));
+                        scene_emit_box(ps, scene_dark(ps)),
+                        rtc_baked(ps.num_tris, scene_has_specular(ps), flat_box_pairs(ps.leaves, ps.num_leaves)));
     if (src_out && cap) {
         const size_t n = std::min(cap - 1, src.size());
         memcpy(src_out, src.data(), n);
@@ -788,7 +821,8 @@
         return set_error(PT_E_ARG, "scene has no flat leaf list (%d leaves, %d triangles)", ps.num_leaves, ps.num_tris);
     const RtcFuture f = rtc_job(
         rtc_flat_source(ps.leaves, ps.num_leaves, scene_has_specular(ps), ps.coords_small, albedo_x2_ok(ps), scene_dark(ps),
-                        scene_emit_box(ps, scene_dark(ps))));
+                        scene_emit_box(ps, scene_dark(ps)),
+                        rtc_baked(ps.num_tris, scene_has_specular(ps), flat_box_pairs(ps.leaves, ps.num_leaves))));
     return f.wait_for(std::chrono::seconds(0)) == std::future_status::ready ? 0 : 1;
 }
 
diff --git a/pathtracer-cpp_amd/csrc/pt_trace.h b/pathtracer-cpp_amd/csrc/pt_trace.h
--- a/pathtracer-cpp_amd/csrc/pt_trace.h
+++ b/pathtracer-cpp_amd/csrc/pt_trace.h
@@ -2,6 +2,7 @@
 
 #include "pt_hip.h"
 #include "pt_math.h"
+#include "pt_flatlds.h"
 #include "pt_raystack.h"
 
 namespace pt {
@@ -205,6 +206,109 @@
     return K;
 }
 
+struct ArgConsts {
+    static constexpr bool kBaked = false;
+    static constexpr bool kThetaTab = true;
+    ArgConsts() = default;
+    __device__ __forceinline__ explicit ArgConsts(const TraceArgs&) {}
+    __device__ __forceinline__ int num_tri4(const TraceArgs& A) const { return A.num_tri4; }
+    __device__ __forceinline__ int num_mat4(const TraceArgs& A) const { return A.num_mat4; }
+    __device__ __forceinline__ int depth(const TraceArgs& A) const { return A.depth; }
+    __device__ __forceinline__ int pair_queue(const TraceArgs& A) const { return A.pair_queue; }
+    __device__ __forceinline__ bool pairs_on(const TraceArgs& A) const { return A.pair_queue > 0; }
+    __device__ __forceinline__ bool fold_unrolled() const { return kernarg_args()->rec_size <= 4; }
+    __device__ __forceinline__ int theta_lanes() const { return kernarg_args()->theta_lanes; }
+    __device__ __forceinline__ uint32_t* flags() const { return kernarg_args()->flags; }
+    __device__ __forceinline__ bool flags_pm() const { return kernarg_args()->flags_pm != 0; }
+    __device__ __forceinline__ float* radiance(const TraceArgs& A) const { return A.radiance; }
+    __device__ __forceinline__ const float4* nodes(const TraceArgs& A) const { return A.nodes; }
+    __device__ __forceinline__ const float4* leaves(const TraceArgs& A) const { return A.leaves; }
+    __device__ __forceinline__ int* exact_stack(const TraceArgs& A) const {
+        return A.exact_stack + (size_t)blockIdx.x * A.exact_rows * kBlock;
+    }
+    __device__ __forceinline__ FlatLds lds(const TraceArgs& A, unsigned box_bytes) const {
+        return flat_lds_layout((unsigned)A.num_tri4, (unsigned)A.num_mat4, box_bytes, (unsigned)A.pair_queue,
+                               (unsigned)A.rec_size);
+    }
+    __device__ __forceinline__ unsigned rec_tri_at(unsigned box_bytes) const {
+        const auto* K = kernarg_args();
+        return flat_lds_fixed((unsigned)K->num_tri4, (unsigned)K->num_mat4, box_bytes) +
+               2u * kFlatLdsWaves * (unsigned)K->pair_queue;
+    }
+    __device__ __forceinline__ unsigned rec_cos_at(unsigned rec_tri) const {
+        return rec_tri + 2u * kFlatLdsBlock * (unsigned)kernarg_args()->rec_size;
+    }
+};
+
+#ifndef PT_KPIN
+#define PT_KPIN 7
+#endif
+template <typename M>
+struct BakedConsts {
+    static constexpr bool kBaked = true;
+    static constexpr bool kThetaTab = M::kThetaLanes > 0;
+    int depth_, pair_queue_;
+    unsigned rec_tri_, rec_cos_;
+    __device__ __forceinline__ static int pin(int v) {
+        asm volatile("" : "+s"(v));
+        return v;
+    }
+    __device__ __forceinline__ explicit BakedConsts(const TraceArgs& A) {
+        depth_ = (PT_KPIN & 1) ? pin(A.depth) : 0;
+        pair_queue_ = (PT_KPIN & 2) ? pin(A.pair_queue) : 0;
+        const FlatLds l = lds(A, (unsigned)M::kBoxTabBytes);
+        rec_tri_ = (PT_KPIN & 4) ? (unsigned)pin((int)l.rec_tri) : 0u;
+        rec_cos_ = (PT_KPIN & 4) ? (unsigned)pin((int)l.rec_cos) : 0u;
+    }
+    __device__ __forceinline__ int num_tri4(const TraceArgs&) const { return M::kNumTri4; }
+    __device__ __forceinline__ int num_mat4(const TraceArgs&) const { return M::kNumMat4; }
+    __device__ __forceinline__ int depth(const TraceArgs&) const { return (PT_KPIN & 1) ? depth_ : kernarg_args()->depth; }
+    __device__ __forceinline__ int pair_queue(const TraceArgs&) const {
+        return (PT_KPIN & 2) ? pair_queue_ : kernarg_args()->pair_queue;
+    }
+    __device__ __forceinline__ bool pairs_on(const TraceArgs&) const { return M::kPairs; }
+    __device__ __forceinline__ bool fold_unrolled() const { return kernarg_args()->rec_size <= 4; }
+    __device__ __forceinline__ const float4* nodes(const TraceArgs&) const { return kernarg_args()->nodes; }
+    __device__ __forceinline__ const float4* leaves(const TraceArgs&) const { return kernarg_args()->leaves; }
+    __device__ __forceinline__ int* exact_stack(const TraceArgs&) const {
+        const auto* K = kernarg_args();
+        return K->exact_stack + (size_t)blockIdx.x * K->exact_rows * kBlock;
+    }
+    __device__ __forceinline__ int theta_lanes() const { return M::kThetaLanes; }
+    __device__ __forceinline__ uint32_t* flags() const { return kernarg_args()->flags; }
+    __device__ __forceinline__ bool flags_pm() const { return kernarg_args()->flags_pm != 0; }
+    __device__ __forceinline__ float* radiance(const TraceArgs& A) const { return A.radiance; }
+    __device__ __forceinline__ FlatLds lds(const TraceArgs& A, unsigned) const {
+        return flat_lds_layout((unsigned)M::kNumTri4, (unsigned)M::kNumMat4, (unsigned)M::kBoxTabBytes, (unsigned)A.pair_queue,
+                               (unsigned)A.rec_size);
+    }
+    __device__ __forceinline__ unsigned rec_tri_at(unsigned) const {
+        if (PT_KPIN & 4) return rec_tri_;
+        return flat_lds_fixed((unsigned)M::kNumTri4, (unsigned)M::kNumMat4, (unsigned)M::kBoxTabBytes) +
+               2u * kFlatLdsWaves * (unsigned)kernarg_args()->pair_queue;
+    }
+    __device__ __forceinline__ unsigned rec_cos_at(unsigned rec_tri) const {
+        return (PT_KPIN & 4) ? rec_cos_ : rec_tri + 2u * kFlatLdsBlock * (unsigned)kernarg_args()->rec_size;
+    }
+};
+
+template <typename M, typename = void>
+struct KConsts {
+    using type = ArgConsts;
+};
+template <typename M>
+struct KConsts<M, decltype((void)M::kBaked)> {
+    template <bool kOn, typename T, typename F>
+    struct Pick {
+        using type = T;
+    };
+    template <typename T, typename F>
+    struct Pick<false, T, F> {
+        using type = F;
+    };
+    using type = typename Pick<M::kBaked, BakedConsts<M>, ArgConsts>::type;
+};
+
 struct NoEmitReject {
     static constexpr bool kCompiled = false;
     __device__ __forceinline__ static bool on() { return false; }
@@ -430,15 +534,16 @@
     return __int_as_float(__builtin_amdgcn_ds_bpermute(addr, __float_as_int(v)));
 }
 
-template <typename BoxMask, typename TriPtr, typename LeafPtr>
+template <typename BoxMask, typename TriPtr, typename LeafPtr, typename KC = ArgConsts>
 __device__ __forceinline__ int intersect_flat_pairs(const TraceArgs& A, unsigned long long mask, LeafPtr lleaves,
                                                     TriPtr tris, uint16_t* __restrict__ queue,
                                                     unsigned long long* __restrict__ best, int tid, int lane, v3 o,
-                                                    v3 d, float& t_out, const uint16_t* __restrict__ boxtab) {
+                                                    v3 d, float& t_out, const uint16_t* __restrict__ boxtab,
+                                                    const KC& kc = KC()) {
     const uint32_t c = (uint32_t)__popcll(mask);
     const uint32_t incl = wave_incl_scan(c);
     const uint32_t total = (uint32_t)__builtin_amdgcn_readlane((int)incl, 63);
-    if (total > (uint32_t)A.pair_queue) {
+    if (total > (uint32_t)kc.pair_queue(A)) {
         if constexpr (BoxMask::kBoxPairs) return flat_box_loop(mask, boxtab, tris, o, d, t_out);
         return flat_tri_loop(mask, lleaves, tris, o, d, t_out);
     }
@@ -1425,11 +1530,12 @@
 
 constexpr int kShadeGo = 0, kShadeEnd = 1, kShadeEndEarly = 2;
 
-template <bool kSpecular = true, typename RecT = int, bool kIds = false, typename Rej = NoEmitReject>
+template <bool kSpecular = true, typename RecT = int, bool kIds = false, typename Rej = NoEmitReject,
+          typename KC = ArgConsts>
 __device__ __forceinline__ int shade_inv(const TraceArgs& A, const float4* __restrict__ mats,
                                           const float4* __restrict__ tris, RecT* __restrict__ rec_tri,
                                           float* __restrict__ rec_cos, int tid, int hit, float t, Lcg& g, v3& o,
-                                          v3& d, v3& inv, int& k, v3& L) {
+                                          v3& d, v3& inv, int& k, v3& L, const KC& kc = KC()) {
     L = v3{0.0f, 0.0f, 0.0f};
     if (hit < 0) return kShadeEnd;
 #ifdef PT_EXP_DUP_SHADE
@@ -1457,7 +1563,7 @@
         L = v3{m1.x, m1.y, m1.z};
         return kShadeEnd;
     }
-    const int depth = A.depth;
+    const int depth = kc.depth(A);
     if (k + 1 >= depth) {
         L = v3{m1.x + 0.0f * m0.y, m1.y + 0.0f * m0.z, m1.z + 0.0f * m0.w};
         return kShadeEnd;
@@ -1490,7 +1596,7 @@
 #if PT_THETA_TAB == 1
         nd = hemisphere_dir_tab(g, n, kernarg_args()->theta_tab);
 #elif PT_THETA_TAB == 2
-        if ((int)__popcll(__ballot(true)) <= kernarg_args()->theta_lanes)
+        if (KC::kThetaTab && (int)__popcll(__ballot(true)) <= kc.theta_lanes())
             nd = hemisphere_dir_tab(g, n, kernarg_args()->theta_tab);
         else
             nd = hemisphere_dir(g, n);
@@ -1556,10 +1662,10 @@
 #ifndef PT_DARK_SKIP
 #define PT_DARK_SKIP 1
 #endif
-template <typename RecT, bool kAlbedoX2 = false, bool kDarkKnown = false, bool kDark = false>
+template <typename RecT, bool kAlbedoX2 = false, bool kDarkKnown = false, bool kDark = false, typename KC = ArgConsts>
 __device__ __forceinline__ void finish_path(const TraceArgs& A, const float4* __restrict__ mats,
                                             const RecT* __restrict__ rec_tri, const float* __restrict__ rec_cos,
-                                            int tid, int k, v3 L, uint32_t at) {
+                                            int tid, int k, v3 L, uint32_t at, const KC& kc = KC()) {
 #ifdef PT_EXP_NO_FOLD
     k = 0;
 #endif
@@ -1569,7 +1675,7 @@
 #ifndef PT_FOLD_UNROLL
 #define PT_FOLD_UNROLL 1
 #endif
-    if (PT_FOLD_UNROLL && kernarg_args()->rec_size <= 4) {
+    if (PT_FOLD_UNROLL && kc.fold_unrolled()) {
         int tj[4];
         float cj[4];
 #pragma unroll
@@ -1628,11 +1734,11 @@
 #ifdef PT_EXP_NO_STORE
     if (L.x == 12345.0f)
 #endif
-    uint32_t* fl = kernarg_args()->flags;
+    uint32_t* fl = kc.flags();
     if (unwind || !fl)
-        *reinterpret_cast<float3*>(A.radiance + 3 * (size_t)at) = make_float3(L.x, L.y, L.z);
+        *reinterpret_cast<float3*>(kc.radiance(A) + 3 * (size_t)at) = make_float3(L.x, L.y, L.z);
     if (unwind && fl) {
-        if (kernarg_args()->flags_pm) {
+        if (kc.flags_pm()) {
             const uint32_t sm = fdiv(at, A.div_npix), q = at - sm * (uint32_t)A.npix;
             atomicOr(fl + flag_word(sm, q, (uint32_t)A.npix), 1u << (sm & 31u));
         } else {
@@ -1680,30 +1786,34 @@
     uint16_t* tri;
     float* cos;
 };
-__device__ __forceinline__ FlatRecs flat_records(float4* lds4) {
-    const auto* K = kernarg_args();
-    uint16_t* rt = reinterpret_cast<uint16_t*>(lds4 + K->num_tri4 + K->num_mat4) + (kBlock / kWave) * K->pair_queue;
-    return FlatRecs{rt, reinterpret_cast<float*>(rt + K->rec_size * kBlock)};
-}
+template <typename BoxMask, typename KC>
+__device__ __forceinline__ FlatRecs flat_records(float4* lds4, const KC& kc) {
+    char* lds = reinterpret_cast<char*>(lds4);
+    const unsigned rt = kc.rec_tri_at(flat_box_tab_bytes((unsigned)BoxMask::kBoxes));
+    return FlatRecs{reinterpret_cast<uint16_t*>(lds + rt), reinterpret_cast<float*>(lds + kc.rec_cos_at(rt))};
+}
+static_assert(kFlatLdsBlock == (unsigned)kBlock && kFlatLdsWaves == (unsigned)(kBlock / kWave), "pt_flatlds.h");
 
 template <typename BoxMask>
 __device__ __forceinline__ void trace_body_flat(const TraceArgs& A) {
     extern __shared__ float4 lds4[];
     const int tid = threadIdx.x;
     const int lane = tid & (kWave - 1);
-    float4* s_tris = lds4;
-    float4* s_mats = s_tris + A.num_tri4;
-    uint16_t* queues = reinterpret_cast<uint16_t*>(s_mats + A.num_mat4);
-    uint16_t* rec_tri = queues + (kBlock / kWave) * A.pair_queue;
-    float* rec_cos = reinterpret_cast<float*>(rec_tri + A.rec_size * kBlock);
-    unsigned long long* best = reinterpret_cast<unsigned long long*>(rec_cos + A.rec_size * kBlock);
-    float4* next_ray = reinterpret_cast<float4*>(best + kBlock);
-    uint32_t* next_at = reinterpret_cast<uint32_t*>(next_ray + kBlock);
-    uint16_t* boxtab = reinterpret_cast<uint16_t*>(next_at + kBlock);
+    using KC = typename KConsts<BoxMask>::type;
+    const KC kc(A);
+    const FlatLds lay = kc.lds(A, flat_box_tab_bytes((unsigned)BoxMask::kBoxes));
+    char* lds = reinterpret_cast<char*>(lds4);
+    float4* s_tris = reinterpret_cast<float4*>(lds + lay.tris);
+    float4* s_mats = reinterpret_cast<float4*>(lds + lay.mats);
+    float4* next_ray = reinterpret_cast<float4*>(lds + lay.next_ray);
+    unsigned long long* best = reinterpret_cast<unsigned long long*>(lds + lay.best);
+    uint32_t* next_at = reinterpret_cast<uint32_t*>(lds + lay.next_at);
+    uint16_t* boxtab = reinterpret_cast<uint16_t*>(lds + lay.boxtab);
+    uint16_t* queues = reinterpret_cast<uint16_t*>(lds + lay.queues);
     if constexpr (BoxMask::kBoxPairs)
         for (int i = tid; i < BoxMask::kBoxes; i += kBlock) boxtab[i] = BoxMask::kBoxTab[i];
-    for (int i = tid; i < A.num_tri4; i += kBlock) s_tris[i] = A.tris[i];
-    for (int i = tid; i < A.num_mat4; i += kBlock) {
+    for (int i = tid; i < kc.num_tri4(A); i += kBlock) s_tris[i] = A.tris[i];
+    for (int i = tid; i < kc.num_mat4(A); i += kBlock) {
         float4 m = A.mats[i];
         if (BoxMask::kAlbedoX2 && !(i & 1)) m = make_float4(m.x, 2.0f * m.y, 2.0f * m.z, 2.0f * m.w);
         s_mats[i] = m;
@@ -1711,8 +1821,7 @@
     __syncthreads();
     const float4* __restrict__ mats = s_mats;
     const float4* __restrict__ tris = s_tris;
-    uint16_t* wq = queues + __builtin_amdgcn_readfirstlane(tid >> 6) * A.pair_queue;
-    int* xstk = A.exact_stack + (size_t)blockIdx.x * A.exact_rows * kBlock;
+    uint16_t* wq = queues + __builtin_amdgcn_readfirstlane(tid >> 6) * kc.pair_queue(A);
 
     bool alive = true;
     bool active = false;
@@ -1831,12 +1940,12 @@
 
         float t = 0.0f;
         int hit = -1;
-        const bool tr = active && A.depth > 0;
-        if (A.depth > 0) n_rays += (unsigned long long)__popcll(__ballot(tr));
+        const bool tr = active && kc.depth(A) > 0;
+        if (kc.depth(A) > 0) n_rays += (unsigned long long)__popcll(__ballot(tr));
         if constexpr (!kCarry) inv = rcp3_exact(d, tr);
         const bool forced = A.force_exact_slab == 1 || (A.force_exact_slab == 2 && ((tid >> 6) & 1));
         const bool fast = !forced && __all(!tr || (BoxMask::kSignMask ? bounded_ray(o, inv) : all_finite(inv)));
-        if (fast && A.pair_queue > 0) {
+        if (fast && kc.pairs_on(A)) {
             if (PT_PRIO_MASK) __builtin_amdgcn_s_setprio(PT_PRIO_MASK);
             unsigned long long mask = BoxMask::mask(A, o, inv);
 #ifdef PT_EXP_DUP_MASK
@@ -1868,14 +1977,14 @@
             t = 1.0f;
 #else
             if (PT_PRIO_PAIRS) __builtin_amdgcn_s_setprio(PT_PRIO_PAIRS);
-            hit = intersect_flat_pairs<BoxMask>(A, mask, A.leaves, tris, wq, best, fresh_tid(), lane, o, d, t, boxtab);
+            hit = intersect_flat_pairs<BoxMask>(A, mask, kc.leaves(A), tris, wq, best, fresh_tid(), lane, o, d, t, boxtab, kc);
             if (PT_PRIO_PAIRS) __builtin_amdgcn_s_setprio(0);
 #endif
             PT_STAMP(st_b3)
             PT_STAMP_ADD(2, st_b2, st_b3)
         } else if (tr) {
-            if (fast) hit = intersect_flat<BoxMask>(A, A.leaves, tris, o, d, inv, t, boxtab);
-            else hit = intersect_tree<false>(A.nodes, tris, xstk, tid, o, d, inv, t);
+            if (fast && !kc.pairs_on(A)) hit = intersect_flat<BoxMask>(A, kc.leaves(A), tris, o, d, inv, t, boxtab);
+            else hit = intersect_tree<false>(kc.nodes(A), tris, kc.exact_stack(A), tid, o, d, inv, t);
         }
         PT_STAMP(st_c)
 
@@ -1883,9 +1992,9 @@
         v3 L{0.0f, 0.0f, 0.0f};
         if (PT_PRIO_SHADE) __builtin_amdgcn_s_setprio(PT_PRIO_SHADE);
         if (active) {
-            const FlatRecs R = flat_records(lds4);
+            const FlatRecs R = flat_records<BoxMask>(lds4, kc);
             sh = shade_inv<BoxMask::kSpecular, uint16_t, false, typename BoxMask::EmitRej>(
-                A, mats, tris, R.tri, R.cos, fresh_tid(), hit, t, g, o, d, inv, k, L);
+                A, mats, tris, R.tri, R.cos, fresh_tid(), hit, t, g, o, d, inv, k, L, kc);
         }
         if (PT_PRIO_SHADE) __builtin_amdgcn_s_setprio(0);
         const bool end = sh != kShadeGo;
@@ -1897,9 +2006,9 @@
         PT_STAMP(st_d)
         if (end) {
             if (PT_PRIO_FOLD) __builtin_amdgcn_s_setprio(PT_PRIO_FOLD);
-            const FlatRecs R = flat_records(lds4);
+            const FlatRecs R = flat_records<BoxMask>(lds4, kc);
             finish_path<uint16_t, BoxMask::kAlbedoX2, BoxMask::kDarkKnown, BoxMask::kDark>(A, mats, R.tri, R.cos,
-                                                                                        fresh_tid(), k, L, at);
+                                                                                        fresh_tid(), k, L, at, kc);
             if (PT_PRIO_FOLD) __builtin_amdgcn_s_setprio(0);
             active = false;
         }
```

Result: faster. 82270, median of 6 (+1.3%).
